# rafaelgmv/Distributed-Autonomous-Exploration-and-Mapping

Hardware: AMD Instinct MI355X
Metric: beam-cell updates/sec + frontier-extract ms on 16384² grid (higher is better)
Workload: dtype int32/u32 ray math + fp32 log-odds (fp64 endpoints)

## Files before the change

### distributed-autonomous-exploration-and-mapping_amd/csrc/dm_api.cpp

```cpp
#include <math.h>
#include <stdarg.h>
#include <stdio.h>
#include <string.h>

#include <algorithm>
#include <new>
#include <string>
#include <vector>

#include "dm_internal.h"

#include <stdlib.h>

hipError_t dm_sync_all(dm_grid* g) {
  for (hipStream_t s : {g->stream, g->fe_streams[0], g->fe_streams[1], g->pass_stream, g->big_stream}) {
    if (!s) continue;
    const hipError_t e = hipStreamSynchronize(s);
    if (e != hipSuccess) return e;
  }
  g->p_pending = false;
  for (auto& f : g->fw) f.busy_pending = false;
  return hipSuccess;
}

// ... 1302 lines not shown
  float* dr = nullptr;
  float* di = nullptr;
  auto cleanup = [&]() { dev_free(dp); dev_free(doff); dev_free(dr); dev_free(di); };
  if ((rc = dev_alloc(&dp, np, "ld06 points")) || (rc = dev_alloc(&doff, S + 1, "ld06 offsets")) ||
      (rc = dev_alloc(&dr, (int64_t)S * N, "ld06 ranges")) ||
      (intensities_out && (rc = dev_alloc(&di, (int64_t)S * N, "ld06 intensities")))) {
    cleanup();
    return rc;
  }
  hipError_t e = hipMemcpyAsync(dp, points, sizeof(dm_ld06_point) * (size_t)np, hipMemcpyHostToDevice, g->stream);
  if (e == hipSuccess)
    e = hipMemcpyAsync(doff, offsets, sizeof(int64_t) * (size_t)(S + 1), hipMemcpyHostToDevice, g->stream);
  if (e == hipSuccess) rc = dm_launch_ld06(g, S, dp, doff, N, laser_scan_dir ? 1 : 0, dr, di);
  if (e == hipSuccess && !rc)
    e = hipMemcpyAsync(ranges_out, dr, sizeof(float) * (size_t)S * N, hipMemcpyDeviceToHost, g->stream);
  if (e == hipSuccess && !rc && intensities_out)
    e = hipMemcpyAsync(intensities_out, di, sizeof(float) * (size_t)S * N, hipMemcpyDeviceToHost, g->stream);
  if (e == hipSuccess) e = hipStreamSynchronize(g->stream);
  cleanup();
  if (e != hipSuccess) return dm_hip_check(e, "dm_ld06_to_scans");
  return rc;
}

static const char kMagic[8] = {'D', 'M', 'A', 'P', '0', '0', '0', '1'};

int dm_save(dm_grid* g, const char* path) {
  int rc = check_grid(g);
  if (rc || (rc = use_device(g))) return rc;
  if (!path) return dm_set_error(DM_ERR_INVALID_ARG, "path is NULL");
  const int64_t cells = g->W * g->R;
  std::vector<float> L((size_t)cells);
  if ((rc = dm_get_logodds(g, L.data()))) return rc;
  FILE* f = fopen(path, "wb");
  if (!f) return dm_set_error(DM_ERR_IO, "cannot open %s for writing", path);
  bool ok = fwrite(kMagic, 1, 8, f) == 8 && fwrite(&g->p, sizeof(dm_params), 1, f) == 1 &&
            fwrite(L.data(), sizeof(float), (size_t)cells, f) == (size_t)cells;
  ok = (fclose(f) == 0) && ok;
  if (!ok) return dm_set_error(DM_ERR_IO, "short write to %s", path);
  return DM_OK;
}

int dm_load(dm_grid* g, const char* path) {
  int rc = check_grid(g);
  if (rc || (rc = use_device(g))) return rc;
  if (!path) return dm_set_error(DM_ERR_INVALID_ARG, "path is NULL");
  FILE* f = fopen(path, "rb");
  if (!f) return dm_set_error(DM_ERR_IO, "cannot open %s", path);
  char magic[8];
  dm_params p;
  const int64_t cells = g->W * g->R;
  std::vector<float> L((size_t)cells);
  bool ok = fread(magic, 1, 8, f) == 8 && memcmp(magic, kMagic, 8) == 0 &&
            fread(&p, sizeof p, 1, f) == 1;
  if (ok && (p.width != g->p.width || p.height != g->p.height || p.band_row0 != g->p.band_row0 ||
             p.band_rows != g->p.band_rows || p.resolution != g->p.resolution)) {
    fclose(f);
    return dm_set_error(DM_ERR_SHAPE, "checkpoint %s has a different grid geometry", path);
  }
  ok = ok && fread(L.data(), sizeof(float), (size_t)cells, f) == (size_t)cells;
  fclose(f);
  if (!ok) return dm_set_error(DM_ERR_IO, "%s is not a dm checkpoint or is truncated", path);
  return dm_set_logodds(g, L.data());
}

int dm_set_stream(dm_grid* g, void* stream) {
  if (int rc0 = not_on_sharded(g, "dm_set_stream")) return rc0;
  int rc = check_grid(g);
  if (rc || (rc = use_device(g))) return rc;
  DM_HIP(dm_sync_all(g));
  if (stream) {
    if (g->own_stream && g->stream) (void)hipStreamDestroy(g->stream);
    g->stream = (hipStream_t)stream;
    g->own_stream = false;
  } else if (!g->own_stream) {
    DM_HIP(hipStreamCreateWithFlags(&g->stream, hipStreamNonBlocking));
    g->own_stream = true;
  }
  return DM_OK;
}

int dm_synchronize(dm_grid* g) {
  if (g && g->sh) return dm_sh_synchronize(g);
  int rc = check_grid(g);
  if (rc || (rc = use_device(g))) return rc;
  DM_HIP(dm_sync_all(g));
  return DM_OK;
}

int dm_profile_enable(dm_grid* g, int enable) {
  if (g && g->sh) return dm_sh_profile_enable(g, enable);
  int rc = check_grid(g);
  if (rc) return rc;
  g->profile = enable != 0;
  return DM_OK;
}

int dm_profile_read(dm_grid* g, dm_kernel_stat* out, int32_t cap, int32_t* n_out) {
  if (g && g->sh) return dm_sh_profile_read(g, out, cap, n_out);
  int rc = check_grid(g);
  if (rc || (rc = use_device(g))) return rc;
  DM_HIP(hipStreamSynchronize(g->stream));
  for (auto& t : g->pending) {
    float ms = 0.0f;
    (void)hipEventElapsedTime(&ms, t.start, t.stop);
    (void)hipEventDestroy(t.start);
    (void)hipEventDestroy(t.stop);
    dm_kernel_stat* s = nullptr;
    for (auto& e : g->stats)
      if (t.name == e.name) s = &e;
    if (!s) {
      dm_kernel_stat ns;
      memset(&ns, 0, sizeof ns);
      snprintf(ns.name, sizeof ns.name, "%s", t.name.c_str());
      g->stats.push_back(ns);
      s = &g->stats.back();
    }
    s->launches += 1;
    s->total_ms += ms;
  }
  g->pending.clear();
  const int32_t n = (int32_t)g->stats.size();
  for (int32_t i = 0; i < std::min(n, cap); ++i) out[i] = g->stats[(size_t)i];
  if (n_out) *n_out = n;
  return DM_OK;
}

int dm_profile_reset(dm_grid* g) {
  if (g && g->sh) return dm_sh_profile_reset(g);
  int rc = check_grid(g);
  if (rc) return rc;
  int32_t n = 0;
  if ((rc = dm_profile_read(g, nullptr, 0, &n))) return rc;
  g->stats.clear();
  return DM_OK;
}

int dm_map_image(dm_grid* g, uint8_t* out) {
  if (g && g->sh) return (out ? dm_sh_map_image(g, out) : dm_set_error(DM_ERR_INVALID_ARG, "out is NULL"));
  int rc = check_grid(g);
  if (rc || (rc = use_device(g))) return rc;
  if (!out) return dm_set_error(DM_ERR_INVALID_ARG, "out is NULL");
  const int64_t cells = g->W * g->R;
  uint8_t* d = nullptr;
  if ((rc = dev_alloc(&d, cells, "image"))) return rc;
  rc = dm_launch_map_image(g, d);
  hipError_t e = hipSuccess;
  if (!rc) e = hipMemcpyAsync(out, d, (size_t)cells, hipMemcpyDeviceToHost, g->stream);
  if (!rc && e == hipSuccess) e = hipStreamSynchronize(g->stream);
  (void)hipFree(d);
  if (e != hipSuccess) return dm_hip_check(e, "dm_map_image");
  return rc;
}

}
```

### distributed-autonomous-exploration-and-mapping_amd/csrc/dm_frontier.hip

```cpp
#include "dm_internal.h"
#include "dm_uf.h"
#include "dm_phase.h"

#include <string.h>

#include <algorithm>

DM_PH_DECL(frontier)
DM_PH_DECL(ftile)

namespace {

constexpr int kFT = 256;
#ifndef DM_EDGE_KERNEL
#define DM_EDGE_KERNEL 1
#endif
#ifndef DM_EDGE_HALVE
#define DM_EDGE_HALVE 0
#endif
#if DM_EDGE_HALVE
#define EDGE_UNITE dm_uf_unite_idx_halve
#else
#define EDGE_UNITE dm_uf_unite_idx2
#endif
// ... 1318 lines not shown
    idx_out[p] = (int32_t)i;
  }
}

__global__ __launch_bounds__(256) void k_rs_rank(double ox, double oy, double res, long long* clusters,
                                                 const long long* sums, const long long* labels,
                                                 const unsigned long long* __restrict__ count, int64_t cap,
                                                 int64_t W, const unsigned long long* __restrict__ keys,
                                                 const int32_t* __restrict__ idx,
                                                 const int32_t* __restrict__ row_off,
                                                 dm_cluster* __restrict__ out, int32_t* __restrict__ rank_of,
                                                 unsigned long long* sorted, const unsigned long long* __restrict__ cnt,
                                                 int ncnt, int sorted_idx, const unsigned long long* __restrict__ fsh,
                                                 dm_raw_record* __restrict__ host_out, int64_t host_cap,
                                                 const unsigned long long* __restrict__ scan_failed) {
  const int64_t K = (int64_t)*count;
  if (*scan_failed) cap = -1;
  if (blockIdx.x == 0) write_rb_header(K, cap, sorted, cnt, ncnt, sorted_idx, fsh, host_out);
  if (K > cap) {
    fix_raw_records(clusters, sums, labels, K);
    return;
  }
  for (int64_t p = (int64_t)blockIdx.x * blockDim.x + threadIdx.x; p < K; p += (int64_t)gridDim.x * blockDim.x) {
    const unsigned long long key = keys[p];
    const int64_t row = (int64_t)(key / (unsigned long long)W);
    const int32_t lo = row_off[row], hi = row_off[row + 1];
    int32_t r = 0;
    int32_t q = lo;
    for (; q + 4 <= hi; q += 4)
      r += (keys[q] < key) + (keys[q + 1] < key) + (keys[q + 2] < key) + (keys[q + 3] < key);
    for (; q < hi; ++q) r += keys[q] < key;
    put_sorted(ox, oy, res, clusters, sums, labels, idx[p], (int64_t)lo + r, out, rank_of, host_out, host_cap);
  }
}

__global__ __launch_bounds__(256) void k_slot_labels(int64_t n, int64_t slot_cap, const int32_t* __restrict__ cslot,
                                                     const int32_t* __restrict__ slot_root,
                                                     const long long* __restrict__ slot_label,
                                                     long long* __restrict__ out) {
  for (int64_t i = (int64_t)blockIdx.x * blockDim.x + threadIdx.x; i < n;
       i += (int64_t)gridDim.x * blockDim.x) {
    const int32_t s = cslot[i];
    out[i] = (s < 0 || s >= slot_cap) ? -1 : slot_label[slot_root[s]];
  }
}

int grid_for(int64_t n, int threads, int64_t cap) {
  int64_t b = (n + threads - 1) / threads;
  if (b < 1) b = 1;
  if (b > cap) b = cap;
  return (int)b;
}

}

static_assert(sizeof(FGeom) == 88, "FGeom has no implicit padding");

static FGeom make_fgeom(const dm_grid* g, bool want_mask, bool want_labels) {
  FGeom fg;
  fg.W = (int32_t)g->W;
  fg.R = (int32_t)g->R;
  fg.row0 = (int32_t)g->row0;
  fg.TX = (int32_t)g->TX;
  fg.TY = (int32_t)g->TY;
  fg.NT = g->NT;
  fg.has_before = g->has_halo[0];
  fg.has_after = g->has_halo[1];
  fg.want_mask = want_mask ? 1 : 0;
  fg.want_labels = want_labels ? 1 : 0;
  fg.H = g->H;
  fg.slot_cap = g->slot_cap;
  fg.slot_per = g->slot_cap / kShards;
  fg.clu_cap = g->slot_cap;
  fg.min_size = g->p.min_frontier_size;
  return fg;
}

DM_PH_READER(frontier)
DM_PH_READER(ftile)

int dm_launch_edge_labels(dm_grid* g) {
  DM_LAUNCH(k_slot_labels, dim3(grid_for(2 * g->W, 256, 1024)), dim3(256), 0, g->stream,
                     2 * g->W, g->slot_cap, g->edge_slot, g->slot_root, g->slot_label, g->edge_label);
  DM_HIP(hipGetLastError());
  return DM_OK;
}

int dm_launch_rank_sort(hipStream_t stream, long long* clusters, const long long* sums,
                        const long long* labels, const unsigned long long* d_count,
                        int64_t max_records, double ox, double oy, double res, dm_cluster* out,
                        int32_t* rank_of, unsigned long long* d_sorted, const unsigned long long* cnt,
                        int ncnt, int sorted_idx, const unsigned long long* fsh, dm_raw_record* host_out,
                        int64_t host_cap, int64_t expect) {
  const int64_t cap = std::min<int64_t>(max_records, kRankSortCap);
  const int64_t want = dm_quantize_up(std::max<int64_t>(2 * expect, 2048));
  DM_LAUNCH(k_rank_sort, dim3(grid_for(std::min(cap, want), 64, 1 << 20)), dim3(kSortThreads), 0, stream,
                     ox, oy, res, clusters, sums, labels, d_count, cap, out, rank_of, d_sorted, cnt, ncnt, sorted_idx,
                     fsh, host_out, host_cap);
  DM_HIP(hipGetLastError());
  return DM_OK;
}

int dm_launch_bucket_sort(dm_grid* g, hipStream_t stream, long long* clusters, const long long* sums,
                          const long long* labels, const unsigned long long* d_count,
                          int64_t max_records, int64_t row_base, int64_t rows, dm_cluster* out,
                          int32_t* rank_of, unsigned long long* d_sorted, const unsigned long long* cnt,
                          int ncnt, int sorted_idx, const unsigned long long* fsh, dm_raw_record* host_out,
                          int64_t host_cap) {
  if (max_records > g->bs_cap || rows > g->rs_rows)
    return dm_set_error(DM_ERR_INVALID_ARG, "row sort: %lld records over %lld rows exceed its workspace",
                        (long long)max_records, (long long)rows);
  const long long base = row_base * g->W;
  const int64_t expect = std::min<int64_t>(max_records, std::max<int64_t>(2 * g->sort_hint, 4096));
  const int eg = grid_for(expect, 256, 4096);
  const int nsb = (int)((rows + kRsChunk - 1) / kRsChunk);
  DM_LAUNCH(k_rs_count, dim3(eg), dim3(256), 0, stream, clusters, labels, d_count, max_records, base, g->W,
            g->rs_cnt, g->bs_key, g->bs_idx2, g->rs_status, nsb);
  DM_HIP(hipGetLastError());
  DM_LAUNCH(k_rs_scan, dim3(nsb), dim3(256), 0, stream, d_count, max_records, rows, g->rs_cnt, g->rs_off,
            g->rs_status);
  DM_HIP(hipGetLastError());
  DM_LAUNCH(k_rs_place, dim3(eg), dim3(256), 0, stream, d_count, max_records, g->W, g->bs_key, g->bs_idx2,
            g->rs_off, g->bs_key2, g->bs_idx);
  DM_HIP(hipGetLastError());
  DM_LAUNCH(k_rs_rank, dim3(eg), dim3(256), 0, stream, g->p.origin_x, g->p.origin_y, g->p.resolution, clusters,
            sums, labels, d_count, max_records, g->W, g->bs_key2, g->bs_idx, g->rs_off, out, rank_of, d_sorted, cnt,
            ncnt, sorted_idx, fsh, host_out, host_cap, g->rs_status + nsb);
  DM_HIP(hipGetLastError());
  return DM_OK;
}

int dm_enqueue_frontiers(dm_grid* g, bool want_mask, bool want_labels, bool split, hipStream_t* end_stream) {
  const FGeom fg = make_fgeom(g, want_mask, want_labels);
  const int64_t cells = g->R * g->W;
  if (!split) DM_HIP(dm_join_pass_stream(g));
  ++g->rb[g->cur_slot].wepoch;
  ++g->fr_pass;
  g->fparity ^= 1;
  dm_grid::FrWs& fw = g->fw[g->fparity];
  if (fw.busy_pending) {
    DM_HIP(hipStreamWaitEvent(g->stream, fw.busy, 0));
    fw.busy_pending = false;
  }
  dm_select_fw(g, g->fparity);
  unsigned long long* list_n = g->fl_n + 16 * (g->fr_pass % 3);
  if (++g->relist_age >= g->relist_period)
    if (int rc = dm_launch_relist(g, true)) return rc;
  KernelTimer t;
  if (want_mask) DM_HIP(hipMemsetAsync(g->mask, 0, (size_t)cells, g->stream));
  if (want_labels) DM_HIP(hipMemsetAsync(g->cell_slot, 0xFF, sizeof(int32_t) * (size_t)cells, g->stream));
  const int64_t want_waves = g->ftile_hint > 0 ? dm_quantize_up(g->ftile_hint + g->ftile_hint / 4 + 64) : g->NT;
  const int wave_grid = grid_for(std::min<int64_t>(want_waves, g->NT), kFW, 8192);
  const int bits_grid = std::max(wave_grid, 64);
  const bool want_on = g->fmask_mode == 1 || (g->fmask_mode == 0 && g->ftile_hint >= kFmaskOnTiles);
  const bool want_off = g->fmask_mode == 2 || (g->fmask_mode == 0 && g->ftile_hint < kFmaskOnTiles / 4);
  if (!g->fmask_on && want_on) {
    if (!g->fmask_valid) {
      if (int rc = dm_launch_recount(g)) return rc;
    }
    g->fmask_on = true;
  } else if (g->fmask_on && want_off) {
    g->fmask_on = false;
  }
  const bool dense = g->frontier_kernel == 2 ||
                     (g->frontier_kernel == 0 && g->ftf_hint > 0 && g->runs_hint > kDenseRuns * g->ftf_hint &&
                      g->ftf_hint <= kDenseMaxTiles);
  const bool edge = DM_EDGE_KERNEL == 2 ||
                    (DM_EDGE_KERNEL == 1 && !dense && g->sort_hint <= std::max<int64_t>(g->ftile_hint, 1));
  auto* const big_kernel = edge ? k_frontier_tile_big<true> : k_frontier_tile_big<false>;
  auto* const wave_kernel = edge ? k_frontier_tile<true> : k_frontier_tile<false>;
  dm_timer_begin(g, "frontier_bits", &t);
  DM_LAUNCH(k_frontier_bits, dim3(bits_grid), dim3(kFW * 64), 0, g->stream, fg, g->state, g->halo, g->fmask,
            g->fedge, g->tile_seen, g->ftiles, g->ftiles_n, list_n, g->fbits, g->cnt, g->fmask_on ? 1 : 0,
            dense ? nullptr : g->big_tiles, g->fsh, g->edge_slot, 2 * g->W, g->slot_parent, g->fe_flag + kHaltWord,
            g->bits_flag + kStampWord);
  dm_timer_end(g, &t);
  DM_HIP(hipGetLastError());
  hipStream_t ps = g->stream;
  if (split) {
    ps = g->pass_stream;
    hipEvent_t eb = g->ev_bits[g->fparity];
    DM_HIP(hipEventRecord(eb, g->stream));
    DM_HIP(dm_mark_ws_free(g, eb));
    DM_HIP(hipStreamWaitEvent(ps, eb, 0));
  }
  if (end_stream) *end_stream = ps;
  if (!dense) {
    const int big_grid =
        grid_for(std::min<int64_t>(g->NT, dm_quantize_up(g->big_hint + g->big_hint / 4 + 64)), 1, 8192);
    DM_HIP(hipEventRecord(g->ev_bigfork, ps));
    DM_HIP(hipStreamWaitEvent(g->big_stream, g->ev_bigfork, 0));
    dm_timer_begin(g, "frontier_big", &t, g->big_stream);
    DM_LAUNCH(big_kernel, dim3(big_grid), dim3(kFT), 0, g->big_stream, fg, g->fbits,
              g->big_tiles,
              g->ftiles, list_n, g->border, g->rel, g->slot_label, g->slot_parent, g->slot_own,
              g->slot_acc, g->mask, g->cell_slot, g->edge_slot, g->cnt, g->fsh, 0);
    dm_timer_end(g, &t);
    DM_HIP(hipGetLastError());
    DM_HIP(hipEventRecord(g->ev_big, g->big_stream));
    dm_timer_begin(g, "frontier_tile", &t, ps);
    DM_LAUNCH(wave_kernel, dim3(wave_grid), dim3(kFW * 64), 0, ps, fg, g->fbits,
                       g->ftiles, list_n, g->border, g->rel,
                       g->slot_label, g->slot_parent, g->slot_own, g->slot_acc, g->mask, g->cell_slot,
                       g->edge_slot, g->cnt, g->fsh, g->big_tiles);
    dm_timer_end(g, &t);
    DM_HIP(hipGetLastError());
    DM_HIP(hipStreamWaitEvent(ps, g->ev_big, 0));
  } else {
    dm_timer_begin(g, "frontier_tile", &t, ps);
    const int dense_grid = grid_for(std::min<int64_t>(g->NT, g->ftile_hint > 0 ? want_waves : g->NT), 1, 8192);
    DM_LAUNCH(big_kernel, dim3(dense_grid), dim3(kFT), 0, ps, fg, g->fbits, nullptr,
              g->ftiles, list_n,
              g->border, g->rel, g->slot_label, g->slot_parent, g->slot_own, g->slot_acc, g->mask,
              g->cell_slot, g->edge_slot, g->cnt, g->fsh, 1);
    dm_timer_end(g, &t);
    DM_HIP(hipGetLastError());
  }
  if (edge) {
    dm_timer_begin(g, "frontier_edges", &t, ps);
    DM_LAUNCH(k_frontier_edges, dim3(grid_for(DM_EDGE_WAVES * std::min<int64_t>(want_waves, g->NT), kFW, 16384)),
              dim3(kFW * 64), 0, ps, fg, g->ftiles, list_n, g->border, g->rel,
              g->slot_parent, g->cnt);
    dm_timer_end(g, &t);
    DM_HIP(hipGetLastError());
  }
  const int sgrid = grid_for(g->slot_cap, 256, 1024);
  dm_timer_begin(g, "frontier_resolve", &t, ps);
  const int fuse = g->p.min_frontier_size <= 1 ? 1 : 0;
  DM_LAUNCH(k_frontier_resolve, dim3(grid_for(g->slot_cap, 256, g->n_cu)), dim3(256), 0, ps, fg,
                     g->slot_parent, g->slot_root, g->slot_own, g->slot_acc, g->fsh, fuse, g->slot_label,
                     g->clusters, g->slot_k, g->cnt);
  dm_timer_end(g, &t);
  DM_HIP(hipGetLastError());
  if (!fuse) {
    dm_timer_begin(g, "frontier_compact", &t, ps);
    DM_LAUNCH(k_frontier_compact, dim3(sgrid), dim3(256), 0, ps, fg,
                       g->slot_root, g->slot_label, g->slot_acc, g->clusters, g->slot_k, g->cnt, g->fsh);
    dm_timer_end(g, &t);
    DM_HIP(hipGetLastError());
  }
  if (want_labels) {
    DM_LAUNCH(k_slot_labels, dim3(grid_for(cells, 256, 8192)), dim3(256), 0, ps,
                       cells, g->slot_cap, g->cell_slot, g->slot_root, g->slot_label, g->labels);
    DM_HIP(hipGetLastError());
  }
  dm_timer_begin(g, "sort_clusters", &t, ps);
  const int rc = g->sort_hint > g->sort_min
      ? dm_launch_bucket_sort(g, ps, g->clusters, fuse ? g->slot_acc : nullptr, fuse ? g->slot_label : nullptr,
                              g->cnt + CNT_CLUSTERS, g->slot_cap, g->row0, g->R, g->out_clu,
                              g->rank_of, g->cnt + CNT_SORTED, g->cnt, CNT_N, CNT_SORTED, g->fsh,
                              g->h_out_dev, g->h_out_cap)
      : dm_launch_rank_sort(ps, g->clusters, fuse ? g->slot_acc : nullptr, fuse ? g->slot_label : nullptr,
                            g->cnt + CNT_CLUSTERS, g->slot_cap, g->p.origin_x,
                            g->p.origin_y, g->p.resolution, g->out_clu, g->rank_of, g->cnt + CNT_SORTED,
                            g->cnt, CNT_N, CNT_SORTED, g->fsh, g->h_out_dev, g->h_out_cap, g->sort_hint);
  dm_timer_end(g, &t);
  return rc;
}

int dm_frontiers_readback(dm_grid* g, int64_t* n_clusters, int64_t* copied) {
  const unsigned long long* hdr = dm_rb_header(g->h_out);
  memcpy(g->h_cnt, hdr, sizeof(unsigned long long) * CNT_N);
  *copied = std::min<int64_t>(g->h_out_cap, g->slot_cap);
  const unsigned long long most = hdr[CNT_N];
  if (g->h_cnt[CNT_OVERFLOW] & kOvPipeline)
    return dm_set_error(DM_ERR_PIPELINE, "the overlapped pipeline's front-end hand-off timed out: a map "
                                         "update was skipped; dm_reset the handle");
  if ((int64_t)most > g->slot_cap / kShards || (g->h_cnt[CNT_OVERFLOW] & kOvSlots)) {
    *n_clusters = (int64_t)most * kShards;
    return DM_ERR_CAPACITY;
  }
  if (g->h_cnt[CNT_OVERFLOW] & kOvUnionFind)
    return dm_set_error(DM_ERR_INCOMPLETE, "frontier union-find did not converge within its bound "
                                           "(dm_uf.h): this pass has no result");
  *n_clusters = (int64_t)g->h_cnt[CNT_CLUSTERS];
  g->sort_hint = *n_clusters;
  g->ftile_hint = (int64_t)g->h_cnt[CNT_FL0];
  g->runs_hint = (int64_t)hdr[CNT_N + 1];
  g->ftf_hint = (int64_t)hdr[CNT_N + 2];
  g->big_hint = (int64_t)hdr[CNT_N + 3];
  return DM_OK;
}

int dm_launch_frontiers(dm_grid* g, bool want_mask, bool want_labels, int64_t* n_clusters,
                        int64_t* copied) {
  int rc = dm_enqueue_frontiers(g, want_mask, want_labels);
  if (rc) return rc;
  DM_HIP(hipStreamSynchronize(g->stream));
  return dm_frontiers_readback(g, n_clusters, copied);
}
```

### distributed-autonomous-exploration-and-mapping_amd/csrc/dm_integrate.hip

```cpp
#include "dm_internal.h"
#include "dm_phase.h"

#include <algorithm>

DM_PH_DECL(integrate)
DM_TL_DECL(accum)

namespace {

constexpr int kLdsPitch = DM_TS + 1;

struct Geom {
  RayGeom r;
  int32_t act_cap;
  int64_t seg_cap;
  int64_t hitem_cap, heavy_cap;
  int64_t nb;
  int32_t chunks, chunk_len;
  int32_t sparse_pieces;
  int32_t pad;
};

struct BeamChunk {
  int64_t b;
  int32_t k_lo, k_hi;
};

__device__ inline BeamChunk beam_chunk(const Geom& g, int64_t v) {
  BeamChunk c;
  if (g.chunks == 1) {
    c.b = v; c.k_lo = 0; c.k_hi = 0x7FFFFFFF;
    return c;
  }
  const int32_t q = (int32_t)(v / g.nb);
  c.b = v - (int64_t)q * g.nb;
  c.k_lo = q * g.chunk_len;
  c.k_hi = q + 1 == g.chunks ? 0x7FFFFFFF : c.k_lo + g.chunk_len - 1;
  return c;
}

__device__ inline int lane_id() { return __lane_id(); }

constexpr int kHash = 1024;
constexpr int kProbe = 32;

__device__ inline uint32_t tile_hash(int32_t t) { return ((uint32_t)t * 2654435761u) >> 22; }

__device__ inline int hash_insert(int32_t* hkey, int32_t tile) {
  uint32_t h = tile_hash(tile);
  for (int p = 0; p < kProbe; ++p, h = (h + 1) & (kHash - 1)) {
    const int32_t k = atomicCAS(&hkey[h], -1, tile);
    if (k == -1 || k == tile) return (int)h;
  }
  return -1;
}

__device__ inline int hash_find(const int32_t* hkey, int32_t tile) {
  uint32_t h = tile_hash(tile);
  for (int p = 0; p < kProbe; ++p, h = (h + 1) & (kHash - 1)) {
    const int32_t k = hkey[h];
    if (k == tile) return (int)h;
    if (k == -1) return -1;
  }
  return -1;
}

struct LaneRun {
  bool head;
  int head_lane;
  int len;
  int rank;
};

__device__ inline LaneRun lane_run(int32_t tile) {
  const int lane = lane_id();
  const unsigned long long act = __ballot(1);
  const int32_t prev = __shfl_up(tile, 1);
  const bool prev_act = lane > 0 && ((act >> (lane - 1)) & 1ull);
  const bool head = !(prev_act && prev == tile);
  const unsigned long long heads = __ballot(head);
  const unsigned long long le = lane == 63 ? ~0ull : ((2ull << lane) - 1ull);
  LaneRun r;
  r.head = head;
  r.head_lane = 63 - __clzll(heads & le);
  const unsigned long long after = heads & ~le;
  const unsigned long long before_end = after ? ((1ull << (__ffsll(after) - 1)) - 1ull) : ~0ull;
  const unsigned long long from_head = ~((1ull << r.head_lane) - 1ull);
  r.len = __popcll(act & from_head & before_end);
  r.rank = __popcll(act & from_head & ((1ull << lane) - 1ull));
  return r;
}

__device__ inline void first_touch(const Geom& g, int32_t tile, int32_t old, int32_t* act_raw,
                                   unsigned long long* ish, unsigned long long* cnt) {
  if (old != 0) return;
  const int sh = blockIdx.x % kShards;
  const unsigned long long l = atomicAdd(&ish[sh * kShardWords + SH_ACT], 1ull);
  if (l < (unsigned long long)g.act_cap) act_raw[(int64_t)sh * g.act_cap + (int64_t)l] = tile;
  else atomicOr(&cnt[CNT_IOVERFLOW], 1ull);
}

__device__ inline PackedPiece make_piece(const Geom& g, const Beam& bm, int32_t tile, int32_t k0, int32_t k1) {
  const int32_t tx0 = (tile % g.r.TX) * DM_TS;
  const int32_t ty0 = (tile / g.r.TX) * DM_TS;
  return dm_pack_piece(dm_tile_piece(bm, k0, k1, g.r.row0, tx0, ty0, kLdsPitch));
}

__global__ __launch_bounds__(256) void k_beam_prep(RayArgs a, Geom g, const double* __restrict__ pose4,
                                                   const float* __restrict__ ranges,
                                                   const double* __restrict__ trig,
                                                   Beam* __restrict__ beams, int32_t* tile_count,
                                                   int32_t* act_raw, unsigned long long* ish,
                                                   int2* __restrict__ blk_hist, int32_t* __restrict__ blk_n,
                                                   unsigned long long* cnt) {
  __shared__ int32_t hkey[kHash];
  __shared__ int32_t hcnt[kHash];
  __shared__ int32_t s_nh;
  const int tid = threadIdx.x;
  for (int e = tid; e < kHash; e += 256) { hkey[e] = -1; hcnt[e] = 0; }
  if (tid == 0) s_nh = 0;
  __syncthreads();
  const int64_t v = (int64_t)blockIdx.x * blockDim.x + tid;
  if (v < g.nb * g.chunks) {
    const BeamChunk bc = beam_chunk(g, v);
    const int32_t s = (int32_t)(bc.b / a.N), i = (int32_t)(bc.b % a.N);
    const Beam bm = dm_make_beam(a, pose4, ranges, trig, s, i);
    if (bc.k_lo == 0) beams[bc.b] = bm;
    if ((bm.flags & 1) && bc.k_lo <= bm.n) {
      dm_for_each_piece(bm, g.r, [&](int32_t tile, int32_t, int32_t) {
        const LaneRun run = lane_run(tile);
        if (run.head) {
          const int h = hash_insert(hkey, tile);
          if (h >= 0) {
            atomicAdd(&hcnt[h], run.len);
          } else {
            const int32_t old = atomicAdd(&tile_count[tile], run.len);
            first_touch(g, tile, old, act_raw, ish, cnt);
          }
        }
      }, bc.k_lo, bc.k_hi);
    }
  }
  __syncthreads();
  int2* my_hist = blk_hist + (int64_t)blockIdx.x * kHash;
  for (int e = tid; e < kHash; e += 256) {
    const int32_t tile = hkey[e];
    if (tile < 0) continue;
    const int32_t old = atomicAdd(&tile_count[tile], hcnt[e]);
    first_touch(g, tile, old, act_raw, ish, cnt);
    my_hist[atomicAdd(&s_nh, 1)] = make_int2(tile, hcnt[e] | (e << 16));
  }
  __syncthreads();
  if (tid == 0) blk_n[blockIdx.x] = s_nh;
}

constexpr int kChunk = kIntegrateChunk;
// ... 58 lines not shown
  }
  __syncthreads();
  const int64_t n = min((int64_t)soff[kShards], (int64_t)g.act_cap);
  if (blockIdx.x == 0 && tid == 0) cnt[CNT_ACTIVE] = (unsigned long long)n;
  const int64_t stride = (int64_t)gridDim.x * blockDim.x;
  for (int64_t j0 = (int64_t)blockIdx.x * blockDim.x + (tid & ~63); j0 < n; j0 += stride) {
    const int64_t j = j0 + lane;
    int32_t t = -1, c = 0;
    if (j < n) {
      int a = 0, b = kShards - 1;
      while (a < b) {
        const int mid = (a + b + 1) >> 1;
        if (soff[mid] <= j) a = mid; else b = mid - 1;
      }
      t = act_raw[(int64_t)a * g.act_cap + (j - soff[a])];
      c = tile_count[t];
    }
    const bool heavy = c > kMedium;
    const bool medium = c > kChunk && !heavy;
    const bool sparse = t >= 0 && c <= g.sparse_pieces;
    const bool light = t >= 0 && c <= kChunk && !sparse;
    const int32_t nh_items = heavy ? (c + kChunk - 1) / kChunk : (medium ? 1 : 0);
    unsigned long long* const ctr[5] = {&cnt[CNT_SEGS], &cnt[CNT_ITEMS], &cnt[CNT_LITEMS], &cnt[CNT_SITEMS],
                                        &cnt[CNT_HEAVY]};
    const unsigned long long want[5] = {(unsigned long long)c, (unsigned long long)nh_items, light ? 1ull : 0ull,
                                        sparse ? 1ull : 0ull, heavy ? 1ull : 0ull};
    unsigned long long got[5];
    wave_alloc_n<5>(ctr, want, got);
    const unsigned long long p0 = got[0], hi = got[1], li = got[2], si = got[3], ho = got[4];
    if (t < 0) continue;
    tile_cur[t] = (int32_t)p0;
    const bool fits = (int64_t)(p0 + c) <= g.seg_cap && (int64_t)(hi + nh_items) <= g.hitem_cap &&
                      (int64_t)li < (int64_t)g.act_cap && (int64_t)si < (int64_t)g.act_cap &&
                      (int64_t)ho < g.heavy_cap;
    if (!fits) {
      atomicOr(&cnt[CNT_IOVERFLOW], 4ull);
      continue;
    }
    if (sparse) {
      litems[(int64_t)g.act_cap - 1 - (int64_t)si] = make_int4(t, (int32_t)p0, c, -1);
    } else if (light) {
      litems[li] = make_int4(t, (int32_t)p0, c, -1);
    } else if (medium) {
      hitems[hi] = make_int4(t, (int32_t)p0, c, -1);
    } else {
      const int32_t wide = c >= 65536 ? 1 : 0;
      heavy_list[ho] = t | (wide << 31);
      for (int32_t q = 0; q < nh_items; ++q)
        hitems[hi + q] = make_int4(t, (int32_t)p0 + q * kChunk, min(kChunk, c - q * kChunk),
                                   (int32_t)(2 * ho + wide));
    }
  }
}

__device__ inline void put_piece(const Geom& g, PackedPiece* pieces, int64_t idx, const Beam& bm,
                                 int32_t tile, int32_t k0, int32_t k1, unsigned long long* cnt) {
  if (idx >= 0 && idx < g.seg_cap) {
    pieces[idx] = make_piece(g, bm, tile, k0, k1);
  } else {
    atomicOr(&cnt[CNT_IOVERFLOW], 2ull);
  }
}

__global__ __launch_bounds__(256) void k_scatter(RayArgs a, Geom g, const Beam* __restrict__ beams,
                                                 int32_t* tile_cur, const int2* __restrict__ blk_hist,
                                                 const int32_t* __restrict__ blk_n,
                                                 PackedPiece* __restrict__ pieces, unsigned long long* cnt) {
  __shared__ int32_t hkey[kHash];
  __shared__ int32_t hcnt[kHash];
  __shared__ int32_t hbase[kHash];
  const int tid = threadIdx.x;
  for (int e = tid; e < kHash; e += 256) { hkey[e] = -1; hcnt[e] = 0; }
  const int64_t v = (int64_t)blockIdx.x * blockDim.x + tid;
  const bool in = v < g.nb * g.chunks;
  const BeamChunk bc = beam_chunk(g, in ? v : 0);
  Beam bm;
  bm.flags = 0;
  if (in) bm = beams[bc.b];
  const int32_t nh = blk_n[blockIdx.x];
  __syncthreads();
  const int2* my_hist = blk_hist + (int64_t)blockIdx.x * kHash;
  for (int e = tid; e < nh; e += 256) {
    const int2 te = my_hist[e];
    const int h = hash_insert(hkey, te.x);
    if (h >= 0) hbase[h] = atomicAdd(&tile_cur[te.x], te.y & 0xFFFF);
  }
  __syncthreads();
  const bool valid = in && (bm.flags & 1) && bc.k_lo <= bm.n;
  if (valid) {
    dm_for_each_piece(bm, g.r, [&](int32_t tile, int32_t k0, int32_t k1) {
      const LaneRun run = lane_run(tile);
      int32_t pos = -1;
      if (run.head) {
        const int h = hash_find(hkey, tile);
        pos = h >= 0 ? hbase[h] + atomicAdd(&hcnt[h], run.len) : atomicAdd(&tile_cur[tile], run.len);
      }
      pos = __shfl(pos, run.head_lane);
      put_piece(g, pieces, (int64_t)pos + run.rank, bm, tile, k0, k1, cnt);
    }, bc.k_lo, bc.k_hi);
  }
}

struct ApplyArgs {
  float l_occ, l_free, l_min, l_max, occ_t, free_t;
};

__device__ inline int8_t state_of(const ApplyArgs& p, float L) {
  int32_t r = -1;
  r = L <= p.free_t ? 0 : r;
  r = L >= p.occ_t ? 100 : r;
  r = L == 0.0f ? -1 : r;
  return (int8_t)r;
}

__device__ inline float apply_one(const ApplyArgs& p, float L, uint32_t h, uint32_t m) {
  const float t = (float)h * p.l_occ;
  const float u = (float)m * p.l_free;
  L = L + t;
  L = L + u;
  return __builtin_amdgcn_fmed3f(L, p.l_min, p.l_max);
}

#ifndef DM_APPLY_BFI
#define DM_APPLY_BFI 1
#endif
__device__ inline uint32_t nz_mask(uint32_t x) {
  uint32_t r;
  asm("v_min_u32_e32 %0, 1, %1\n\tv_sub_u32_e32 %0, 0, %0" : "=&v"(r) : "v"(x));
  return r;
}
__device__ inline uint32_t bfi(uint32_t m, uint32_t a, uint32_t b) {
  uint32_t r;
  asm("v_bfi_b32 %0, %1, %2, %3" : "=v"(r) : "v"(m), "v"(a), "v"(b));
  return r;
}
__device__ inline uint32_t state_bits(const ApplyArgs& p, float L) {
  const int32_t sge = (int32_t)__float_as_uint(L - p.occ_t) >> 31;
  const int32_t sle = (int32_t)__float_as_uint(p.free_t - L) >> 31;
  const int32_t mz = (int32_t)((__float_as_uint(L) & 0x7FFFFFFFu) - 1u) >> 31;
  uint32_t s = bfi((uint32_t)sle, 0xFFFFFFFFu, 0u);
  s = bfi((uint32_t)sge, s, 100u);
  return s | (uint32_t)mz;
}

__device__ inline uint8_t state_nibbles(uint32_t w) {
  auto zb = [](uint32_t v) {
    uint32_t t = (v & 0x7F7F7F7Fu) + 0x7F7F7F7Fu;
    t = ~(t | v | 0x7F7F7F7Fu);
    return (((t >> 7) * 0x00204081u) >> 21) & 0xFu;
  };
  return (uint8_t)(zb(w) | (zb(~w) << 4));
}

template <class G>
__device__ inline uint8_t state_nibbles_at(const G& g, const int8_t* __restrict__ state, int32_t x0, int32_t y) {
  uint32_t fn = 0u, un = 0u;
  for (int e = 0; e < 4; ++e) {
    if (x0 + e >= g.r.W) break;
    const int8_t b = state[(int64_t)y * g.r.W + x0 + e];
    fn |= (b == 0 ? 1u : 0u) << e;
    un |= (b == -1 ? 1u : 0u) << e;
  }
  return (uint8_t)(fn | (un << 4));
}

__device__ inline uint32_t every4th(uint64_t x) {
  x &= 0x1111111111111111ull;
  x = (x | (x >> 3)) & 0x0303030303030303ull;
  x = (x | (x >> 6)) & 0x000F000F000F000Full;
  x = (x | (x >> 12)) & 0x000000FF000000FFull;
  return (uint32_t)((x | (x >> 24)) & 0xFFFFull);
}

struct EdgeAcc {
  uint64_t w[4] = {0ull, 0ull, 0ull, 0ull};
};
__device__ inline void edge_acc(EdgeAcc& e, uint32_t out, int q, int lane) {
  const int c = lane & 3;
  const uint64_t b0 = __ballot(c == 0 && ((out >> 4) & 1u));
  const uint64_t b3 = __ballot(c == 3 && ((out >> 31) & 1u));
  e.w[0] |= (uint64_t)every4th(b0) << (16 * q);
  e.w[1] |= (uint64_t)every4th(b3 >> 3) << (16 * q);
  if (q == 0 || q == 3) {
    const uint32_t u16 = ((out >> 4) & 0xFu) | ((out >> 8) & 0xF0u) | ((out >> 12) & 0xF00u) | ((out >> 16) & 0xF000u);
    const int base = q == 0 ? 0 : 60;
    uint64_t r = 0ull;
#pragma unroll
    for (int k = 0; k < 4; ++k) r |= (uint64_t)__shfl(u16, base + k) << (16 * k);
    e.w[q == 0 ? 2 : 3] = r;
  }
}

__device__ inline void edge_store(const EdgeAcc& e, uint64_t* __restrict__ fedge, int64_t tile, uint64_t rows,
                                  int lane) {
  if (lane >= 4) return;
  const uint64_t v = lane == 0 ? e.w[0] : lane == 1 ? e.w[1] : lane == 2 ? e.w[2] : e.w[3];
  const uint64_t m = lane < 2 ? rows : ((rows >> (lane == 2 ? 0 : 63)) & 1ull) ? ~0ull : 0ull;
  uint64_t* p = fedge + tile * 4 + lane;
  if (m == ~0ull) *p = v;
  else if (m) *p = (*p & ~m) | (v & m);
}

__device__ inline int32_t zero_bytes(uint32_t x) {
  uint32_t t = (x & 0x7F7F7F7Fu) + 0x7F7F7F7Fu;
  t = ~(t | x | 0x7F7F7F7Fu);
  return __popc(t);
}

template <int ROWS>
struct CellRows {
  float4 l[ROWS];
  char4 s[ROWS];
  bool vec;

  __device__ void prefetch(const Geom& g, int32_t tx0, int32_t ty0, int ly0, int dly, int cx,
                           const float* __restrict__ L, const int8_t* __restrict__ state, int vec_ok) {
    vec = vec_ok && tx0 + cx + 4 <= g.r.W;
#pragma unroll
    for (int rr = 0; rr < ROWS; ++rr) {
      const int32_t y = ty0 + ly0 + rr * dly;
      const int64_t base = (vec && y < g.r.R) ? (int64_t)y * g.r.W + tx0 + cx : 0;
      l[rr] = *reinterpret_cast<const float4*>(L + base);
      s[rr] = *reinterpret_cast<const char4*>(state + base);
    }
  }

  template <class Touched>
  __device__ void load_touched(const Geom& g, int32_t tx0, int32_t ty0, int ly0, int dly, int cx,
                               const float* __restrict__ L, const int8_t* __restrict__ state, int vec_ok,
                               Touched&& touched) {
    vec = vec_ok && tx0 + cx + 4 <= g.r.W;
#pragma unroll
    for (int rr = 0; rr < ROWS; ++rr) {
      const int32_t y = ty0 + ly0 + rr * dly;
      l[rr] = make_float4(0.0f, 0.0f, 0.0f, 0.0f);
      s[rr] = make_char4(0, 0, 0, 0);
      if (vec && y < g.r.R && touched(ly0 + rr * dly)) {
        const int64_t base = (int64_t)y * g.r.W + tx0 + cx;
        l[rr] = *reinterpret_cast<const float4*>(L + base);
        s[rr] = *reinterpret_cast<const char4*>(state + base);
      }
    }
  }

  template <class Counts>
  __device__ void apply(const Geom& g, const ApplyArgs& p, int32_t tx0, int32_t ty0, int ly0, int dly,
                        int cx, float* __restrict__ L, int8_t* __restrict__ state, Counts&& counts,
                        int32_t* sh_T, int32_t* sh_free, uint32_t* sh_U) {
    int32_t dT = 0, dFree = 0;
    uint32_t dU = 0;
#pragma unroll
    for (int rr = 0; rr < ROWS; ++rr) {
      const int ly = ly0 + rr * dly;
      const int32_t y = ty0 + ly;
      if (y >= g.r.R) continue;
      uint32_t h4[4], m4[4];
      counts(ly, h4, m4);
      if (((h4[0] | m4[0]) | (h4[1] | m4[1]) | (h4[2] | m4[2]) | (h4[3] | m4[3])) == 0u) continue;
      const int64_t base = (int64_t)y * g.r.W + tx0 + cx;
      if (sh_U) {
#pragma unroll
        for (int e = 0; e < 4; ++e) dU += tx0 + cx + e < g.r.W ? h4[e] + m4[e] : 0u;
      }
      if (vec && DM_APPLY_BFI) {
        const float lv[4] = {l[rr].x, l[rr].y, l[rr].z, l[rr].w};
        const uint32_t sw = *reinterpret_cast<const uint32_t*>(&s[rr]);
        uint32_t nlb[4], nsw = 0u, msk = 0u;
#pragma unroll
        for (int e = 0; e < 4; ++e) {
          const uint32_t mh = nz_mask(h4[e] | m4[e]);
          const float nl = apply_one(p, lv[e], h4[e], m4[e]);
          nlb[e] = bfi(mh, __float_as_uint(nl), __float_as_uint(lv[e]));
          nsw |= (state_bits(p, nl) & 0xFFu) << (8 * e);
          msk |= (mh & 0xFFu) << (8 * e);
          dT += (int32_t)(mh & 1u);
        }
        const uint32_t ns = bfi(msk, nsw, sw);
        dFree += zero_bytes(ns) - zero_bytes(sw);
        *reinterpret_cast<float4*>(L + base) =
            make_float4(__uint_as_float(nlb[0]), __uint_as_float(nlb[1]), __uint_as_float(nlb[2]),
                        __uint_as_float(nlb[3]));
        *reinterpret_cast<uint32_t*>(state + base) = ns;
      } else if (vec) {
        float lv[4] = {l[rr].x, l[rr].y, l[rr].z, l[rr].w};
        int8_t sv[4] = {(int8_t)s[rr].x, (int8_t)s[rr].y, (int8_t)s[rr].z, (int8_t)s[rr].w};
#pragma unroll
        for (int e = 0; e < 4; ++e) {
          const bool hit = (h4[e] | m4[e]) != 0u;
          const float nl = apply_one(p, lv[e], h4[e], m4[e]);
          const int8_t ns = state_of(p, nl);
          lv[e] = hit ? nl : lv[e];
          sv[e] = hit ? ns : sv[e];
          dT += hit ? 1 : 0;
        }
        const char4 ns4 = make_char4(sv[0], sv[1], sv[2], sv[3]);
        dFree += zero_bytes(*reinterpret_cast<const uint32_t*>(&ns4)) -
                 zero_bytes(*reinterpret_cast<const uint32_t*>(&s[rr]));
        *reinterpret_cast<float4*>(L + base) = make_float4(lv[0], lv[1], lv[2], lv[3]);
        *reinterpret_cast<char4*>(state + base) = ns4;
      } else {
        for (int e = 0; e < 4; ++e) {
          if ((h4[e] | m4[e]) == 0u || tx0 + cx + e >= g.r.W) continue;
          const int64_t i = base + e;
          const int8_t old = state[i];
          const float nl = apply_one(p, L[i], h4[e], m4[e]);
          const int8_t ns = state_of(p, nl);
          L[i] = nl;
          state[i] = ns;
          dT += 1;
          dFree += (ns == 0) - (old == 0);
        }
      }
    }
    if (dT) atomicAdd(sh_T, dT);
    if (dFree) atomicAdd(sh_free, dFree);
    if (dU) atomicAdd(sh_U, dU);
  }
};

__device__ inline int32_t walk_tp(uint32_t* tl, const TilePiece& tp, int32_t len, int lane) {
  int32_t wl = len;
  for (int o = 32; o > 0; o >>= 1) wl = max(wl, __shfl_xor(wl, o));
  const int32_t s0 = len > 0 ? lane % len : 0;
  PieceCursor cur;
  cur.init(tp);
  if (s0 > 0) {
    const int32_t num = tp.rem0 + s0 * tp.two_adb;
    const int32_t dq = dm_udiv_small(num, tp.two_n, __builtin_amdgcn_rcpf((float)tp.two_n));
    cur.addr = tp.addr0 + s0 * tp.da + dq * tp.db;
    cur.rem = num - dq * tp.two_n;
  }
  int32_t k = s0;
  for (int32_t st = 0; st < wl; ++st) {
    if (st < len) {
      atomicAdd(&tl[cur.addr], 1u);
      cur.step(tp);
      if (++k == len) cur.init(tp);
    }
  }
  if (len > 0 && tp.addr_end >= 0) atomicAdd(&tl[tp.addr_end], 0xFFFFu);
  return len;
}

__device__ inline int32_t walk_piece(uint32_t* tl, const PackedPiece& mine, bool valid, int lane) {
  const TilePiece tp = dm_unpack_piece(mine.x, mine.y, mine.z, mine.w);
  return walk_tp(tl, tp, valid ? tp.len : 0, lane);
}

#ifndef DM_SPLIT_WALK
#define DM_SPLIT_WALK 1
#endif

__device__ inline int32_t walk_tp_split(uint32_t* tl, const TilePiece& tp, int32_t len, int32_t f, int32_t part,
                                        float rf, int lane) {
  const SplitPart sp = dm_split_part(len, f, part, rf);
  int32_t wl = sp.n;
  for (int o = 32; o > 0; o >>= 1) wl = max(wl, __shfl_xor(wl, o));
  const int32_t spare = kTileWords + lane;
  PieceCursor cur;
  if (f == 1) cur.init(tp);
  else cur.init_at(tp, sp.j0, __builtin_amdgcn_rcpf((float)tp.two_n));
  for (int32_t st = 0; st < wl; ++st) {
    atomicAdd(&tl[st < sp.n ? cur.addr : spare], 1u);
    cur.step(tp);
  }
  if (sp.n > 0 && sp.j0 + sp.n == len && tp.addr_end >= 0) atomicAdd(&tl[tp.addr_end], 0xFFFFu);
  return sp.n;
}

constexpr int kSparseMax = 15;
#ifndef DM_SPARSE_LIST
#define DM_SPARSE_LIST 256
#endif
constexpr int kSparseList = DM_SPARSE_LIST > 0 ? DM_SPARSE_LIST : 1;

__device__ inline int32_t to_pitch64(int32_t a) {
  return a >= 0 ? a - a / kLdsPitch : -((-a) - (-a) / kLdsPitch);
}

__device__ inline int32_t walk_piece_bytes(uint32_t* tq, const PackedPiece& mine, bool valid, int32_t f,
                                           int32_t part, float rf) {
  TilePiece tp = dm_unpack_piece(mine.x, mine.y, mine.z, mine.w);
  const int32_t len = valid ? tp.len : 0;
  const SplitPart sp = dm_split_part(len, f, part, rf);
  int32_t wl = sp.n;
  for (int o = 32; o > 0; o >>= 1) wl = max(wl, __shfl_xor(wl, o));
  tp.addr0 = to_pitch64(tp.addr0);
  tp.da = to_pitch64(tp.da);
  tp.db = to_pitch64(tp.db);
  PieceCursor cur;
  if (f == 1) cur.init(tp);
  else cur.init_at(tp, sp.j0, __builtin_amdgcn_rcpf((float)tp.two_n));
  for (int32_t st = 0; st < wl; ++st) {
    if (st < sp.n) atomicAdd(&tq[cur.addr >> 2], 1u << (8 * (cur.addr & 3)));
    cur.step(tp);
  }
  if (sp.n > 0 && sp.j0 + sp.n == len && tp.addr_end >= 0) {
    const int32_t e = to_pitch64(tp.addr_end);
    atomicAdd(&tq[e >> 2], 0x0Fu << (8 * (e & 3)));
  }
  return sp.n;
}

__device__ inline PackedPiece no_piece() {
  PackedPiece q;
  q.x = 0u; q.y = 0u; q.z = 0u; q.w = 1u;
  return q;
}

__device__ inline int32_t free_update(int32_t old, int32_t dfree, int32_t tile, int32_t* tlist,
                                      unsigned long long* tlist_n) {
  int32_t v = old + dfree;
  if (dfree > 0 && !(old & kTileListed)) {
    v |= kTileListed;
    tlist[atomicAdd(tlist_n, 1ull)] = tile;
  }
  return v;
}

__device__ inline void finish_tile(const Geom& g, int32_t tile, int32_t T, int32_t dfree, uint32_t U,
                                   bool heavy, int32_t* tile_count, int32_t* tile_free, int32_t old_free,
                                   int32_t* tlist, unsigned long long* tlist_n, unsigned long long* ish) {
  unsigned long long* sh = ish + (blockIdx.x % kShards) * kShardWords;
  if (T) {
    atomicAdd(&sh[SH_T], (unsigned long long)T);
    if (heavy) atomicAdd(&sh[SH_TH], (unsigned long long)T);
  }
  if (U) atomicAdd(&sh[SH_U], (unsigned long long)U);
  if (dfree) tile_free[tile] = free_update(old_free, dfree, tile, tlist, tlist_n);
  tile_count[tile] = 0;
}

__device__ inline void heavy_quarter(const Geom& g, const ApplyArgs& p, int64_t h, int q, int32_t tile,
                                     bool wide, uint32_t* __restrict__ slabs, float* __restrict__ L,
                                     int8_t* __restrict__ state, int32_t* s_T, int32_t* s_free,
                                     uint32_t* s_U) {
  constexpr int kQ = DM_TS * DM_TS / 4;
  const int tid = threadIdx.x;
  const int32_t x = (tile % g.r.TX) * DM_TS + (tid & 63);
  const int32_t yq = (tile / g.r.TX) * DM_TS + q * (DM_TS / 4) + (tid >> 6);
  uint32_t* sh = slabs + h * (2 * DM_TS * DM_TS) + q * kQ + tid;
  uint32_t hc[4], mc[4];
  float lv[4];
  int8_t sv[4];
#pragma unroll
  for (int k = 0; k < 4; ++k) {
    const int32_t y = yq + 4 * k;
    lv[k] = 0.0f;
    sv[k] = 0;
    if (y < g.r.R && x < g.r.W) {
      lv[k] = L[(int64_t)y * g.r.W + x];
      sv[k] = state[(int64_t)y * g.r.W + x];
    }
  }
#pragma unroll
  for (int k = 0; k < 4; ++k) {
    hc[k] = atomicExch(sh + k * kQuarter, 0u);
    mc[k] = wide ? atomicExch(sh + DM_TS * DM_TS + k * kQuarter, 0u) : 0u;
  }
  int32_t dT = 0, dFree = 0;
  uint32_t dU = 0;
#pragma unroll
  for (int k = 0; k < 4; ++k) {
    uint32_t hk = hc[k], mk;
    if (wide) {
      mk = mc[k];
    } else {
      mk = hk & 0xFFFFu;
      hk >>= 16;
    }
    const int32_t y = yq + 4 * k;
    if ((hk | mk) == 0u || y >= g.r.R || x >= g.r.W) continue;
    const int64_t i = (int64_t)y * g.r.W + x;
    const float nl = apply_one(p, lv[k], hk, mk);
    const int8_t ns = state_of(p, nl);
    L[i] = nl;
    state[i] = ns;
    dU += hk + mk;
    dT += 1;
    dFree += (ns == 0) - (sv[k] == 0);
  }
  if (dT) atomicAdd(s_T, dT);
  if (dFree) atomicAdd(s_free, dFree);
  if (dU) atomicAdd(s_U, dU);
}

#ifndef DM_ACCUM_OCC
#define DM_ACCUM_OCC 7
#endif
#ifndef DM_EARLY_PIECES
#define DM_EARLY_PIECES 1
#endif
constexpr int kAccumPerCu = DM_ACCUM_OCC;
__global__ __launch_bounds__(kQuarter, kAccumPerCu) void k_tile_accum(
    Geom g, ApplyArgs p, const int4* __restrict__ list_a, int cnt_a, const int4* __restrict__ list_b,
    int cnt_b, int cnt_c, const PackedPiece* __restrict__ pieces, int32_t* tile_count, int32_t* tile_free,
    uint32_t* __restrict__ slabs, float* __restrict__ L, int8_t* __restrict__ state,
    const unsigned long long* __restrict__ cnt, unsigned long long* ish, int vec_ok,
    const int32_t* __restrict__ heavy_list, int32_t* heavy_done, int32_t* tlist, unsigned long long* tlist_n,
    unsigned long long* hint, const unsigned long long* __restrict__ halt, uint8_t* __restrict__ tile_seen) {
  __shared__ uint32_t tl[kTileWords + 64];
  __shared__ int32_t s_T, s_free, s_last;
  __shared__ uint32_t s_U;
  const int tid = threadIdx.x, lane = lane_id();
  DM_TL_BEGIN();
  const unsigned long long hv = *halt;
  const unsigned long long ca = cnt[cnt_a];
  const unsigned long long cb = cnt[cnt_b];
  const unsigned long long cc = cnt[cnt_c];
  const int64_t HI = min((int64_t)ca, g.hitem_cap);
  const int64_t LI = min((int64_t)cb, (int64_t)g.act_cap);
  const int64_t n_items = HI + LI;
  const int64_t SI = min((int64_t)cc, (int64_t)g.act_cap);
  const int64_t G = gridDim.x;
  const int64_t sp_rank = ((int64_t)blockIdx.x - n_items % G + G) % G;
  if (blockIdx.x == 0 && tid == 0) {
    volatile unsigned long long* h = hint;
    h[0] = (unsigned long long)(n_items + (SI + 3) / 4);
    h[1] = (unsigned long long)(n_items + SI);
  }
  const unsigned long long idle =
      ((int64_t)blockIdx.x >= n_items && sp_rank * (kQuarter / 64) >= SI) ? 1ull : 0ull;
  if ((hv | idle) != 0ull) {
    DM_TL_END(accum, 0);
    return;
  }
  auto item_of = [&](int64_t it) {
    int4 d = it < n_items ? (it < HI ? list_a[it] : list_b[it - HI]) : make_int4(0, 0, 0, -1);
    d.z = (int64_t)d.y + d.z <= g.seg_cap ? d.z : 0;
    return d;
  };
  const int cx = (tid & 15) * 4;
  __shared__ unsigned long long s_accT, s_accU;
  int4 info = item_of(blockIdx.x);
  int4 next = item_of(blockIdx.x + G);
  PackedPiece mine;
  CellRows<4> cells;
  int32_t tfree;
  auto split_of = [&](const int4& d) -> int32_t {
    const int32_t c = __builtin_amdgcn_readfirstlane(d.z);
    const int32_t heavy = __builtin_amdgcn_readfirstlane(d.w);
    return DM_SPLIT_WALK && heavy < 0 ? dm_split_factor(c, kQuarter) : 1;
  };
  auto piece_of = [&](int32_t f) -> int32_t {
    return f == 1 ? tid : dm_udiv_small(tid, f, __builtin_amdgcn_rcpf((float)f));
  };
  auto load_pieces = [&](const int4& d) -> PackedPiece {
    const int32_t c0 = __builtin_amdgcn_readfirstlane(d.y);
    const int32_t c = __builtin_amdgcn_readfirstlane(d.z);
    return pieces[c0 + min(piece_of(split_of(d)), max(c - 1, 0))];
  };
  mine = load_pieces(info);
  PackedPiece mine_n = mine;
  for (int e = tid; e < kTileWords; e += kQuarter) tl[e] = 0u;
  if (tid == 0) { s_T = 0; s_free = 0; s_U = 0u; s_accT = 0ull; s_accU = 0ull; }
  __syncthreads();
  DM_PH_INIT();
  [[maybe_unused]] unsigned long long tl_word = 0;
  for (int64_t it = blockIdx.x; it < n_items; it += G) {
    tl_word += 1;
    const int32_t tile = __builtin_amdgcn_readfirstlane(info.x);
    const int32_t c0 = __builtin_amdgcn_readfirstlane(info.y);
    const int32_t c = __builtin_amdgcn_readfirstlane(info.z);
    const int32_t heavy = __builtin_amdgcn_readfirstlane(info.w);
    const int32_t tx0 = (tile % g.r.TX) * DM_TS, ty0 = (tile / g.r.TX) * DM_TS;
    DM_PH(dm_phase_acc_integrate, 0);
    if (heavy >= 0) {
      walk_piece(tl, mine, tid < c, lane);
      if (DM_EARLY_PIECES) mine_n = load_pieces(next);
      __syncthreads();
      DM_PH(dm_phase_acc_integrate, 1);
      DM_PH_COUNT(dm_phase_acc_integrate, 17, 1);
      DM_PH_COUNT(dm_phase_acc_integrate, 19, c);
      uint32_t* sh = slabs + (int64_t)(heavy >> 1) * (2 * DM_TS * DM_TS);
      if (heavy & 1) {
        for (int e = tid; e < DM_TS * DM_TS; e += kQuarter) {
          const uint32_t v = tl[(e >> 6) * kLdsPitch + (e & 63)];
          const uint32_t h = v >> 16, m = v & 0xFFFFu;
          if (h) atomicAdd(&sh[e], h);
          if (m) atomicAdd(&sh[DM_TS * DM_TS + e], m);
        }
      } else {
        for (int e = tid; e < DM_TS * DM_TS; e += kQuarter) {
          const uint32_t v = tl[(e >> 6) * kLdsPitch + (e & 63)];
          if (v) atomicAdd(&sh[e], v);
        }
      }
      DM_PH(dm_phase_acc_integrate, 2);
      asm volatile("s_waitcnt vmcnt(0)" ::: "memory");
      __syncthreads();
      if (tid == 0) {
        const int32_t n_it = (tile_count[tile] + kChunk - 1) / kChunk;
        s_last = atomicAdd(&heavy_done[heavy >> 1], 1) == n_it - 1;
      }
      __syncthreads();
      if (s_last) {
#ifdef DM_PHASE_TIMING
        const long long tf0 = wall_clock64();
#endif
        const int64_t h = heavy >> 1;
        const bool wide = heavy_list[h] < 0;
        const int32_t old_free = tid == 0 ? tile_free[tile] : 0;
        for (int q = 0; q < 4; ++q)
          heavy_quarter(g, p, h, q, tile, wide, slabs, L, state, &s_T, &s_free, &s_U);
        __syncthreads();
        if (tid == 0) {
          finish_tile(g, tile, s_T, s_free, s_U, true, tile_count, tile_free, old_free, tlist, tlist_n, ish);
          heavy_done[h] = 0;
          tile_seen[tile] = 1;
        }
#ifdef DM_PHASE_TIMING
        tl_word += (unsigned long long)(wall_clock64() - tf0) << 32;
#endif
      }
    } else {
      tfree = tile_free[tile];
      cells.prefetch(g, tx0, ty0, tid >> 4, 16, cx, L, state, vec_ok);
      int32_t u;
      if (c <= kChunk) {
        const int32_t f = split_of(info);
        const int32_t pi = piece_of(f);
        const TilePiece tp = dm_unpack_piece(mine.x, mine.y, mine.z, mine.w);
        u = walk_tp_split(tl, tp, pi < c ? tp.len : 0, f, tid - pi * f, __builtin_amdgcn_rcpf((float)f), lane);
      } else {
        u = walk_piece(tl, mine, tid < c, lane);
        for (int32_t r0 = kChunk; r0 < c; r0 += kChunk) {
          const PackedPiece more = r0 + tid < c ? pieces[c0 + r0 + tid] : no_piece();
          u += walk_piece(tl, more, r0 + tid < c, lane);
        }
      }
      const bool inside = tx0 + DM_TS <= g.r.W && ty0 + DM_TS <= g.r.R;
      if (inside) {
        for (int o = 32; o > 0; o >>= 1) u += __shfl_xor(u, o);
        if (lane == 0) atomicAdd(&s_U, (uint32_t)u);
      }
      if (DM_EARLY_PIECES) mine_n = load_pieces(next);
      __syncthreads();
      DM_PH(dm_phase_acc_integrate, 3);
      DM_PH_COUNT(dm_phase_acc_integrate, 16, 1);
      DM_PH_COUNT(dm_phase_acc_integrate, 18, c);
      cells.apply(g, p, tx0, ty0, tid >> 4, 16, cx, L, state,
                  [&](int ly, uint32_t* h4, uint32_t* m4) {
                    for (int e = 0; e < 4; ++e) {
                      const uint32_t v = tl[ly * kLdsPitch + cx + e];
                      h4[e] = v >> 16;
                      m4[e] = v & 0xFFFFu;
                    }
                  },
                  &s_T, &s_free, inside ? nullptr : &s_U);
      DM_PH(dm_phase_acc_integrate, 4);
    }
    __syncthreads();
    if (tid == 0 && heavy < 0) {
      s_accT += (unsigned long long)s_T;
      s_accU += (unsigned long long)s_U;
      if (s_free) tile_free[tile] = free_update(tfree, s_free, tile, tlist, tlist_n);
      tile_count[tile] = 0;
      tile_seen[tile] = 1;
    }
    info = next;
    next = item_of(it + 2 * G);
    mine = DM_EARLY_PIECES ? mine_n : load_pieces(info);
    for (int e = tid; e < kTileWords; e += kQuarter) tl[e] = 0u;
    if (tid == 0) { s_T = 0; s_free = 0; s_U = 0u; }
    __syncthreads();
  }
  __shared__ int32_t s_wT[kQuarter / 64], s_wfree[kQuarter / 64];
  __shared__ uint32_t s_wU[kQuarter / 64];
  __shared__ uint16_t s_list[kQuarter / 64][kSparseList];
  const int wv = tid >> 6;
  uint32_t* tq = tl + wv * (DM_TS * DM_TS / 4);
  const int hcx = (lane & 15) * 4;
  if (lane == 0) { s_wT[wv] = 0; s_wfree[wv] = 0; s_wU[wv] = 0u; }
  const int nw = kQuarter / 64;
  for (int64_t it = sp_rank * nw + wv; it < SI; it += (int64_t)G * nw) {
    int4 d = list_b[(int64_t)g.act_cap - 1 - it];
    d.z = (int64_t)d.y + d.z <= g.seg_cap ? d.z : 0;
    const int32_t tile = d.x, c0 = d.y, c = d.z;
    if (lane == 0 && wv == 0) tl_word += 1ull << 16;
    const int32_t tx0 = (tile % g.r.TX) * DM_TS, ty0 = (tile / g.r.TX) * DM_TS;
    const int32_t fs = DM_SPLIT_WALK ? dm_split_factor(c, 64) : 1;
    const float rfs = __builtin_amdgcn_rcpf((float)fs);
    const int32_t spi = fs == 1 ? lane : dm_udiv_small(lane, fs, rfs);
    const PackedPiece sp = spi < c ? pieces[c0 + spi] : no_piece();
    const int32_t sfree = tile_free[tile];
    int32_t u = walk_piece_bytes(tq, sp, spi < c, fs, lane - spi * fs, rfs);
    const bool inside = tx0 + DM_TS <= g.r.W && ty0 + DM_TS <= g.r.R;
    uint32_t wU = 0u;
    if (inside) {
      for (int o = 32; o > 0; o >>= 1) u += __shfl_xor(u, o);
      wU = (uint32_t)u;
    }
    __builtin_amdgcn_fence(__ATOMIC_ACQ_REL, "wavefront");
    __builtin_amdgcn_wave_barrier();
    DM_PH(dm_phase_acc_integrate, 6);
    auto counts = [&](int wi, uint32_t* h4, uint32_t* m4) {
      const uint32_t w = tq[wi];
      for (int e = 0; e < 4; ++e) {
        const uint32_t v = (w >> (8 * e)) & 0xFFu;
        h4[e] = v >> 4;
        m4[e] = v & 0xFu;
      }
    };
    uint16_t* lst = s_list[wv];
    int nt = 0;
    {
      const unsigned long long lt = (1ull << lane) - 1ull;
#pragma unroll
      for (int k = 0; k < 16; ++k) {
        const int wi = k * 64 + lane;
        const bool nz = tq[wi] != 0u;
        const unsigned long long m = __ballot(nz);
        const int at = nt + __popcll(m & lt);
        if (nz && at < kSparseList) lst[at] = (uint16_t)wi;
        nt += __popcll(m);
      }
    }
    __builtin_amdgcn_fence(__ATOMIC_ACQ_REL, "wavefront");
    __builtin_amdgcn_wave_barrier();
    if (DM_SPARSE_LIST > 0 && nt <= kSparseList) {
      for (int e0 = 0; e0 < nt; e0 += 128) {
        const int ea = e0 + lane, eb = e0 + 64 + lane;
        const int wa = ea < nt ? lst[ea] : 0, wb = eb < nt ? lst[eb] : 0;
        CellRows<1> ca, cb;
        ca.load_touched(g, tx0, ty0, wa >> 4, 0, (wa & 15) * 4, L, state, vec_ok, [&](int) { return ea < nt; });
        cb.load_touched(g, tx0, ty0, wb >> 4, 0, (wb & 15) * 4, L, state, vec_ok, [&](int) { return eb < nt; });
        if (ea < nt)
          ca.apply(g, p, tx0, ty0, wa >> 4, 0, (wa & 15) * 4, L, state,
                   [&](int, uint32_t* h4, uint32_t* m4) { counts(wa, h4, m4); }, &s_wT[wv], &s_wfree[wv],
                   inside ? nullptr : &s_wU[wv]);
        if (eb < nt)
          cb.apply(g, p, tx0, ty0, wb >> 4, 0, (wb & 15) * 4, L, state,
                   [&](int, uint32_t* h4, uint32_t* m4) { counts(wb, h4, m4); }, &s_wT[wv], &s_wfree[wv],
                   inside ? nullptr : &s_wU[wv]);
      }
    } else {
      for (int pass = 0; pass < 4; ++pass) {
        const int ly0 = (lane >> 4) + 16 * pass;
        CellRows<4> sc;
        sc.load_touched(g, tx0, ty0, ly0, 4, hcx, L, state, vec_ok,
                        [&](int ly) { return tq[ly * 16 + (hcx >> 2)] != 0u; });
        sc.apply(g, p, tx0, ty0, ly0, 4, hcx, L, state,
                 [&](int ly, uint32_t* h4, uint32_t* m4) { counts(ly * 16 + (hcx >> 2), h4, m4); },
                 &s_wT[wv], &s_wfree[wv], inside ? nullptr : &s_wU[wv]);
      }
    }
    DM_PH(dm_phase_acc_integrate, 7);
    DM_PH_COUNT(dm_phase_acc_integrate, 21, 1);
    DM_PH_COUNT(dm_phase_acc_integrate, 22, c);
    __builtin_amdgcn_fence(__ATOMIC_ACQ_REL, "wavefront");
    __builtin_amdgcn_wave_barrier();
    if (lane == 0) {
      const int32_t T = s_wT[wv], df = s_wfree[wv];
      const uint32_t U = s_wU[wv] + wU;
      atomicAdd(&s_accT, (unsigned long long)T);
      atomicAdd(&s_accU, (unsigned long long)U);
      if (df) tile_free[tile] = free_update(sfree, df, tile, tlist, tlist_n);
      tile_count[tile] = 0;
      tile_seen[tile] = 1;
      s_wT[wv] = 0;
      s_wfree[wv] = 0;
      s_wU[wv] = 0u;
    }
    for (int e = lane; e < DM_TS * DM_TS / 4; e += 64) tq[e] = 0u;
    __builtin_amdgcn_fence(__ATOMIC_ACQ_REL, "wavefront");
    __builtin_amdgcn_wave_barrier();
  }
  __syncthreads();
  if (tid == 0) {
    unsigned long long* sh = ish + (blockIdx.x % kShards) * kShardWords;
    if (s_accT) atomicAdd(&sh[SH_T], s_accT);
    if (s_accU) atomicAdd(&sh[SH_U], s_accU);
  }
  DM_PH_FLUSH(dm_phase_acc_integrate);
  DM_TL_END(accum, tl_word);
}


__global__ __launch_bounds__(256) void k_integrate_reset(unsigned long long* cnt, unsigned long long* ish) {
  const int i = blockIdx.x * blockDim.x + threadIdx.x;
  constexpr int nI = (int)(sizeof(kIntegrateCounters) / sizeof(kIntegrateCounters[0]));
  if (i < nI) cnt[kIntegrateCounters[i]] = 0ull;
  if (i < kShards * kShardWords) ish[i] = 0ull;
}

constexpr unsigned long long kGateTicks = 500000000ull;

__global__ __launch_bounds__(64) void k_seq_signal(unsigned long long* flag) {
  if (threadIdx.x != 0) return;
  const unsigned long long v = __hip_atomic_load(flag + kSigWord, __ATOMIC_RELAXED, __HIP_MEMORY_SCOPE_AGENT);
  __hip_atomic_store(flag + kSigWord, v + 1, __ATOMIC_RELAXED, __HIP_MEMORY_SCOPE_AGENT);
}

__global__ __launch_bounds__(64) void k_seq_gate(unsigned long long* flag, unsigned long long* err,
                                                 unsigned long long err_bit, unsigned long long ticks,
                                                 unsigned long long fault) {
  if (threadIdx.x != 0) return;
  const unsigned long long seq = flag[kGateWord] + 1;
  flag[kGateWord] = seq;
  const unsigned long long t0 = wall_clock64();
  while (__hip_atomic_load(flag + kSigWord, __ATOMIC_RELAXED, __HIP_MEMORY_SCOPE_AGENT) < seq + fault) {
    __builtin_amdgcn_s_sleep(2);
    if (wall_clock64() - t0 > ticks) {
      atomicOr(err, err_bit);
      return;
    }
  }
}

__device__ inline uint8_t fmask_byte(uint64_t fm, uint64_t um, int j) {
  return (uint8_t)(((fm >> (4 * j)) & 0xFull) | (((um >> (4 * j)) & 0xFull) << 4));
}

__global__ __launch_bounds__(256) void k_recount(Geom g, const int8_t* __restrict__ state,
                                                 int32_t* __restrict__ tile_free, uint8_t* __restrict__ fmask,
                                                 uint64_t* __restrict__ fedge, uint8_t* __restrict__ tile_seen) {
  const int64_t tile = blockIdx.x;
  const int32_t tx0 = (int32_t)(tile % g.r.TX) * DM_TS, ty0 = (int32_t)(tile / g.r.TX) * DM_TS;
  __shared__ int32_t acc, seen;
  __shared__ uint64_t s_edge[4][4];
  if (threadIdx.x == 0) { acc = 0; seen = 0; }
  __syncthreads();
  int32_t c = 0, known = 0;
  uint64_t ew[4] = {0ull, 0ull, 0ull, 0ull};
  uint8_t* tm = fmask + tile * (DM_TS * 16);
  for (int e = threadIdx.x; e < DM_TS * DM_TS; e += 256) {
    const int32_t x = tx0 + (e & 63), y = ty0 + (e >> 6);
    const int8_t b = (x < g.r.W && y < g.r.R) ? state[(int64_t)y * g.r.W + x] : (int8_t)1;
    c += b == 0;
    known |= (x < g.r.W && y < g.r.R && b != -1) ? 1 : 0;
    const uint64_t fm = __ballot(b == 0);
    const uint64_t um = __ballot(b == -1);
    const int l = e & 63, r = e >> 6;
    if (l < 16) tm[r * 16 + l] = fmask_byte(fm, um, l);
    ew[0] |= (um & 1ull) << r;
    ew[1] |= (um >> 63) << r;
    if (r == 0) ew[2] = um;
    if (r == DM_TS - 1) ew[3] = um;
  }
  if (c) atomicAdd(&acc, c);
  if (known) seen = 1;
  const int l4 = __lane_id();
  if (l4 < 4) s_edge[threadIdx.x >> 6][l4] = l4 == 0 ? ew[0] : l4 == 1 ? ew[1] : l4 == 2 ? ew[2] : ew[3];
  __syncthreads();
  if (threadIdx.x == 0) {
    tile_free[tile] = acc;
    tile_seen[tile] = (uint8_t)seen;
  }
  if (threadIdx.x < 4)
    fedge[tile * 4 + threadIdx.x] = s_edge[0][threadIdx.x] | s_edge[1][threadIdx.x] | s_edge[2][threadIdx.x] |
                                    s_edge[3][threadIdx.x];
}

constexpr int kListIters = 16;
__global__ __launch_bounds__(256) void k_list_tiles(int64_t NT, int32_t* __restrict__ tile_free,
                                                    int32_t* __restrict__ ftiles, unsigned long long* list_n,
                                                    int iters) {
  const int lane = __lane_id();
  __shared__ int32_t s_wn[kListIters][4];
  __shared__ unsigned long long s_base;
  const int w = threadIdx.x >> 6;
  const int64_t chunk = (int64_t)iters * blockDim.x;
  for (int64_t c0 = (int64_t)blockIdx.x * chunk; c0 < NT; c0 += (int64_t)gridDim.x * chunk) {
    uint32_t mine = 0u;
    for (int i = 0; i < iters; ++i) {
      const int64_t t = c0 + (int64_t)i * blockDim.x + threadIdx.x;
      if (t >= NT) continue;
      const int32_t v = tile_free[t];
      const bool f = (v & kTileFreeMask) > 0;
      mine |= (f ? 1u : 0u) << i;
      if (f != ((v & kTileListed) != 0)) tile_free[t] = f ? (v | kTileListed) : (v & kTileFreeMask);
    }
    for (int i = 0; i < iters; ++i) {
      const unsigned long long bal = __ballot((mine >> i) & 1u);
      if (lane == 0) s_wn[i][w] = __popcll(bal);
    }
    __syncthreads();
    if (threadIdx.x == 0) {
      int total = 0;
      for (int i = 0; i < iters; ++i) total += s_wn[i][0] + s_wn[i][1] + s_wn[i][2] + s_wn[i][3];
      s_base = total ? atomicAdd(list_n, (unsigned long long)total) : 0ull;
    }
    __syncthreads();
    int64_t pre = (int64_t)s_base;
    for (int i = 0; i < iters; ++i) {
      const bool f = (mine >> i) & 1u;
      const unsigned long long bal = __ballot(f);
      int before = 0;
      for (int q = 0; q < w; ++q) before += s_wn[i][q];
      if (f) {
        const int64_t t = c0 + (int64_t)i * blockDim.x + threadIdx.x;
        ftiles[pre + before + __popcll(bal & ((1ull << lane) - 1ull))] = (int32_t)t;
      }
      pre += s_wn[i][0] + s_wn[i][1] + s_wn[i][2] + s_wn[i][3];
    }
    __syncthreads();
  }
}

__device__ inline uint64_t upto_rows(int p) {
  return p >= 63 ? ~0ull : ((2ull << p) - 1ull);
}

__global__ __launch_bounds__(256) void k_fmask_items(Geom g, const int4* __restrict__ list_a, int cnt_a,
                                                     const int4* __restrict__ list_b, int cnt_b, int cnt_c,
                                                     const PackedPiece* __restrict__ pieces,
                                                     const unsigned long long* __restrict__ cnt,
                                                     const int8_t* __restrict__ state, uint8_t* __restrict__ fmask,
                                                     uint64_t* __restrict__ fedge,
                                                     const unsigned long long* __restrict__ halt) {
  if (*halt) return;
  const int64_t HI = min((int64_t)cnt[cnt_a], g.hitem_cap);
  const int64_t LI = min((int64_t)cnt[cnt_b], (int64_t)g.act_cap);
  const int64_t SI = min((int64_t)cnt[cnt_c], (int64_t)g.act_cap);
  const int lane = __lane_id();
  for (int64_t it = (int64_t)blockIdx.x * 4 + (threadIdx.x >> 6); it < HI + LI + SI;
       it += (int64_t)gridDim.x * 4) {
    const int4 d = it < HI ? list_a[it]
                           : (it < HI + LI ? list_b[it - HI] : list_b[(int64_t)g.act_cap - 1 - (it - HI - LI)]);
    const int32_t tile = __builtin_amdgcn_readfirstlane(d.x);
    uint64_t rows = ~0ull;
    if (it >= HI + LI) {
      const int32_t c0 = __builtin_amdgcn_readfirstlane(d.y);
      const int32_t c = __builtin_amdgcn_readfirstlane(d.z);
      uint64_t mine = 0ull;
      if (lane < c && (int64_t)c0 + c <= g.seg_cap) {
        const PackedPiece q = pieces[c0 + lane];
        const TilePiece tp = dm_unpack_piece(q.x, q.y, q.z, q.w);
        if (tp.len > 0) {
          const int32_t ya = tp.addr0 / kLdsPitch;
          const int32_t yb = dm_piece_addr(tp, tp.len - 1, __builtin_amdgcn_rcpf((float)tp.two_n)) / kLdsPitch;
          const int lo = min(ya, yb), hi = max(ya, yb);
          mine = upto_rows(hi) & ~(lo > 0 ? upto_rows(lo - 1) : 0ull);
        }
      }
      for (int o = 32; o > 0; o >>= 1) mine |= __shfl_xor(mine, o);
      rows = mine;
    }
    const int32_t tx0 = (tile % g.r.TX) * DM_TS, ty0 = (tile / g.r.TX) * DM_TS;
    const int32_t x0 = tx0 + (lane & 3) * 16;
    uint8_t* tm = fmask + (int64_t)tile * (DM_TS * 16);
    EdgeAcc ea;
#pragma unroll
    for (int q = 0; q < 4; ++q) {
      const int ly = 16 * q + (lane >> 2);
      const bool mine = (rows >> ly) & 1ull;
      const int32_t y = ty0 + ly;
      uint32_t out = 0u;
      if (mine && y < g.r.R) {
        const int64_t off = (int64_t)y * g.r.W + x0;
        if (x0 + 16 <= g.r.W && (off & 15) == 0) {
          const uint4 v = *reinterpret_cast<const uint4*>(state + off);
          const uint32_t wd[4] = {v.x, v.y, v.z, v.w};
#pragma unroll
          for (int k = 0; k < 4; ++k) out |= (uint32_t)state_nibbles(wd[k]) << (8 * k);
        } else {
          for (int k = 0; k < 4; ++k) out |= (uint32_t)state_nibbles_at(g, state, x0 + 4 * k, y) << (8 * k);
        }
      }
      if (mine) *reinterpret_cast<uint32_t*>(tm + ly * 16 + (lane & 3) * 4) = out;
      edge_acc(ea, out, q, lane);
    }
    edge_store(ea, fedge, tile, rows, lane);
  }
}

__global__ __launch_bounds__(256) void k_state_from_l(ApplyArgs p, int64_t cells, const float* __restrict__ L,
                                                      int8_t* __restrict__ state) {
  for (int64_t i = (int64_t)blockIdx.x * blockDim.x + threadIdx.x; i < cells;
       i += (int64_t)gridDim.x * blockDim.x)
    state[i] = state_of(p, L[i]);
}

__global__ __launch_bounds__(256) void k_set_state(ApplyArgs p, int64_t cells, const int8_t* __restrict__ in,
                                                   float* __restrict__ L, int8_t* __restrict__ state) {
  for (int64_t i = (int64_t)blockIdx.x * blockDim.x + threadIdx.x; i < cells;
       i += (int64_t)gridDim.x * blockDim.x) {
    const int8_t v = in[i];
    const float l = v == 100 ? p.l_occ : (v == 0 ? p.l_free : 0.0f);
    L[i] = l;
    state[i] = state_of(p, l);
  }
}

__global__ __launch_bounds__(256) void k_map_image(int64_t R, int64_t W, const int8_t* __restrict__ state,
                                                   uint8_t* __restrict__ img) {
  const int64_t cells = R * W;
  for (int64_t i = (int64_t)blockIdx.x * blockDim.x + threadIdx.x; i < cells;
       i += (int64_t)gridDim.x * blockDim.x) {
    const int64_t y = i / W, x = i - y * W;
    const int8_t v = state[i];
    img[(R - 1 - y) * W + x] = v == 0 ? 255 : (v == 100 ? 0 : 127);
  }
}

static_assert(sizeof(Geom) == 72 && sizeof(RayArgs) == 40 && sizeof(ApplyArgs) == 24,
              "kernel argument structs have no implicit padding");

Geom make_geom(const dm_grid* g) {
  Geom ge;
  ge.r.W = (int32_t)g->W;
  ge.r.R = (int32_t)g->R;
  ge.r.row0 = (int32_t)g->row0;
  ge.r.TX = (int32_t)g->TX;
  ge.r.TY = (int32_t)g->TY;
  ge.act_cap = (int32_t)g->act_cap;
  ge.seg_cap = g->segs_cap;
  ge.hitem_cap = g->hitem_cap;
  ge.heavy_cap = g->heavy_cap;
  ge.nb = 0;
  ge.chunks = 1;
  ge.chunk_len = 0;
  ge.sparse_pieces = std::min(g->sparse_pieces, kSparseMax);
  ge.pad = 0;
  return ge;
}

ApplyArgs make_apply(const dm_grid* g) {
  ApplyArgs a;
  a.l_occ = g->p.l_occ;
  a.l_free = g->p.l_free;
  a.l_min = g->p.l_min == 0.0f ? 0.0f : g->p.l_min;
  a.l_max = g->p.l_max == 0.0f ? 0.0f : g->p.l_max;
  a.occ_t = g->p.occ_thresh == 0.0f ? 0.0f : g->p.occ_thresh;
  a.free_t = g->p.free_thresh == 0.0f ? 0.0f : g->p.free_thresh;
  return a;
}

int grid_for(int64_t n, int threads, int64_t cap = 8192) {
  int64_t b = (n + threads - 1) / threads;
  if (b < 1) b = 1;
  if (b > cap) b = cap;
  return (int)b;
}

}

DM_PH_READER(integrate)
DM_TL_READER(accum)

int dm_launch_integrate(dm_grid* g, int32_t S, const double* d_pose4, int32_t N,
                        const float* d_ranges, const double* d_trig) {
  const int64_t nb = (int64_t)S * N;
  g->iw_cur = (g->iw_cur + 1) % dm_grid::kIntSets;
  dm_grid::IntWs& w = g->iw[g->iw_cur];
  hipStream_t fs = g->stream;
  if (g->overlap) {
    fs = dm_fe_stream_of(g, g->iw_cur);
    DM_HIP(dm_mark_ws_free(g));
    DM_HIP(hipStreamWaitEvent(fs, w.free_wait ? w.free_wait : w.ev_free, 0));
  }
  DM_LAUNCH(k_integrate_reset, dim3(2), dim3(256), 0, fs, w.cnt, w.sh);
  DM_HIP(hipGetLastError());
  if (nb == 0) {
    if (g->overlap) {
      DM_HIP(hipEventRecord(g->ev_fe, fs));
      DM_HIP(hipStreamWaitEvent(g->stream, g->ev_fe, 0));
      w.free_owed = true;
    }
    return DM_OK;
  }
  RayArgs a;
  a.S = S;
  a.N = N;
  a.ox = g->p.origin_x;
  a.oy = g->p.origin_y;
  a.res = g->p.resolution;
  a.range_min = g->p.range_min;
  a.range_max = g->p.range_max;
  Geom ge = make_geom(g);
  ge.nb = nb;
  ge.chunks = dm_integrate_chunks(g, nb);
  ge.chunk_len = (int32_t)((g->nmax + ge.chunks) / ge.chunks);
  const int nblk = (int)((nb * ge.chunks + 255) / 256);
  KernelTimer t;
  dm_timer_begin(g, "beam_prep", &t, fs);
  DM_LAUNCH(k_beam_prep, dim3(nblk), dim3(256), 0, fs, a, ge, d_pose4, d_ranges,
            d_trig, w.beams, w.tile_count, w.act_raw, w.sh, w.blk_hist, w.blk_n, w.cnt);
  dm_timer_end(g, &t);
  DM_HIP(hipGetLastError());
  dm_timer_begin(g, "plan", &t, fs);
  DM_LAUNCH(k_plan, dim3(grid_for(g->act_cap, kPlanThreads, 256)), dim3(kPlanThreads), 0, fs,
                     ge, w.act_raw, w.sh, w.tile_cur, w.tile_count, w.hitems, w.litems,
                     w.heavy_list, w.cnt);
  dm_timer_end(g, &t);
  DM_HIP(hipGetLastError());
  dm_timer_begin(g, "scatter", &t, fs);
  DM_LAUNCH(k_scatter, dim3(nblk), dim3(256), 0, fs, a, ge, w.beams,
            w.tile_cur, w.blk_hist, w.blk_n, w.pieces, w.cnt);
  dm_timer_end(g, &t);
  DM_HIP(hipGetLastError());
  if (g->overlap) {
    DM_HIP(hipEventRecord(g->ev_fe_end[g->iw_cur % 2], fs));
    unsigned long long* flag = dm_fe_flag_of(g, g->iw_cur);
    if (int rc = dm_launch_signal(fs, flag)) return rc;
    if (int rc = dm_launch_gate(g->stream, flag, g->fe_flag + kHaltWord, 1ull, g->fault_gate ? 1000ull : 0ull,
                                g->fault_gate ? (1ull << 40) : 0ull))
      return rc;
  }
#ifdef DM_FE_DUMMY
  if (g->overlap) {
    struct Dummy {
      Beam* beams = nullptr; int32_t* tc = nullptr; int32_t* act = nullptr; int2* hist = nullptr;
      int32_t* hn = nullptr; unsigned long long* sh = nullptr; unsigned long long* cnt = nullptr;
      int64_t nb = 0, nt = 0, blocks = 0, act_cap = 0;
    };
    static Dummy d;
    if (d.nb < nb || d.nt < g->NT || d.blocks < nblk || d.act_cap < g->act_cap) {
      (void)hipDeviceSynchronize();
      for (void* q : {(void*)d.beams, (void*)d.tc, (void*)d.act, (void*)d.hist, (void*)d.hn, (void*)d.sh,
                      (void*)d.cnt})
        if (q) (void)hipFree(q);
      d.nb = nb; d.nt = g->NT; d.blocks = nblk; d.act_cap = g->act_cap;
      DM_HIP(hipMalloc((void**)&d.beams, sizeof(Beam) * nb));
      DM_HIP(hipMalloc((void**)&d.tc, sizeof(int32_t) * g->NT));
      DM_HIP(hipMalloc((void**)&d.act, sizeof(int32_t) * g->act_cap * kShards));
      DM_HIP(hipMalloc((void**)&d.hist, sizeof(int2) * 1024 * nblk));
      DM_HIP(hipMalloc((void**)&d.hn, sizeof(int32_t) * nblk));
      DM_HIP(hipMalloc((void**)&d.sh, sizeof(unsigned long long) * kShards * kShardWords));
      DM_HIP(hipMalloc((void**)&d.cnt, sizeof(unsigned long long) * CNT_N));
    }
    DM_HIP(hipMemsetAsync(d.tc, 0, sizeof(int32_t) * g->NT, fs));
    DM_LAUNCH(k_integrate_reset, dim3(2), dim3(256), 0, fs, d.cnt, d.sh);
    DM_LAUNCH(k_beam_prep, dim3(nblk), dim3(256), 0, fs, a, ge, d_pose4, d_ranges, d_trig, d.beams, d.tc,
              d.act, d.sh, d.hist, d.hn, d.cnt);
    DM_HIP(hipGetLastError());
  }
#endif
  const int vec_ok = (g->W % 4 == 0) ? 1 : 0;
  dm_timer_begin(g, "tile_accum", &t);
  const volatile unsigned long long* hint = g->h_hint;
  const int64_t cap = g->hitem_cap + g->act_cap;
#ifndef DM_ACCUM_HINT
#define DM_ACCUM_HINT 1
#endif
  const int64_t hw = DM_ACCUM_HINT ? (int64_t)hint[0] : 0, hi = DM_ACCUM_HINT ? (int64_t)hint[1] : 0;
  const int64_t accum_wgs = hw > 0 ? std::min(cap, dm_quantize_up(hw + hw / 16 + 64)) : cap;
  DM_LAUNCH(k_tile_accum, dim3(grid_for(accum_wgs, 1, dm_grid::kAccumGrid)),
                     dim3(kQuarter), 0,
                     g->stream, ge, make_apply(g), w.hitems, (int)CNT_ITEMS, w.litems, (int)CNT_LITEMS,
                     (int)CNT_SITEMS, w.pieces, w.tile_count, g->tile_free, w.slabs, g->L, g->state, w.cnt, w.sh, vec_ok,
                     w.heavy_list, w.heavy_done, g->ftiles, g->ftiles_n, g->d_hint, g->fe_flag + kHaltWord,
                     g->tile_seen);
  dm_timer_end(g, &t);
  DM_HIP(hipGetLastError());
  if (g->overlap) w.free_owed = true;
  if (!g->fmask_on) {
    g->fmask_valid = false;
    return DM_OK;
  }
  dm_timer_begin(g, "fmask", &t);
  const int64_t fmask_items = hi > 0 ? std::min(cap, dm_quantize_up(hi + hi / 16 + 64)) : cap;
  DM_LAUNCH(k_fmask_items, dim3(grid_for(fmask_items, 4, 8192)), dim3(256), 0, g->stream,
                     ge, w.hitems, (int)CNT_ITEMS, w.litems, (int)CNT_LITEMS, (int)CNT_SITEMS, w.pieces, w.cnt,
                     g->state, g->fmask, g->fedge,
                     g->fe_flag + kHaltWord);
  dm_timer_end(g, &t);
  DM_HIP(hipGetLastError());
  return DM_OK;
}

int dm_launch_signal(hipStream_t s, unsigned long long* flag) {
  DM_LAUNCH(k_seq_signal, dim3(1), dim3(64), 0, s, flag);
  DM_HIP(hipGetLastError());
  return DM_OK;
}

int dm_launch_gate(hipStream_t s, unsigned long long* flag, unsigned long long* err, unsigned long long err_bit,
                   unsigned long long ticks, unsigned long long fault) {
  DM_LAUNCH(k_seq_gate, dim3(1), dim3(64), 0, s, flag, err, err_bit, ticks ? ticks : kGateTicks, fault);
  DM_HIP(hipGetLastError());
  return DM_OK;
}

int dm_launch_relist(dm_grid* g, bool swap) {
  if (swap) {
    const int x = 1 - g->flist_cur;
    if (g->flist_ev_set[x] && hipEventQuery(g->flist_ev[x]) != hipSuccess)
      DM_HIP(hipStreamWaitEvent(g->stream, g->flist_ev[x], 0));
    if (g->pass_stream) {
      DM_HIP(hipEventRecord(g->flist_ev[g->flist_cur], g->pass_stream));
      g->flist_ev_set[g->flist_cur] = true;
    }
    g->flist_cur = x;
    g->ftiles = g->flist[x];
    g->ftiles_n = g->flist_n[x];
  }
  DM_HIP(hipMemsetAsync(g->ftiles_n, 0, sizeof(unsigned long long), g->stream));
  const int iters = (int)std::min<int64_t>(kListIters, std::max<int64_t>(1, (g->NT + 65535) / 65536));
  DM_LAUNCH(k_list_tiles, dim3(grid_for((g->NT + iters - 1) / iters, 256, 1024)), dim3(256), 0, g->stream,
            g->NT, g->tile_free, g->ftiles, g->ftiles_n, iters);
  DM_HIP(hipGetLastError());
  g->relist_age = 0;
  g->relist_period = swap ? std::min(2 * g->relist_period, kRelistPasses) : 1;
  return DM_OK;
}

int dm_launch_recount(dm_grid* g) {
  const Geom ge = make_geom(g);
  DM_HIP(dm_join_pass_stream(g));
  DM_LAUNCH(k_recount, dim3((unsigned)g->NT), dim3(256), 0, g->stream, ge, g->state,
                     g->tile_free, g->fmask, g->fedge, g->tile_seen);
  DM_HIP(hipGetLastError());
  if (int rc = dm_launch_relist(g, false)) return rc;
  g->fmask_valid = true;
  return DM_OK;
}

int dm_launch_state_from_logodds(dm_grid* g) {
  const int64_t cells = g->R * g->W;
  DM_LAUNCH(k_state_from_l, dim3(grid_for(cells, 256)), dim3(256), 0, g->stream,
                     make_apply(g), cells, g->L, g->state);
  DM_HIP(hipGetLastError());
  return dm_launch_recount(g);
}

int dm_launch_set_state(dm_grid* g, const int8_t* d_in) {
  const int64_t cells = g->R * g->W;
  DM_LAUNCH(k_set_state, dim3(grid_for(cells, 256)), dim3(256), 0, g->stream,
                     make_apply(g), cells, d_in, g->L, g->state);
  DM_HIP(hipGetLastError());
  return dm_launch_recount(g);
}

int dm_launch_map_image(dm_grid* g, uint8_t* d_img) {
  const int64_t cells = g->R * g->W;
  DM_LAUNCH(k_map_image, dim3(grid_for(cells, 256)), dim3(256), 0, g->stream, g->R,
                     g->W, g->state, d_img);
  DM_HIP(hipGetLastError());
  return DM_OK;
}
```

### distributed-autonomous-exploration-and-mapping_amd/csrc/dm_internal.h

```cpp
#pragma once

#include <hip/hip_runtime.h>
#include <stdint.h>

#include <atomic>
#include <chrono>
#include <string>
#include <vector>

#include "../../include/dm.h"

#include "dm_ray.h"


enum {
  CNT_ACTIVE = 0,
  CNT_U = 1,
  CNT_T = 2,
  CNT_SEGS = 3,
  CNT_FTILES = 4,
  CNT_SLOTS = 5,
  CNT_CLUSTERS = 6,
  CNT_OVERFLOW = 7,
  CNT_ITEMS = 8,
  CNT_HEAVY = 9,
  CNT_TH = 10,
  CNT_SORTED = 11,
  CNT_FL0 = 12,
  CNT_STAMP = 13,
  CNT_LITEMS = 14,
  CNT_IOVERFLOW = 15,
  CNT_BIG = 16,
  CNT_SITEMS = 17,
  CNT_N = 18
};
constexpr unsigned long long kOvSlots = 4ull;
constexpr unsigned long long kOvUnionFind = 8ull;
constexpr unsigned long long kOvPipeline = 32ull;
constexpr int kHaltWord = 8;
constexpr int kSigWord = 0;
constexpr int kGateWord = 4;
constexpr int kStampWord = 8;
constexpr int kIntegrateCounters[] = {CNT_ACTIVE, CNT_U, CNT_T, CNT_SEGS, CNT_ITEMS,
                                      CNT_HEAVY, CNT_TH, CNT_LITEMS, CNT_IOVERFLOW, CNT_SITEMS};

constexpr int kIntegrateChunk = 256;
constexpr int kIntegrateMedium = 1024;


constexpr int kShards = 32;
constexpr int kShardWords = 16;
static_assert(kShards * kShardWords == 512, "k_integrate_reset covers 512 shard words");
enum { SH_U = 0, SH_T = 1, SH_TH = 2, SH_ACT = 3 };
enum { SH_SLOT = 0, SH_RUNS = 1, SH_FTF = 2, SH_BIG = 3 };

constexpr int kNStats = 11;
constexpr bool dm_stat_is_frontier(int i) { return i >= 7 && i <= 9; }

constexpr int kRbRecords = 6;
static_assert(kRbRecords * sizeof(dm_cluster) >= (CNT_N + 4) * sizeof(unsigned long long), "readback header");
struct dm_raw_record {
  long long label, size, sum_x, sum_y;
};
constexpr int kRbHostRecords = 6;
static_assert(kRbHostRecords * sizeof(dm_raw_record) >= (CNT_N + 4) * sizeof(unsigned long long),
              "readback header");
__host__ __device__ inline unsigned long long* dm_rb_header(dm_raw_record* records) {
  return reinterpret_cast<unsigned long long*>(records - kRbHostRecords);
}
__host__ __device__ inline const unsigned long long* dm_rb_header(const dm_raw_record* records) {
  return reinterpret_cast<const unsigned long long*>(records - kRbHostRecords);
}
__host__ __device__ inline double dm_centroid(double origin, long long sum, long long size, double res) {
  const double m = (double)sum / (double)size;
  return origin + (m + 0.5) * res;
}

struct dm_grid;
hipError_t dm_copy_shards(dm_grid* g);
inline unsigned long long dm_shard_sum(const unsigned long long* sh, int field) {
  unsigned long long s = 0;
  for (int i = 0; i < kShards; ++i) s += sh[i * kShardWords + field];
  return s;
}

struct KernelTimer {
  std::string name;
  hipEvent_t start, stop;
  hipStream_t stream = nullptr;
};

struct dm_shard_set;

struct dm_grid {
  dm_params p;
  dm_shard_set* sh = nullptr;
  int device = 0;
  int n_cu = 256;
  hipStream_t stream = nullptr;
  bool own_stream = false;
  bool overlap = false;
#ifndef DM_FE_STREAMS
#define DM_FE_STREAMS 1
#endif
  static constexpr int kFeStreams = DM_FE_STREAMS;
  static_assert(kFeStreams == 1 || kFeStreams == 2, "one or two front-end streams");
  hipStream_t fe_streams[2] = {nullptr, nullptr};
  hipEvent_t ev_fe = nullptr;
  hipEvent_t ev_fe_end[2] = {nullptr, nullptr};
  unsigned long long* fe_flag = nullptr;
  bool fault_gate = false;
  hipEvent_t ev_bits[2] = {nullptr, nullptr};
  uint64_t integrate_seq = 0;
  struct RbSlot {
    dm_cluster* out_clu = nullptr;
    dm_raw_record* h_out = nullptr;
    dm_raw_record* h_out_dev = nullptr;
    int64_t h_out_cap = 0;
    dm_cluster* m_out = nullptr;
    hipEvent_t ev = nullptr;
    int kind = 0;
    uint64_t seq = 0;
    uint64_t gen = 0;
    uint64_t pass = 0;
    int64_t merge_n = 0;
    uint64_t wepoch = 0, mepoch = 0;
  };
#ifndef DM_RB_SLOTS
#define DM_RB_SLOTS 2
#endif
  static constexpr int kRbSlots = DM_RB_SLOTS;
  static constexpr int kRbSync = kRbSlots;
  RbSlot rb[kRbSlots + 1];
  int rb_head = 0, rb_count = 0;
  int cur_slot = 0;
  uint64_t rb_gen = 0;
  uint64_t fr_pass = 0, m_pass = 0;
  int64_t W = 0, H = 0, R = 0, row0 = 0;
  int64_t TX = 0, TY = 0, NT = 0;
  int32_t nmax = 0;

  float* L = nullptr;
  int8_t* state = nullptr;
  int32_t* tile_free = nullptr;
  uint8_t* fmask = nullptr;
  uint64_t* fedge = nullptr;
  uint8_t* tile_seen = nullptr;
  bool fmask_on = false, fmask_valid = false;
  int fmask_mode = 0;
  unsigned long long* cnt = nullptr;
  unsigned long long* h_cnt = nullptr;
  unsigned long long* fsh = nullptr;
  unsigned long long* h_sh = nullptr;

  int64_t beams_cap = 0;
  int64_t blk_cap = 0;
  int64_t segs_cap = 0;
  int64_t act_cap = 0;
  int64_t hitem_cap = 0;
  int64_t heavy_cap = 0;
  struct IntWs {
    Beam* beams = nullptr;
    int2* blk_hist = nullptr;
    int32_t* blk_n = nullptr;
    int32_t* act_raw = nullptr;
    PackedPiece* pieces = nullptr;
    int4* hitems = nullptr;
    int4* litems = nullptr;
    int32_t* heavy_list = nullptr;
    uint32_t* slabs = nullptr;
    int32_t* heavy_done = nullptr;
    int32_t* tile_count = nullptr;
    int32_t* tile_cur = nullptr;
    unsigned long long* cnt = nullptr;
    unsigned long long* sh = nullptr;
    double* pose4 = nullptr;
    float* ranges = nullptr;
    int64_t pose_cap = 0, ranges_cap = 0;
    hipEvent_t ev_free = nullptr;
    hipEvent_t free_wait = nullptr;
    bool free_owed = false;
  };
  static constexpr int kIntSets = 2;
  IntWs iw[kIntSets];
  int iw_cur = 0;
  double* trig = nullptr; int32_t trig_n = -1; float trig_amin = 0, trig_inc = 0;
  int64_t trig_cap = 0;
  static constexpr int kPoseRing = 2;
  double* h_pose4[kPoseRing] = {nullptr, nullptr};
  hipEvent_t ev_pose[kPoseRing] = {nullptr, nullptr};
  double* h_pose4_dev[kPoseRing] = {nullptr, nullptr};
#ifndef DM_HOST_POSE
#define DM_HOST_POSE 1
#endif
  int64_t h_pose_cap = 0;
  int pose_head = 0;
  int32_t last_S = 0, last_N = 0;

  struct FrWs {
    unsigned long long* cnt = nullptr;
    unsigned long long* fsh = nullptr;
    int32_t* big_tiles = nullptr;
    uint64_t* fbits = nullptr;
    int32_t* edge_slot = nullptr;
    int32_t* slot_parent = nullptr;
    hipEvent_t busy = nullptr;
    hipEvent_t ev_split = nullptr;
    bool busy_pending = false;
    uint64_t busy_pass = 0;
  };
  FrWs fw[2];
  unsigned long long* fl_n = nullptr;
  hipStream_t pass_stream = nullptr;
  hipStream_t big_stream = nullptr;
  hipEvent_t ev_bigfork = nullptr, ev_big = nullptr;
  unsigned long long* bits_flag = nullptr;
  hipEvent_t p_tail = nullptr;
  bool p_pending = false;
  uint64_t p_tail_pass = 0;
  int32_t* ftiles = nullptr;
  unsigned long long* ftiles_n = nullptr;
  int32_t* flist[2] = {nullptr, nullptr};
  unsigned long long* flist_n[2] = {nullptr, nullptr};
  hipEvent_t flist_ev[2] = {nullptr, nullptr};
  bool flist_ev_set[2] = {false, false};
  int flist_cur = 0;
  int relist_age = 0;
  int relist_period = 1;
  int32_t* big_tiles = nullptr;
  uint64_t* fbits = nullptr;
  int32_t* border = nullptr;
  unsigned long long* rel = nullptr;
  int32_t fparity = 0;
  int64_t border_cap = 0;
  int64_t slot_cap = 0;
  long long* slot_label = nullptr;
  int32_t* slot_parent = nullptr;
  int32_t* slot_root = nullptr;
  long long* slot_own = nullptr;
  long long* slot_acc = nullptr;
  long long* clusters = nullptr;
  int32_t* slot_k = nullptr;
  int32_t* rank_of = nullptr;
  dm_cluster* out_clu = nullptr;
  dm_raw_record* h_out = nullptr;
  dm_raw_record* h_out_dev = nullptr;
  int64_t h_out_cap = 0;
  int32_t* cell_slot = nullptr;
  int32_t* edge_slot = nullptr;
  long long* edge_label = nullptr;
  uint8_t* mask = nullptr;
  long long* labels = nullptr;
  int8_t* halo = nullptr;
  int has_halo[2] = {0, 0};
  bool frontier_valid = false;

  unsigned long long* bs_key = nullptr;
  unsigned long long* bs_key2 = nullptr;
  int32_t* bs_idx = nullptr;
  int32_t* bs_idx2 = nullptr;
  int64_t bs_cap = 0;
  int32_t* rs_cnt = nullptr;
  int32_t* rs_off = nullptr;
  unsigned long long* rs_status = nullptr;
  int64_t rs_rows = 0;
  int64_t sort_hint = 0, msort_hint = 0;
  int64_t ftile_hint = 0;
  int64_t runs_hint = 0, ftf_hint = 0;
  int64_t big_hint = 0;
  int64_t sort_min = 4096;
  int frontier_kernel = 0;
  static constexpr int kAccumGrid = 16384;
  static constexpr int kChunkThreadsPerCu = 512;
  int sparse_pieces = 15;

  int64_t m_cap = 0;
  int32_t* m_parent = nullptr;
  long long* m_label = nullptr;
  long long* m_acc = nullptr;
  long long* m_clu = nullptr;
  dm_cluster* m_out = nullptr;
  unsigned long long* m_cnt = nullptr;
  unsigned long long* h_mcnt = nullptr;
  unsigned long long* h_hint = nullptr;
  unsigned long long* d_hint = nullptr;

  int goal_slot = -1, goal_kind = 0;
  uint64_t goal_epoch = 0, goal_gen = 0;
  int64_t goal_n = 0;
  unsigned long long* goal_k[2] = {nullptr, nullptr};
  uint32_t* goal_i[2] = {nullptr, nullptr};
  int64_t goal_cap = 0;
  double* goal_io = nullptr;
  int64_t* goal_idx = nullptr;

  bool profile = false;
  std::vector<KernelTimer> pending;
  std::vector<dm_kernel_stat> stats;
};

inline void dm_select_slot(dm_grid* g, int slot) {
  const dm_grid::RbSlot& r = g->rb[slot];
  g->cur_slot = slot;
  g->out_clu = r.out_clu;
  g->h_out = r.h_out;
  g->h_out_dev = r.h_out_dev;
  g->h_out_cap = r.h_out_cap;
  g->m_out = r.m_out;
}

inline hipStream_t dm_fe_stream_of(const dm_grid* g, int set) {
  return g->fe_streams[set % dm_grid::kFeStreams];
}
inline unsigned long long* dm_fe_flag_of(const dm_grid* g, int set) {
  return g->fe_flag + 16 * (set % dm_grid::kFeStreams);
}
inline int dm_next_set(const dm_grid* g) { return (g->iw_cur + 1) % dm_grid::kIntSets; }

inline hipError_t dm_mark_ws_free(dm_grid* g, hipEvent_t recorded = nullptr) {
  for (int i = 0; i < dm_grid::kIntSets; ++i) {
    dm_grid::IntWs& w = g->iw[i];
    if (!w.free_owed) continue;
    w.free_owed = false;
    w.free_wait = recorded ? recorded : w.ev_free;
    if (recorded) continue;
    const hipError_t e = hipEventRecord(w.ev_free, g->stream);
    if (e != hipSuccess) return e;
  }
  return hipSuccess;
}

inline void dm_select_fw(dm_grid* g, int s) {
  const dm_grid::FrWs& f = g->fw[s];
  g->cnt = f.cnt;
  g->fsh = f.fsh;
  g->big_tiles = f.big_tiles;
  g->fbits = f.fbits;
  g->edge_slot = f.edge_slot;
  g->slot_parent = f.slot_parent;
}

inline void dm_cpu_relax() {
#if defined(__x86_64__) || defined(__i386__)
  __builtin_ia32_pause();
#elif defined(__aarch64__)
  asm volatile("yield" ::: "memory");
#else
  std::atomic_signal_fence(std::memory_order_seq_cst);
#endif
}

inline hipError_t dm_event_wait(hipEvent_t ev) {
  constexpr long long kSpinNs = 2000000;
  const auto t0 = std::chrono::steady_clock::now();
  for (unsigned it = 0;; ++it) {
    const hipError_t e = hipEventQuery(ev);
    if (e != hipErrorNotReady) return e;
    if ((it & 63u) == 63u &&
        std::chrono::duration_cast<std::chrono::nanoseconds>(std::chrono::steady_clock::now() - t0).count() > kSpinNs)
      return hipEventSynchronize(ev);
    dm_cpu_relax();
  }
}

inline hipError_t dm_join_pass_stream(dm_grid* g) {
  if (!g->p_pending) return hipSuccess;
  g->p_pending = false;
  return hipStreamWaitEvent(g->stream, g->p_tail, 0);
}

inline int32_t dm_integrate_chunks(const dm_grid* g, int64_t nb) {
  const int64_t want = (int64_t)dm_grid::kChunkThreadsPerCu * (int64_t)(g->n_cu > 0 ? g->n_cu : 256);
  if (nb <= 0 || nb >= want) return 1;
  const int64_t by_len = (g->nmax + 1) / 64 > 1 ? (g->nmax + 1) / 64 : 1;
  const int64_t by_fill = (want + nb - 1) / nb;
  return (int32_t)(by_fill < by_len ? by_fill : by_len);
}


int dm_launch_integrate(dm_grid* g, int32_t S, const double* d_pose4, int32_t N,
                        const float* d_ranges, const double* d_trig);
int dm_launch_recount(dm_grid* g);
int dm_launch_relist(dm_grid* g, bool swap);
constexpr int kRelistPasses = 16;
int dm_launch_state_from_logodds(dm_grid* g);
int dm_launch_map_image(dm_grid* g, uint8_t* d_img);
int dm_launch_set_state(dm_grid* g, const int8_t* d_state_in);
int dm_enqueue_frontiers(dm_grid* g, bool want_mask, bool want_labels, bool split = false,
                         hipStream_t* end_stream = nullptr);
int dm_launch_signal(hipStream_t s, unsigned long long* flag);
int dm_launch_gate(hipStream_t s, unsigned long long* flag, unsigned long long* err, unsigned long long err_bit,
                   unsigned long long ticks = 0, unsigned long long fault = 0);
int dm_launch_edge_labels(dm_grid* g);
int dm_frontiers_readback(dm_grid* g, int64_t* n_clusters, int64_t* copied);
int dm_launch_frontiers(dm_grid* g, bool want_mask, bool want_labels, int64_t* n_clusters,
                        int64_t* copied);
int dm_launch_rank_sort(hipStream_t stream, long long* clusters, const long long* sums,
                        const long long* labels, const unsigned long long* d_count,
                        int64_t max_records, double ox, double oy, double res, dm_cluster* out,
                        int32_t* rank_of, unsigned long long* d_sorted, const unsigned long long* cnt,
                        int ncnt, int sorted_idx, const unsigned long long* fsh, dm_raw_record* host_out,
                        int64_t host_cap, int64_t expect);
constexpr int64_t kFmaskOnTiles = 8192;
constexpr int32_t kTileListed = 1 << 30;
constexpr int32_t kTileFreeMask = kTileListed - 1;
constexpr int64_t kSlotsPerTile = 4;
int dm_grow_bucket_sort(dm_grid* g, int64_t n);
int dm_launch_bucket_sort(dm_grid* g, hipStream_t stream, long long* clusters, const long long* sums,
                          const long long* labels, const unsigned long long* d_count,
                          int64_t max_records, int64_t row_base, int64_t rows, dm_cluster* out,
                          int32_t* rank_of, unsigned long long* d_sorted, const unsigned long long* cnt,
                          int ncnt, int sorted_idx, const unsigned long long* fsh, dm_raw_record* host_out,
                          int64_t host_cap);
int64_t dm_export_nbytes(int64_t W, int64_t rec_cap);
int dm_launch_export(dm_grid* g, hipStream_t s, void* d_export, int64_t rec_cap);
int dm_launch_merge(dm_grid* g, hipStream_t s, const void* d_gathered, int32_t nranks, int64_t rec_cap,
                    int64_t min_size);
inline hipStream_t dm_exchange_stream_of(const dm_grid* g) { return g->overlap ? g->pass_stream : g->stream; }
int dm_launch_goal_topk(dm_grid* g, const dm_cluster* d_recs, int64_t K, const double* d_robots, int32_t R,
                        int32_t T, int64_t min_size, double w, double min_dist,
                        const unsigned long long** d_k, const uint32_t** d_i);
int dm_launch_goal_gather(dm_grid* g, const dm_cluster* d_recs, const int64_t* d_idx, int32_t R, double* d_xy);
int dm_launch_ld06(dm_grid* g, int32_t S, const dm_ld06_point* d_pts, const int64_t* d_offsets,
                   int32_t N, int dir, float* d_ranges, float* d_intensities);

int dm_sh_destroy(dm_grid* g);
int dm_sh_reset(dm_grid* g);
int dm_sh_integrate(dm_grid* g, int32_t S, const double* poses, int32_t N, const float* ranges, float amin,
                    float inc, uint64_t* U, uint64_t* T);
int dm_sh_integrate_async(dm_grid* g, int32_t S, const double* poses, int32_t N, const float* ranges,
                          float amin, float inc);
int dm_sh_integrate_device(dm_grid* g, int32_t S, const double* d_pose4, int32_t N, const float* d_ranges,
                           float amin, float inc);
int dm_sh_last_counts(dm_grid* g, uint64_t* U, uint64_t* T);
int dm_sh_last_stats(dm_grid* g, uint64_t* out, int32_t cap, int32_t* n_out);
int dm_sh_get_state(dm_grid* g, int8_t* out);
int dm_sh_get_logodds(dm_grid* g, float* out);
int dm_sh_set_logodds(dm_grid* g, const float* in);
int dm_sh_set_state(dm_grid* g, const int8_t* in);
int dm_sh_frontiers(dm_grid* g, uint8_t* mask, int64_t* labels, dm_cluster* out, int64_t cap, int64_t* n_out);
int dm_sh_frontiers_begin(dm_grid* g);
int dm_sh_frontiers_end(dm_grid* g, dm_cluster* out, int64_t cap, int64_t* n_out);
int dm_sh_frontiers_poll(dm_grid* g, int32_t* ready);
int dm_sh_assign_goals(dm_grid* g, const double* robots_xy, int32_t n_robots, int64_t min_size, double w,
                       double min_distance, int64_t* out_index, double* out_xy);
int dm_sh_set_overlap(dm_grid* g, int32_t on);
int dm_sh_synchronize(dm_grid* g);
int dm_sh_profile_enable(dm_grid* g, int enable);
int dm_sh_profile_read(dm_grid* g, dm_kernel_stat* out, int32_t cap, int32_t* n_out);
int dm_sh_profile_reset(dm_grid* g);
int dm_sh_map_image(dm_grid* g, uint8_t* out);
int dm_sh_ld06_to_scans(dm_grid* g, int32_t S, const dm_ld06_point* points, const int64_t* offsets, int32_t N,
                        int dir, float* ranges, float* intensities);
int dm_sh_ld06_to_scans_device(dm_grid* g, int32_t S, const dm_ld06_point* d_points, const int64_t* d_offsets,
                               int32_t N, int dir, float* d_ranges, float* d_intensities);

int dm_set_error(int code, const char* fmt, ...);
int dm_hip_check(hipError_t e, const char* what);
void dm_timer_begin(dm_grid* g, const char* name, KernelTimer* t, hipStream_t s = nullptr);
void dm_timer_end(dm_grid* g, KernelTimer* t);

#define DM_HIP(call)                                         \
  do {                                                       \
    hipError_t _e = (call);                                  \
    if (_e != hipSuccess) return dm_hip_check(_e, #call);    \
  } while (0)

#define DM_LAUNCH(kernel, grid, block, shmem, stream, ...) \
  hipLaunchKernelGGL(kernel, grid, block, shmem, stream, __VA_ARGS__)

inline int64_t dm_quantize_up(int64_t n) {
  if (n <= 8) return n;
  int sh = 0;
  while ((n >> sh) >= 8) ++sh;
  const int64_t step = (int64_t)1 << sh;
  return ((n + step - 1) / step) * step;
}
```

### distributed-autonomous-exploration-and-mapping_amd/csrc/dm_sharded.cpp

```cpp
#include <string.h>

#include <algorithm>
#include <new>
#include <numeric>
#include <vector>

#include "dm_internal.h"

namespace {

constexpr int kSets = 2;

struct Staging {
  double* poses = nullptr;
  float* ranges = nullptr;
  int64_t pose_cap = 0, ranges_cap = 0;
};

int64_t ceil_div(int64_t a, int64_t b) { return (a + b - 1) / b; }

template <class T>
int dev_alloc_on(int dev, T** p, int64_t count, const char* what) {
  (void)hipSetDevice(dev);
  if (*p) { (void)hipFree(*p); *p = nullptr; }
// ... 311 lines not shown
    st.poses = nullptr;
    st.pose_cap = 0;
    DM_HIP(hipHostMalloc((void**)&st.poses, sizeof(double) * 3 * (size_t)std::max(S, 1), hipHostMallocDefault));
    st.pose_cap = (int64_t)std::max(S, 1) * 3;
  }
  if ((int64_t)S * N > st.ranges_cap) {
    if (st.ranges) (void)hipHostFree(st.ranges);
    st.ranges = nullptr;
    st.ranges_cap = 0;
    const int64_t n = std::max<int64_t>((int64_t)S * N, 1);
    DM_HIP(hipHostMalloc((void**)&st.ranges, sizeof(float) * (size_t)n, hipHostMallocDefault));
    st.ranges_cap = n;
  }
  const double reach = (double)p.range_max + 2.0 * p.resolution;
  const double ylo = p.origin_y + (double)s->row0[(size_t)r] * p.resolution - reach;
  const double yhi = p.origin_y + (double)(s->row0[(size_t)r] + s->rows[(size_t)r]) * p.resolution + reach;
  int32_t k = 0;
  for (int32_t i = 0; i < S; ++i) {
    const double y = poses[3 * i + 1];
    if (y < ylo || y > yhi) continue;
    memcpy(st.poses + 3 * (size_t)k, poses + 3 * (size_t)i, 3 * sizeof(double));
    memcpy(st.ranges + (size_t)k * (size_t)N, ranges + (size_t)i * (size_t)N, sizeof(float) * (size_t)N);
    ++k;
  }
  *S_out = k;
  return DM_OK;
}

}

int dm_sh_integrate_async(dm_grid* g, int32_t S, const double* poses, int32_t N, const float* ranges,
                          float amin, float inc) {
  dm_shard_set* s = g->sh;
  if (S < 0 || N < 0) return dm_set_error(DM_ERR_SHAPE, "S and N must be >= 0");
  if ((int64_t)S * N > 0 && (!poses || !ranges)) return dm_set_error(DM_ERR_INVALID_ARG, "poses/ranges is NULL");
  int rc = 0;
  for (int r = 0; r < s->P; ++r) {
    int32_t k = 0;
    if ((rc = sh_stage(s, g->p, r, S, poses, N, ranges, &k))) return rc;
    s->active[(size_t)r] = k > 0;
    if (!k) continue;
    int& head = s->stage_head[(size_t)r];
    const Staging& st = s->stage[head][(size_t)r];
    if ((rc = dm_integrate_async(s->band[(size_t)r], k, st.poses, N, st.ranges, amin, inc))) return rc;
    head = (head + 1) % 3;
  }
  return DM_OK;
}

int dm_sh_last_counts(dm_grid* g, uint64_t* U, uint64_t* T) {
  dm_shard_set* s = g->sh;
  uint64_t su = 0, st = 0;
  for (int r = 0; r < s->P; ++r) {
    if (!s->active[(size_t)r]) continue;
    uint64_t u = 0, t = 0;
    if (int rc = dm_last_counts(s->band[(size_t)r], &u, &t)) return rc;
    su += u;
    st += t;
  }
  if (U) *U = su;
  if (T) *T = st;
  return DM_OK;
}

int dm_sh_integrate(dm_grid* g, int32_t S, const double* poses, int32_t N, const float* ranges, float amin,
                    float inc, uint64_t* U, uint64_t* T) {
  if (int rc = dm_sh_integrate_async(g, S, poses, N, ranges, amin, inc)) return rc;
  return dm_sh_last_counts(g, U, T);
}

int dm_sh_integrate_device(dm_grid* g, int32_t S, const double* d_pose4, int32_t N, const float* d_ranges,
                           float amin, float inc) {
  dm_shard_set* s = g->sh;
  if (S < 0 || N < 0) return dm_set_error(DM_ERR_SHAPE, "S and N must be >= 0");
  const int64_t nb = (int64_t)S * N;
  if (nb > 0 && (!d_pose4 || !d_ranges)) return dm_set_error(DM_ERR_INVALID_ARG, "poses/ranges is NULL");
  int src = s->dev[0];
  if (nb > 0) {
    hipPointerAttribute_t a;
    DM_HIP(hipPointerGetAttributes(&a, d_ranges));
    src = a.device;
  }
  const bool wait_in = s->in_pending;
  s->in_pending = false;
  for (int r = 0; r < s->P; ++r) {
    dm_grid* b = s->band[(size_t)r];
    const int d = s->dev[(size_t)r];
    const double* pp = d_pose4;
    const float* rp = d_ranges;
    hipStream_t fs = b->overlap ? dm_fe_stream_of(b, dm_next_set(b)) : b->stream;
    DM_HIP(hipSetDevice(d));
    if (wait_in) DM_HIP(hipStreamWaitEvent(fs, s->ev_in, 0));
    if (nb > 0 && d != src) {
      if ((int64_t)S * 4 > s->d_pose_cap[(size_t)r] || nb > s->d_ranges_cap[(size_t)r]) {
        if (int rc = dm_synchronize(b)) return rc;
      }
      if ((int64_t)S * 4 > s->d_pose_cap[(size_t)r]) {
        if (int rc = dev_alloc_on(d, &s->d_pose[(size_t)r], (int64_t)S * 4, "sharded poses")) return rc;
        s->d_pose_cap[(size_t)r] = (int64_t)S * 4;
      }
      if (nb > s->d_ranges_cap[(size_t)r]) {
        if (int rc = dev_alloc_on(d, &s->d_ranges[(size_t)r], nb, "sharded ranges")) return rc;
        s->d_ranges_cap[(size_t)r] = nb;
      }
      if (dm_grid::kFeStreams > 1 && b->overlap) DM_HIP(hipStreamWaitEvent(fs, b->ev_fe_end[b->iw_cur % 2], 0));
      DM_HIP(hipMemcpyPeerAsync(s->d_pose[(size_t)r], d, d_pose4, src, sizeof(double) * 4 * (size_t)S, fs));
      DM_HIP(hipMemcpyPeerAsync(s->d_ranges[(size_t)r], d, d_ranges, src, sizeof(float) * (size_t)nb, fs));
      pp = s->d_pose[(size_t)r];
      rp = s->d_ranges[(size_t)r];
    }
    if (int rc = dm_integrate_device(b, S, pp, N, rp, amin, inc)) return rc;
    s->active[(size_t)r] = 1;
  }
  return DM_OK;
}


int dm_sh_get_state(dm_grid* g, int8_t* out) {
  dm_shard_set* s = g->sh;
  for (int r = 0; r < s->P; ++r)
    if (int rc = dm_get_state(s->band[(size_t)r], out + s->row0[(size_t)r] * s->W)) return rc;
  return DM_OK;
}

int dm_sh_get_logodds(dm_grid* g, float* out) {
  dm_shard_set* s = g->sh;
  for (int r = 0; r < s->P; ++r)
    if (int rc = dm_get_logodds(s->band[(size_t)r], out + s->row0[(size_t)r] * s->W)) return rc;
  return DM_OK;
}

int dm_sh_set_logodds(dm_grid* g, const float* in) {
  dm_shard_set* s = g->sh;
  for (int r = 0; r < s->P; ++r)
    if (int rc = dm_set_logodds(s->band[(size_t)r], in + s->row0[(size_t)r] * s->W)) return rc;
  return DM_OK;
}

int dm_sh_set_state(dm_grid* g, const int8_t* in) {
  dm_shard_set* s = g->sh;
  for (int r = 0; r < s->P; ++r)
    if (int rc = dm_set_state(s->band[(size_t)r], in + s->row0[(size_t)r] * s->W)) return rc;
  return DM_OK;
}

int dm_sh_map_image(dm_grid* g, uint8_t* out) {
  dm_shard_set* s = g->sh;
  for (int r = 0; r < s->P; ++r)
    if (int rc = dm_map_image(s->band[(size_t)r], out + (s->H - s->row0[(size_t)r] - s->rows[(size_t)r]) * s->W))
      return rc;
  return DM_OK;
}

int dm_sh_reset(dm_grid* g) {
  dm_shard_set* s = g->sh;
  for (int r = 0; r < s->P; ++r)
    if (int rc = dm_reset(s->band[(size_t)r])) return rc;
  return DM_OK;
}

int dm_sh_synchronize(dm_grid* g) { return sh_sync(g->sh); }

int dm_sh_set_overlap(dm_grid* g, int32_t on) {
  dm_shard_set* s = g->sh;
  for (int r = 0; r < s->P; ++r)
    if (int rc = dm_set_overlap(s->band[(size_t)r], on)) return rc;
  return DM_OK;
}

int dm_sh_last_stats(dm_grid* g, uint64_t* out, int32_t cap, int32_t* n_out) {
  dm_shard_set* s = g->sh;
  if (cap > 0 && !out) return dm_set_error(DM_ERR_INVALID_ARG, "out is NULL");
  uint64_t sum[kNStats] = {0};
  for (int r = 0; r < s->P; ++r) {
    uint64_t v[kNStats] = {0};
    int32_t n = 0;
    if (int rc = dm_last_stats(s->band[(size_t)r], v, kNStats, &n)) return rc;
    for (int i = 0; i < kNStats; ++i)
      if (s->active[(size_t)r] || dm_stat_is_frontier(i)) sum[i] += v[i];
  }
  for (int32_t i = 0; i < cap && i < kNStats; ++i) out[i] = sum[i];
  if (n_out) *n_out = kNStats;
  return DM_OK;
}

int dm_sh_profile_enable(dm_grid* g, int enable) {
  dm_shard_set* s = g->sh;
  for (int r = 0; r < s->P; ++r)
    if (int rc = dm_profile_enable(s->band[(size_t)r], enable)) return rc;
  return DM_OK;
}

int dm_sh_profile_read(dm_grid* g, dm_kernel_stat* out, int32_t cap, int32_t* n_out) {
  dm_shard_set* s = g->sh;
  std::vector<dm_kernel_stat> all;
  for (int r = 0; r < s->P; ++r) {
    int32_t n = 0;
    if (int rc = dm_profile_read(s->band[(size_t)r], nullptr, 0, &n)) return rc;
    std::vector<dm_kernel_stat> v((size_t)std::max(n, 1));
    if (int rc = dm_profile_read(s->band[(size_t)r], v.data(), n, &n)) return rc;
    for (int32_t i = 0; i < n; ++i) {
      auto it = std::find_if(all.begin(), all.end(),
                             [&](const dm_kernel_stat& e) { return !strcmp(e.name, v[(size_t)i].name); });
      if (it == all.end()) {
        all.push_back(v[(size_t)i]);
      } else {
        it->launches += v[(size_t)i].launches;
        it->total_ms += v[(size_t)i].total_ms;
      }
    }
  }
  for (int32_t i = 0; i < cap && i < (int32_t)all.size(); ++i) out[i] = all[(size_t)i];
  if (n_out) *n_out = (int32_t)all.size();
  return DM_OK;
}

int dm_sh_profile_reset(dm_grid* g) {
  dm_shard_set* s = g->sh;
  for (int r = 0; r < s->P; ++r)
    if (int rc = dm_profile_reset(s->band[(size_t)r])) return rc;
  return DM_OK;
}


namespace {

int sh_labels(dm_shard_set* s, uint8_t* mask, int64_t* labels) {
  const int P = s->P;
  const int64_t W = s->W;
  HostMerge hm;
  hm.labels.resize((size_t)P);
  hm.base.resize((size_t)P);
  int64_t total = 0;
  for (int r = 0; r < P; ++r) {
    const int64_t off = s->row0[(size_t)r] * W;
    std::vector<dm_cluster> c(4096);
    int64_t n = 0;
    int rc = 0;
    while (true) {
      rc = dm_frontiers(s->band[(size_t)r], mask ? mask + off : nullptr, labels ? labels + off : nullptr, c.data(),
                        (int64_t)c.size(), &n);
      if (rc != DM_ERR_CAPACITY) break;
      c.resize((size_t)n);
    }
    if (rc) return rc;
    if (!labels) continue;
    hm.base[(size_t)r] = total;
    auto& v = hm.labels[(size_t)r];
    v.resize((size_t)n);
    for (int64_t i = 0; i < n; ++i) v[(size_t)i] = c[(size_t)i].label;
    total += n;
  }
  if (!labels) return DM_OK;
  hm.parent.resize((size_t)total);
  hm.final_label.resize((size_t)total);
  for (int r = 0; r < P; ++r)
    for (size_t i = 0; i < hm.labels[(size_t)r].size(); ++i) {
      const int64_t e = hm.base[(size_t)r] + (int64_t)i;
      hm.parent[(size_t)e] = e;
      hm.final_label[(size_t)e] = hm.labels[(size_t)r][i];
    }
  for (int r = 0; r + 1 < P; ++r) {
    const int64_t* last = labels + (s->row0[(size_t)r] + s->rows[(size_t)r] - 1) * W;
    const int64_t* first = labels + s->row0[(size_t)r + 1] * W;
    for (int64_t x = 0; x < W; ++x) {
      if (last[x] < 0) continue;
      const int64_t a = hm.elem(r, last[x]);
      for (int64_t d = -1; d <= 1; ++d) {
        const int64_t y = x + d;
        if (y < 0 || y >= W || first[y] < 0) continue;
        const int64_t b = hm.elem(r + 1, first[y]);
        if (a >= 0 && b >= 0) hm.unite(a, b);
      }
    }
  }
  for (int r = 0; r < P; ++r) {
    int64_t* lab = labels + s->row0[(size_t)r] * W;
    const int64_t cells = s->rows[(size_t)r] * W;
    for (int64_t i = 0; i < cells; ++i) {
      if (lab[i] < 0) continue;
      const int64_t e = hm.elem(r, lab[i]);
      if (e >= 0) lab[i] = hm.final_label[(size_t)hm.find(e)];
    }
  }
  return DM_OK;
}

}

int dm_sh_frontiers(dm_grid* g, uint8_t* mask, int64_t* labels, dm_cluster* out, int64_t cap, int64_t* n_out) {
  dm_shard_set* s = g->sh;
  if (cap < 0 || (cap > 0 && !out)) return dm_set_error(DM_ERR_INVALID_ARG, "bad cluster buffer");
  int rc = 0;
  int k = s->set;
  for (int attempt = 0;; ++attempt) {
    const bool synced = s->pending > 0;
    if (synced && (rc = sh_sync(s))) return rc;
    if ((rc = sh_refresh_bands(s, synced))) return rc;
    k = s->set;
    if ((rc = sh_enqueue_exchange(s, k))) return rc;
    DM_HIP(hipSetDevice(s->dev[0]));
    int64_t n = 0;
    rc = dm_merge_bands(s->band[0], s->gathered[k], s->P, s->rec_cap, s->min_size, out, cap, &n);
    if (n_out) *n_out = n;
    if (rc != DM_ERR_INCOMPLETE) break;
    if (attempt == 4) return dm_set_error(DM_ERR_INCOMPLETE, "band exports stayed incomplete after growing");
// ... 81 lines not shown
```

### distributed-autonomous-exploration-and-mapping_amd/dm/_ffi.py

```python
from __future__ import annotations

import ctypes
import os
import threading

_HERE = os.path.dirname(os.path.abspath(__file__))
LIB_PATH = os.environ.get("DM_LIB", os.path.join(_HERE, "libdm.so"))

DM_OK = 0
DM_ERR_INVALID_ARG = -1
DM_ERR_SHAPE = -2
DM_ERR_HIP = -3
DM_ERR_OOM = -4
DM_ERR_CAPACITY = -5
DM_ERR_IO = -6
DM_ERR_STATE = -7
DM_ERR_INCOMPLETE = -8
DM_ERR_PIPELINE = -9
DM_ERR_COLLECTIVE = -10
DM_TILE = 64

_ERR_NAMES = {
    DM_ERR_INVALID_ARG: "DM_ERR_INVALID_ARG",
    DM_ERR_SHAPE: "DM_ERR_SHAPE",
    DM_ERR_HIP: "DM_ERR_HIP",
    DM_ERR_OOM: "DM_ERR_OOM",
    DM_ERR_CAPACITY: "DM_ERR_CAPACITY",
    DM_ERR_IO: "DM_ERR_IO",
    DM_ERR_STATE: "DM_ERR_STATE",
    DM_ERR_INCOMPLETE: "DM_ERR_INCOMPLETE",
    DM_ERR_PIPELINE: "DM_ERR_PIPELINE",
    DM_ERR_COLLECTIVE: "DM_ERR_COLLECTIVE",
}


class DmError(RuntimeError):

    def __init__(self, code: int, message: str):
        self.code = code
        super().__init__(f"{_ERR_NAMES.get(code, code)}: {message}")


class DmParams(ctypes.Structure):

    _fields_ = [
        ("width", ctypes.c_int64),
        ("height", ctypes.c_int64),
        ("resolution", ctypes.c_double),
        ("origin_x", ctypes.c_double),
        ("origin_y", ctypes.c_double),
        ("range_min", ctypes.c_float),
        ("range_max", ctypes.c_float),
        ("l_occ", ctypes.c_float),
        ("l_free", ctypes.c_float),
        ("l_min", ctypes.c_float),
        ("l_max", ctypes.c_float),
        ("occ_thresh", ctypes.c_float),
        ("free_thresh", ctypes.c_float),
        ("min_frontier_size", ctypes.c_int64),
        ("band_row0", ctypes.c_int64),
        ("band_rows", ctypes.c_int64),
    ]

    def as_dict(self) -> dict:
        return {name: getattr(self, name) for name, _ in self._fields_}


class DmCluster(ctypes.Structure):

    _fields_ = [
        ("label", ctypes.c_int64),
        ("size", ctypes.c_int64),
        ("sum_x", ctypes.c_int64),
        ("sum_y", ctypes.c_int64),
        ("cx_m", ctypes.c_double),
        ("cy_m", ctypes.c_double),
    ]


class DmLd06Point(ctypes.Structure):

    _fields_ = [
        ("angle_deg", ctypes.c_float),
        ("distance_mm", ctypes.c_uint16),
        ("intensity", ctypes.c_uint8),
        ("pad", ctypes.c_uint8),
    ]


LD06_POINT_DTYPE = [("angle_deg", "<f4"), ("distance_mm", "<u2"), ("intensity", "u1"), ("pad", "u1")]


class DmKernelStat(ctypes.Structure):
    _fields_ = [
        ("name", ctypes.c_char * 32),
        ("launches", ctypes.c_uint64),
        ("total_ms", ctypes.c_double),
    ]


CLUSTER_DTYPE = [
    ("label", "<i8"),
    ("size", "<i8"),
    ("sum_x", "<i8"),
    ("sum_y", "<i8"),
    ("cx_m", "<f8"),
    ("cy_m", "<f8"),
]

_vp = ctypes.c_void_p
_i32 = ctypes.c_int32
_i64 = ctypes.c_int64
_f32 = ctypes.c_float

SIGNATURES = {
    "dm_default_params": [ctypes.POINTER(DmParams), _i64, _i64],
    "dm_create": [ctypes.POINTER(_vp), ctypes.POINTER(DmParams), ctypes.c_int],
    "dm_create_sharded": [ctypes.POINTER(_vp), ctypes.POINTER(DmParams), _i32, ctypes.POINTER(_i32)],
    "dm_sharded_band_rows": [_i64, _i32, _i32, ctypes.POINTER(_i64), ctypes.POINTER(_i64)],
    "dm_sharded_info": [_vp, ctypes.POINTER(_i32), ctypes.POINTER(_i64)],
    "dm_destroy": [_vp],
    "dm_reset": [_vp],
    "dm_get_params": [_vp, ctypes.POINTER(DmParams)],
    "dm_integrate": [_vp, _i32, _vp, _i32, _vp, _f32, _f32, _vp, _vp],
    "dm_integrate_device": [_vp, _i32, _vp, _i32, _vp, _f32, _f32],
    "dm_integrate_async": [_vp, _i32, _vp, _i32, _vp, _f32, _f32],
    "dm_last_counts": [_vp, _vp, _vp],
    "dm_last_stats": [_vp, _vp, _i32, ctypes.POINTER(_i32)],
    "dm_get_state": [_vp, _vp],
    "dm_get_logodds": [_vp, _vp],
    "dm_set_logodds": [_vp, _vp],
    "dm_set_state": [_vp, _vp],
    "dm_frontiers": [_vp, _vp, _vp, _vp, _i64, ctypes.POINTER(_i64)],
    "dm_set_halo": [_vp, _vp, _vp],
    "dm_set_halo_device": [_vp, _vp, _vp],
    "dm_get_edge_rows": [_vp, _vp, _vp],
    "dm_get_edge_rows_device": [_vp, _vp, _vp],
    "dm_get_edge_labels": [_vp, _vp, _vp],
    "dm_save": [_vp, ctypes.c_char_p],
    "dm_load": [_vp, ctypes.c_char_p],
    "dm_set_stream": [_vp, _vp],
    "dm_exchange_stream": [_vp, ctypes.POINTER(ctypes.c_void_p)],
    "dm_synchronize": [_vp],
    "dm_profile_enable": [_vp, ctypes.c_int],
    "dm_profile_read": [_vp, ctypes.POINTER(DmKernelStat), _i32, ctypes.POINTER(_i32)],
    "dm_profile_reset": [_vp],
    "dm_map_image": [_vp, _vp],
    "dm_ld06_to_scans": [_vp, _i32, _vp, _vp, _i32, ctypes.c_int, _vp, _vp],
    "dm_ld06_to_scans_device": [_vp, _i32, _vp, _vp, _i32, ctypes.c_int, _vp, _vp],
    "dm_export_bytes": [_vp, _i64, ctypes.POINTER(_i64)],
    "dm_frontiers_export_device": [_vp, _vp, _i64],
    "dm_merge_bands": [_vp, _vp, _i32, _i64, _i64, _vp, _i64, ctypes.POINTER(_i64)],
    "dm_merge_bands_begin": [_vp, _vp, _i32, _i64, _i64],
    "dm_merge_bands_end": [_vp, _vp, _i64, ctypes.POINTER(_i64)],
    "dm_merge_max_band_k": [_vp, ctypes.POINTER(_i64)],
    "dm_frontiers_begin": [_vp],
    "dm_max_passes_in_flight": [],
    "dm_frontiers_end": [_vp, _vp, _i64, ctypes.POINTER(_i64)],
    "dm_frontiers_poll": [_vp, ctypes.POINTER(_i32)],
    "dm_set_overlap": [_vp, _i32],
    "dm_atomic_peak": [ctypes.c_int, _vp, _i32, ctypes.POINTER(_i32)],
    "dm_assign_goals": [_vp, _vp, _i32, ctypes.c_int64, ctypes.c_double, ctypes.c_double, _vp, _vp],
}
STRING_FUNCS = ("dm_last_error", "dm_version")

_lib = None
_lib_lock = threading.Lock()


def load_library(path: str | None = None) -> ctypes.CDLL:
    global _lib
    with _lib_lock:
        if _lib is not None:
            return _lib
        p = path or LIB_PATH
        if not os.path.exists(p):
            raise DmError(
                DM_ERR_STATE,
                f"libdm.so not found at {p}; build it with "
                "`make -C distributed-autonomous-exploration-and-mapping_amd/csrc` "
                "(or __graft_entry__.build())",
            )
        lib = ctypes.CDLL(p, mode=ctypes.RTLD_GLOBAL)
        for name, argtypes in SIGNATURES.items():
            fn = getattr(lib, name)
            fn.argtypes = argtypes
            fn.restype = ctypes.c_int
        for name in STRING_FUNCS:
            fn = getattr(lib, name)
            fn.argtypes = []
            fn.restype = ctypes.c_char_p
        _lib = lib
        return lib


def last_error() -> str:
    v = load_library().dm_last_error()
    return v.decode() if isinstance(v, bytes) else str(v)


def check(rc: int) -> int:
    if rc < 0:
        msg = load_library().dm_last_error()
        raise DmError(rc, msg.decode() if msg else "")
    return rc


def exported_symbols() -> list[str]:
    return list(SIGNATURES) + list(STRING_FUNCS)
```

### distributed-autonomous-exploration-and-mapping_amd/dm/grid.py

```python
from __future__ import annotations

import ctypes
import threading
from dataclasses import dataclass

import numpy as np

from . import _ffi
from ._ffi import CLUSTER_DTYPE, DmError, DmParams, check, load_library


def default_params(width: int, height: int, **overrides) -> DmParams:
    lib = load_library()
    p = DmParams()
    check(lib.dm_default_params(ctypes.byref(p), int(width), int(height)))
    res_given = "resolution" in overrides
    for k, v in overrides.items():
        if not hasattr(p, k):
            raise DmError(_ffi.DM_ERR_INVALID_ARG, f"unknown parameter {k!r}")
        setattr(p, k, v)
    if res_given and "origin_x" not in overrides:
        p.origin_x = -0.5 * p.width * p.resolution
    if res_given and "origin_y" not in overrides:
        p.origin_y = -0.5 * p.height * p.resolution
# ... 23 lines not shown
    labels: np.ndarray | None = None

    def __len__(self) -> int:
        return int(self.clusters.shape[0])


def _vp(a: np.ndarray | None):
    return None if a is None else a.ctypes.data_as(ctypes.c_void_p)


class OccupancyMapper:

    def __init__(self, params: DmParams, device: int = 0, devices=None):
        self._lib = load_library()
        self._lock = threading.RLock()
        self._h = ctypes.c_void_p()
        if devices is not None:
            devs = (ctypes.c_int32 * len(devices))(*[int(d) for d in devices])
            check(self._lib.dm_create_sharded(ctypes.byref(self._h), ctypes.byref(params), len(devices), devs))
            device = int(devices[0])
        else:
            check(self._lib.dm_create(ctypes.byref(self._h), ctypes.byref(params), int(device)))
        self.devices = list(devices) if devices is not None else [int(device)]
        out = DmParams()
        check(self._lib.dm_get_params(self._h, ctypes.byref(out)))
        self.params = out
        self.device = device
        self.width = int(out.width)
        self.rows = int(out.band_rows)
        self.row0 = int(out.band_row0)
        self._cap = 1 << 12
        self.last_incomplete = None

    def close(self):
        with self._lock:
            if self._h:
                self._lib.dm_destroy(self._h)
                self._h = ctypes.c_void_p()

    def __del__(self):
        try:
            self.close()
        except Exception:
            pass

    def __enter__(self):
        return self

    def __exit__(self, *exc):
        self.close()

    def _handle(self):
        if not self._h:
            raise DmError(_ffi.DM_ERR_STATE, "mapper is closed")
        return self._h

    def integrate(self, poses, ranges, angle_min, angle_increment):
        poses = np.ascontiguousarray(poses, dtype=np.float64).reshape(-1, 3)
        ranges = np.ascontiguousarray(ranges, dtype=np.float32)
        if ranges.ndim != 2:
            ranges = ranges.reshape(poses.shape[0], -1)
        S, N = ranges.shape
        U = ctypes.c_uint64(0)
        T = ctypes.c_uint64(0)
        with self._lock:
            check(self._lib.dm_integrate(self._handle(), S, _vp(poses), N, _vp(ranges),
                                         float(angle_min), float(angle_increment),
                                         ctypes.byref(U), ctypes.byref(T)))
        return int(U.value), int(T.value)

    def integrate_scan(self, scan, pose):
        ranges = np.asarray(scan.ranges, dtype=np.float32)[None, :]
        return self.integrate(np.asarray(pose, np.float64)[None, :], ranges,
                              np.float32(scan.angle_min), np.float32(scan.angle_increment))

    def integrate_async(self, poses, ranges_ptr: int, S: int, N: int, angle_min, angle_increment):
        poses = np.ascontiguousarray(poses, dtype=np.float64).reshape(-1, 3)
        if poses.shape[0] != S:
            raise DmError(_ffi.DM_ERR_SHAPE, f"poses has {poses.shape[0]} rows, S = {S}")
        with self._lock:
            check(self._lib.dm_integrate_async(self._handle(), int(S), _vp(poses), int(N),
                                               ctypes.c_void_p(ranges_ptr), float(angle_min),
                                               float(angle_increment)))

    def integrate_device(self, d_pose4_ptr: int, S: int, d_ranges_ptr: int, N: int,
                         angle_min, angle_increment):
        with self._lock:
            check(self._lib.dm_integrate_device(self._handle(), int(S), ctypes.c_void_p(d_pose4_ptr),
                                                int(N), ctypes.c_void_p(d_ranges_ptr),
                                                float(angle_min), float(angle_increment)))

    def last_counts(self):
        U = ctypes.c_uint64(0)
        T = ctypes.c_uint64(0)
        with self._lock:
            check(self._lib.dm_last_counts(self._handle(), ctypes.byref(U), ctypes.byref(T)))
        return int(U.value), int(T.value)

    STAT_NAMES = ("updates", "touched", "touched_heavy", "pieces", "active_tiles", "work_items",
                  "heavy_tiles", "frontier_tiles", "frontier_slots", "frontier_clusters", "sparse_items")

    def last_stats(self) -> dict:
        k = len(self.STAT_NAMES)
        out = (ctypes.c_uint64 * k)()
        n = ctypes.c_int32(0)
        with self._lock:
            check(self._lib.dm_last_stats(self._handle(), out, k, ctypes.byref(n)))
        return {k: int(out[i]) for i, k in enumerate(self.STAT_NAMES)}

    def ld06_to_scans(self, points, offsets, n_beams: int, laser_scan_dir: bool = True,
                      want_intensities: bool = False):
        pts = np.ascontiguousarray(points, dtype=np.dtype(_ffi.LD06_POINT_DTYPE))
        off = np.ascontiguousarray(offsets, dtype=np.int64)
        S = off.shape[0] - 1
        ranges = np.empty((S, n_beams), np.float32)
        inten = np.empty((S, n_beams), np.float32) if want_intensities else None
        with self._lock:
            check(self._lib.dm_ld06_to_scans(self._handle(), S, _vp(pts), _vp(off), int(n_beams),
                                             1 if laser_scan_dir else 0, _vp(ranges), _vp(inten)))
        return (ranges, inten) if want_intensities else ranges

    def state(self) -> np.ndarray:
        out = np.empty((self.rows, self.width), np.int8)
        with self._lock:
            check(self._lib.dm_get_state(self._handle(), _vp(out)))
        return out

    def logodds(self) -> np.ndarray:
        out = np.empty((self.rows, self.width), np.float32)
        with self._lock:
            check(self._lib.dm_get_logodds(self._handle(), _vp(out)))
        return out

    def set_logodds(self, L):
        L = np.ascontiguousarray(L, dtype=np.float32).reshape(self.rows, self.width)
        with self._lock:
            check(self._lib.dm_set_logodds(self._handle(), _vp(L)))

    def set_state(self, st):
        st = np.ascontiguousarray(st, dtype=np.int8).reshape(self.rows, self.width)
        with self._lock:
            check(self._lib.dm_set_state(self._handle(), _vp(st)))

    def reset(self):
        with self._lock:
            check(self._lib.dm_reset(self._handle()))

    def map_image(self) -> np.ndarray:
        out = np.empty((self.rows, self.width), np.uint8)
        with self._lock:
            check(self._lib.dm_map_image(self._handle(), _vp(out)))
        return out

    def assign_goals(self, robots_xy, min_size: int = 8, distance_weight: float = 1.0,
                     min_distance: float = 0.0):
        xy = np.ascontiguousarray(np.asarray(robots_xy, np.float64).reshape(-1, 2))
        R = xy.shape[0]
        idx = np.empty(R, np.int64)
        out = np.empty((R, 2), np.float64)
        with self._lock:
            check(self._lib.dm_assign_goals(self._handle(), _vp(xy), R, int(min_size), float(distance_weight),
                                            float(min_distance), _vp(idx), _vp(out)))
        return [(int(i), (float(p[0]), float(p[1]))) if i >= 0 else None for i, p in zip(idx, out)]

    def frontiers(self, want_mask=False, want_labels=False, cap=None) -> Frontiers:
        mask = np.empty((self.rows, self.width), np.uint8) if want_mask else None
        labels = np.empty((self.rows, self.width), np.int64) if want_labels else None
        n = ctypes.c_int64(0)
        with self._lock:
            if cap is not None and self._cap < cap:
                self._cap = max(1, int(cap))
            while True:
                buf = np.empty(self._cap, dtype=np.dtype(CLUSTER_DTYPE))
                rc = self._lib.dm_frontiers(self._handle(), _vp(mask), _vp(labels), _vp(buf),
                                            buf.shape[0], ctypes.byref(n))
                if rc == _ffi.DM_ERR_CAPACITY and n.value > buf.shape[0]:
                    self._cap = int(n.value) * 2
                    continue
                check(rc)
                break
            clusters = buf[: int(n.value)]
        return Frontiers(clusters=clusters, mask=mask, labels=labels)

    def frontiers_begin(self):
        with self._lock:
            check(self._lib.dm_frontiers_begin(self._handle()))

    def frontiers_ready(self) -> bool:
        r = ctypes.c_int32(0)
        with self._lock:
            check(self._lib.dm_frontiers_poll(self._handle(), ctypes.byref(r)))
        return bool(r.value)

    def frontiers_end(self) -> Frontiers | None:
        n = ctypes.c_int64(0)
        with self._lock:
            while True:
                buf = np.empty(self._cap, dtype=np.dtype(CLUSTER_DTYPE))
                rc = self._lib.dm_frontiers_end(self._handle(), _vp(buf), buf.shape[0], ctypes.byref(n))
                if rc == _ffi.DM_ERR_CAPACITY and n.value > buf.shape[0]:
                    self._cap = int(n.value) * 2
                    continue
                if rc == _ffi.DM_ERR_INCOMPLETE:
                    self.last_incomplete = _ffi.last_error()
                    return None
                check(rc)
                return Frontiers(clusters=buf[: int(n.value)])

    def set_overlap(self, on: bool = True):
        with self._lock:
            check(self._lib.dm_set_overlap(self._handle(), 1 if on else 0))

    def set_halo(self, before=None, after=None):
        b = None if before is None else np.ascontiguousarray(before, np.int8)
        a = None if after is None else np.ascontiguousarray(after, np.int8)
        with self._lock:
            check(self._lib.dm_set_halo(self._handle(), _vp(b), _vp(a)))

    def set_halo_device(self, before_ptr: int | None, after_ptr: int | None):
        with self._lock:
            check(self._lib.dm_set_halo_device(self._handle(),
                                               None if before_ptr is None else ctypes.c_void_p(before_ptr),
                                               None if after_ptr is None else ctypes.c_void_p(after_ptr)))

    def edge_rows(self):
        first = np.empty(self.width, np.int8)
        last = np.empty(self.width, np.int8)
        with self._lock:
            check(self._lib.dm_get_edge_rows(self._handle(), _vp(first), _vp(last)))
        return first, last

    def edge_rows_device(self, first_ptr: int, last_ptr: int):
        with self._lock:
            check(self._lib.dm_get_edge_rows_device(self._handle(), ctypes.c_void_p(first_ptr),
                                                    ctypes.c_void_p(last_ptr)))

    def edge_labels(self):
        first = np.empty(self.width, np.int64)
        last = np.empty(self.width, np.int64)
        with self._lock:
            check(self._lib.dm_get_edge_labels(self._handle(), _vp(first), _vp(last)))
        return first, last

    def export_bytes(self, rec_cap: int) -> int:
        n = ctypes.c_int64(0)
        check(self._lib.dm_export_bytes(self._handle(), int(rec_cap), ctypes.byref(n)))
        return int(n.value)

    def frontiers_export_device(self, d_export_ptr: int, rec_cap: int):
        with self._lock:
            check(self._lib.dm_frontiers_export_device(self._handle(), ctypes.c_void_p(d_export_ptr),
                                                       int(rec_cap)))

    def exchange_stream(self) -> int:
        s = ctypes.c_void_p(0)
        with self._lock:
            check(self._lib.dm_exchange_stream(self._handle(), ctypes.byref(s)))
        return int(s.value or 0)

    def merge_bands(self, d_gathered_ptr: int, nranks: int, rec_cap: int, min_size: int):
        n = ctypes.c_int64(0)
        with self._lock:
            while True:
                buf = self._mbuf if getattr(self, "_mbuf", None) is not None else \
                    np.empty(1 << 14, dtype=np.dtype(CLUSTER_DTYPE))
                rc = self._lib.dm_merge_bands(self._handle(), ctypes.c_void_p(d_gathered_ptr), int(nranks),
                                              int(rec_cap), int(min_size), _vp(buf), buf.shape[0],
                                              ctypes.byref(n))
                self._mbuf = buf
                if rc == _ffi.DM_ERR_INCOMPLETE:
                    self.last_incomplete = _ffi.last_error()
                    return None, int(n.value)
                if rc == _ffi.DM_ERR_CAPACITY and n.value > buf.shape[0]:
                    self._mbuf = np.empty(int(n.value) * 2, dtype=np.dtype(CLUSTER_DTYPE))
                    continue
                check(rc)
                return buf[: int(n.value)].copy(), None

    def merge_max_band_k(self) -> int:
        k = ctypes.c_int64(0)
        with self._lock:
            check(self._lib.dm_merge_max_band_k(self._handle(), ctypes.byref(k)))
        return int(k.value)

    def merge_bands_begin(self, d_gathered_ptr: int, nranks: int, rec_cap: int, min_size: int):
        with self._lock:
            check(self._lib.dm_merge_bands_begin(self._handle(), ctypes.c_void_p(d_gathered_ptr), int(nranks),
                                                 int(rec_cap), int(min_size)))

    def merge_bands_end(self):
        n = ctypes.c_int64(0)
        with self._lock:
            while True:
                buf = self._mbuf if getattr(self, "_mbuf", None) is not None else \
                    np.empty(1 << 14, dtype=np.dtype(CLUSTER_DTYPE))
                rc = self._lib.dm_merge_bands_end(self._handle(), _vp(buf), buf.shape[0], ctypes.byref(n))
                self._mbuf = buf
                if rc == _ffi.DM_ERR_INCOMPLETE:
                    self.last_incomplete = _ffi.last_error()
                    return None, int(n.value)
                if rc == _ffi.DM_ERR_CAPACITY and n.value > buf.shape[0]:
                    self._mbuf = np.empty(int(n.value) * 2, dtype=np.dtype(CLUSTER_DTYPE))
                    continue
                check(rc)
                return buf[: int(n.value)].copy(), None

# ... 34 lines not shown
```

### include/dm.h

```cpp
#ifndef DM_H
#define DM_H

#include <stddef.h>
#include <stdint.h>

#ifdef __cplusplus
extern "C" {
#endif

#define DM_OK 0
#define DM_ERR_INVALID_ARG (-1)
#define DM_ERR_SHAPE (-2)
#define DM_ERR_HIP (-3)
#define DM_ERR_OOM (-4)
#define DM_ERR_CAPACITY (-5)
#define DM_ERR_IO (-6)
#define DM_ERR_STATE (-7)
#define DM_ERR_INCOMPLETE (-8)
#define DM_ERR_PIPELINE (-9)
#define DM_ERR_COLLECTIVE (-10)

#define DM_TILE 64

typedef struct dm_params {
  int64_t width;
  int64_t height;
  double resolution;
  double origin_x;
  double origin_y;
  float range_min;
  float range_max;
  float l_occ;
  float l_free;
  float l_min;
  float l_max;
  float occ_thresh;
  float free_thresh;
  int64_t min_frontier_size;
  int64_t band_row0;
  int64_t band_rows;
} dm_params;

typedef struct dm_cluster {
  int64_t label;
  int64_t size;
  int64_t sum_x;
  int64_t sum_y;
  double cx_m;
  double cy_m;
} dm_cluster;

typedef struct dm_kernel_stat {
  char name[32];
  uint64_t launches;
  double total_ms;
} dm_kernel_stat;

typedef struct dm_grid dm_grid;

int dm_default_params(dm_params* p, int64_t width, int64_t height);

int dm_create(dm_grid** out, const dm_params* p, int device);
int dm_destroy(dm_grid* g);
int dm_reset(dm_grid* g);
int dm_get_params(const dm_grid* g, dm_params* out);

int dm_integrate(dm_grid* g, int32_t S, const double* poses, int32_t N,
                 const float* ranges, float angle_min, float angle_increment,
                 uint64_t* out_updates, uint64_t* out_touched);

int dm_integrate_async(dm_grid* g, int32_t S, const double* poses, int32_t N,
                       const float* ranges, float angle_min, float angle_increment);

int dm_integrate_device(dm_grid* g, int32_t S, const double* d_pose4,
                        int32_t N, const float* d_ranges, float angle_min,
                        float angle_increment);
int dm_last_counts(dm_grid* g, uint64_t* updates, uint64_t* touched);

int dm_last_stats(dm_grid* g, uint64_t* out, int32_t cap, int32_t* n_out);

int dm_get_state(dm_grid* g, int8_t* out);
int dm_get_logodds(dm_grid* g, float* out);
int dm_set_logodds(dm_grid* g, const float* in);
int dm_set_state(dm_grid* g, const int8_t* in);

int dm_frontiers(dm_grid* g, uint8_t* mask, int64_t* labels, dm_cluster* out,
                 int64_t cap, int64_t* n_out);

int dm_frontiers_begin(dm_grid* g);
int dm_frontiers_end(dm_grid* g, dm_cluster* out, int64_t cap, int64_t* n_out);
int dm_frontiers_poll(dm_grid* g, int32_t* ready);
int dm_max_passes_in_flight(void);

int dm_set_overlap(dm_grid* g, int32_t on);


int dm_create_sharded(dm_grid** out, const dm_params* p, int32_t nranks, const int32_t* devices);
int dm_sharded_band_rows(int64_t height, int32_t nranks, int32_t rank, int64_t* row0, int64_t* rows);
int dm_sharded_info(const dm_grid* g, int32_t* nranks, int64_t* rec_cap);

int dm_set_halo(dm_grid* g, const int8_t* row_before, const int8_t* row_after);
int dm_set_halo_device(dm_grid* g, const int8_t* d_row_before,
                       const int8_t* d_row_after);
int dm_get_edge_rows(dm_grid* g, int8_t* first_row, int8_t* last_row);
int dm_get_edge_rows_device(dm_grid* g, int8_t* d_first_row, int8_t* d_last_row);
int dm_get_edge_labels(dm_grid* g, int64_t* first_row, int64_t* last_row);

int dm_export_bytes(const dm_grid* g, int64_t rec_cap, int64_t* bytes);
int dm_frontiers_export_device(dm_grid* g, void* d_export, int64_t rec_cap);
int dm_exchange_stream(dm_grid* g, void** stream);
int dm_merge_bands(dm_grid* g, const void* d_gathered, int32_t nranks, int64_t rec_cap,
                   int64_t min_size, dm_cluster* out, int64_t cap, int64_t* n_out);
int dm_merge_bands_begin(dm_grid* g, const void* d_gathered, int32_t nranks, int64_t rec_cap,
                         int64_t min_size);
int dm_merge_bands_end(dm_grid* g, dm_cluster* out, int64_t cap, int64_t* n_out);
int dm_merge_max_band_k(const dm_grid* g, int64_t* max_k);

typedef struct dm_ld06_point {
  float angle_deg;
  uint16_t distance_mm;
  uint8_t intensity;
  uint8_t pad;
} dm_ld06_point;

int dm_ld06_to_scans(dm_grid* g, int32_t S, const dm_ld06_point* points,
                     const int64_t* offsets, int32_t N, int laser_scan_dir,
                     float* ranges_out, float* intensities_out);
int dm_ld06_to_scans_device(dm_grid* g, int32_t S, const dm_ld06_point* d_points,
                            const int64_t* d_offsets, int32_t N, int laser_scan_dir,
                            float* d_ranges_out, float* d_intensities_out);

int dm_save(dm_grid* g, const char* path);
int dm_load(dm_grid* g, const char* path);

int dm_set_stream(dm_grid* g, void* stream);
int dm_synchronize(dm_grid* g);
int dm_profile_enable(dm_grid* g, int enable);
int dm_profile_read(dm_grid* g, dm_kernel_stat* out, int32_t cap, int32_t* n_out);
int dm_profile_reset(dm_grid* g);

int dm_map_image(dm_grid* g, uint8_t* out);

int dm_assign_goals(dm_grid* g, const double* robots_xy, int32_t n_robots, int64_t min_size,
                    double distance_weight, double min_distance, int64_t* out_index, double* out_xy);

int dm_atomic_peak(int device, double* out, int32_t cap, int32_t* n_out);

const char* dm_last_error(void);
const char* dm_version(void);

#ifdef __cplusplus
}
#endif
#endif
```

Measured before the change: 213.1 billion.

## Fuse frontier bit-record maintenance into tile accumulation kernel

Removes the separate k_fmask_items pass and the adaptive fmask on/off heuristic. The tile accumulation kernel now emits per-tile frontier nibble records and edge words straight from the updated state registers, with a re-read fallback for heavy or non-vector tiles. The accumulate kernel is also templated on vec_ok so the scalar path is compiled out. This saves a second pass over touched cells, at the cost of extra LDS atomics and record stores in the hot integrate kernel, which now always run. A debug checker entry point is added.

```diff
diff --git a/distributed-autonomous-exploration-and-mapping_amd/csrc/dm_api.cpp b/distributed-autonomous-exploration-and-mapping_amd/csrc/dm_api.cpp
--- a/distributed-autonomous-exploration-and-mapping_amd/csrc/dm_api.cpp
+++ b/distributed-autonomous-exploration-and-mapping_amd/csrc/dm_api.cpp
@@ -1478,4 +1478,23 @@
   return rc;
 }
 
-}
+int dm_check_bit_records(dm_grid* g, int64_t* mismatches) {
+  if (g && g->sh) return (mismatches ? dm_sh_check_bit_records(g, mismatches)
+                                     : dm_set_error(DM_ERR_INVALID_ARG, "mismatches is NULL"));
+  int rc = check_grid(g);
+  if (rc || (rc = use_device(g))) return rc;
+  if (!mismatches) return dm_set_error(DM_ERR_INVALID_ARG, "mismatches is NULL");
+  unsigned long long* d = nullptr;
+  if ((rc = dev_alloc(&d, 1, "record mismatches"))) return rc;
+  unsigned long long n = 0;
+  hipError_t e = hipMemsetAsync(d, 0, sizeof n, g->stream);
+  if (e == hipSuccess) rc = dm_launch_check_records(g, d);
+  if (!rc && e == hipSuccess) e = hipMemcpyAsync(&n, d, sizeof n, hipMemcpyDeviceToHost, g->stream);
+  if (!rc && e == hipSuccess) e = hipStreamSynchronize(g->stream);
+  (void)hipFree(d);
+  if (e != hipSuccess) return dm_hip_check(e, "dm_check_bit_records");
+  *mismatches = (int64_t)n;
+  return rc;
+}
+
+}
diff --git a/distributed-autonomous-exploration-and-mapping_amd/csrc/dm_frontier.hip b/distributed-autonomous-exploration-and-mapping_amd/csrc/dm_frontier.hip
--- a/distributed-autonomous-exploration-and-mapping_amd/csrc/dm_frontier.hip
+++ b/distributed-autonomous-exploration-and-mapping_amd/csrc/dm_frontier.hip
@@ -1494,16 +1494,7 @@
   const int64_t want_waves = g->ftile_hint > 0 ? dm_quantize_up(g->ftile_hint + g->ftile_hint / 4 + 64) : g->NT;
   const int wave_grid = grid_for(std::min<int64_t>(want_waves, g->NT), kFW, 8192);
   const int bits_grid = std::max(wave_grid, 64);
-  const bool want_on = g->fmask_mode == 1 || (g->fmask_mode == 0 && g->ftile_hint >= kFmaskOnTiles);
-  const bool want_off = g->fmask_mode == 2 || (g->fmask_mode == 0 && g->ftile_hint < kFmaskOnTiles / 4);
-  if (!g->fmask_on && want_on) {
-    if (!g->fmask_valid) {
-      if (int rc = dm_launch_recount(g)) return rc;
-    }
-    g->fmask_on = true;
-  } else if (g->fmask_on && want_off) {
-    g->fmask_on = false;
-  }
+  const int use_fmask = g->fmask_mode == 2 ? 0 : 1;
   const bool dense = g->frontier_kernel == 2 ||
                      (g->frontier_kernel == 0 && g->ftf_hint > 0 && g->runs_hint > kDenseRuns * g->ftf_hint &&
                       g->ftf_hint <= kDenseMaxTiles);
@@ -1513,7 +1504,7 @@
   auto* const wave_kernel = edge ? k_frontier_tile<true> : k_frontier_tile<false>;
   dm_timer_begin(g, "frontier_bits", &t);
   DM_LAUNCH(k_frontier_bits, dim3(bits_grid), dim3(kFW * 64), 0, g->stream, fg, g->state, g->halo, g->fmask,
-            g->fedge, g->tile_seen, g->ftiles, g->ftiles_n, list_n, g->fbits, g->cnt, g->fmask_on ? 1 : 0,
+            g->fedge, g->tile_seen, g->ftiles, g->ftiles_n, list_n, g->fbits, g->cnt, use_fmask,
             dense ? nullptr : g->big_tiles, g->fsh, g->edge_slot, 2 * g->W, g->slot_parent, g->fe_flag + kHaltWord,
             g->bits_flag + kStampWord);
   dm_timer_end(g, &t);
diff --git a/distributed-autonomous-exploration-and-mapping_amd/csrc/dm_integrate.hip b/distributed-autonomous-exploration-and-mapping_amd/csrc/dm_integrate.hip
--- a/distributed-autonomous-exploration-and-mapping_amd/csrc/dm_integrate.hip
+++ b/distributed-autonomous-exploration-and-mapping_amd/csrc/dm_integrate.hip
@@ -2,6 +2,7 @@
 #include "dm_phase.h"
 
 #include <algorithm>
+#include <type_traits>
 
 DM_PH_DECL(integrate)
 DM_TL_DECL(accum)
@@ -366,54 +367,103 @@
   return (uint8_t)(zb(w) | (zb(~w) << 4));
 }
 
-template <class G>
-__device__ inline uint8_t state_nibbles_at(const G& g, const int8_t* __restrict__ state, int32_t x0, int32_t y) {
-  uint32_t fn = 0u, un = 0u;
-  for (int e = 0; e < 4; ++e) {
-    if (x0 + e >= g.r.W) break;
-    const int8_t b = state[(int64_t)y * g.r.W + x0 + e];
-    fn |= (b == 0 ? 1u : 0u) << e;
-    un |= (b == -1 ? 1u : 0u) << e;
-  }
-  return (uint8_t)(fn | (un << 4));
-}
-
-__device__ inline uint32_t every4th(uint64_t x) {
-  x &= 0x1111111111111111ull;
-  x = (x | (x >> 3)) & 0x0303030303030303ull;
-  x = (x | (x >> 6)) & 0x000F000F000F000Full;
-  x = (x | (x >> 12)) & 0x000000FF000000FFull;
-  return (uint32_t)((x | (x >> 24)) & 0xFFFFull);
-}
-
-struct EdgeAcc {
-  uint64_t w[4] = {0ull, 0ull, 0ull, 0ull};
+__device__ inline uint8_t fmask_byte(uint64_t fm, uint64_t um, int j) {
+  return (uint8_t)(((fm >> (4 * j)) & 0xFull) | (((um >> (4 * j)) & 0xFull) << 4));
+}
+
+__device__ inline void edge_row(uint64_t (&ew)[4], uint64_t um, int r) {
+  ew[0] |= (um & 1ull) << r;
+  ew[1] |= (um >> 63) << r;
+  if (r == 0) ew[2] = um;
+  if (r == DM_TS - 1) ew[3] = um;
+}
+
+template <class G, class Byte, class Sink>
+__device__ inline void tile_record_rows(const G& g, const int8_t* __restrict__ state, int64_t tile, int r0, int dr,
+                                        uint64_t (&ew)[4], Byte&& byte, Sink&& sink) {
+  const int32_t tx0 = (int32_t)(tile % g.r.TX) * DM_TS, ty0 = (int32_t)(tile / g.r.TX) * DM_TS;
+  const int lane = (int)__lane_id();
+  constexpr int kB = 8;
+  const int32_t x = tx0 + lane;
+  for (int rb = r0; rb < DM_TS; rb += kB * dr) {
+    int8_t b[kB];
+#pragma unroll
+    for (int j = 0; j < kB; ++j) {
+      const int r = rb + j * dr;
+      const bool in = r < DM_TS && x < g.r.W && ty0 + r < g.r.R;
+      b[j] = in ? state[(int64_t)(ty0 + r) * g.r.W + x] : (int8_t)1;
+    }
+#pragma unroll
+    for (int j = 0; j < kB; ++j) {
+      const int r = rb + j * dr;
+      if (r >= DM_TS) break;
+      const bool in = x < g.r.W && ty0 + r < g.r.R;
+      const uint64_t fm = __ballot(b[j] == 0);
+      const uint64_t um = __ballot(b[j] == -1);
+      if (lane < 16) byte(r, fmask_byte(fm, um, lane));
+      edge_row(ew, um, r);
+      sink(r, b[j], in);
+    }
+  }
+}
+
+__device__ inline void edge_or_words(uint32_t* s_edge, const uint64_t (&ew)[4]) {
+#pragma unroll
+  for (int k = 0; k < 4; ++k) {
+    if ((uint32_t)ew[k]) atomicOr(&s_edge[2 * k], (uint32_t)ew[k]);
+    if ((uint32_t)(ew[k] >> 32)) atomicOr(&s_edge[2 * k + 1], (uint32_t)(ew[k] >> 32));
+  }
+}
+
+struct DenseRec {
+  static constexpr bool on = true, all = true;
+  uint8_t* rec;
+  uint32_t* s_edge;
+  uint32_t tid;
+  __device__ void dense(uint32_t pk) const {
+    uint32_t t = tid;
+    asm volatile("" : "+v"(t));
+    uint8_t* r = rec + t;
+#pragma unroll
+    for (int rr = 0; rr < 4; ++rr) r[256 * rr] = (uint8_t)(pk >> (8 * rr));
+    const uint32_t un = pk & 0xF0F0F0F0u;
+    if (un == 0u) return;
+    const uint32_t grp = t & 15u, ly0 = t >> 4;
+    if (grp == 0u || grp == 15u) {
+      const uint32_t c = un >> (grp == 0u ? 4 : 7);
+      const uint32_t lo = ((c & 1u) | ((c >> 8) & 1u) << 16) << ly0;
+      const uint32_t hi = (((c >> 16) & 1u) | ((c >> 24) & 1u) << 16) << ly0;
+      uint32_t* w = s_edge + (grp == 0u ? 0 : 2);
+      if (lo) atomicOr(w, lo);
+      if (hi) atomicOr(w + 1, hi);
+    }
+    if (ly0 == 0u && (un & 0xF0u)) atomicOr(&s_edge[4 + (grp >> 3)], ((un >> 4) & 0xFu) << (4 * (grp & 7u)));
+    if (ly0 == 15u && (un >> 28)) atomicOr(&s_edge[6 + (grp >> 3)], (un >> 28) << (4 * (grp & 7u)));
+  }
+  __device__ void operator()(int, int, uint32_t) const {}
 };
-__device__ inline void edge_acc(EdgeAcc& e, uint32_t out, int q, int lane) {
-  const int c = lane & 3;
-  const uint64_t b0 = __ballot(c == 0 && ((out >> 4) & 1u));
-  const uint64_t b3 = __ballot(c == 3 && ((out >> 31) & 1u));
-  e.w[0] |= (uint64_t)every4th(b0) << (16 * q);
-  e.w[1] |= (uint64_t)every4th(b3 >> 3) << (16 * q);
-  if (q == 0 || q == 3) {
-    const uint32_t u16 = ((out >> 4) & 0xFu) | ((out >> 8) & 0xF0u) | ((out >> 12) & 0xF00u) | ((out >> 16) & 0xF000u);
-    const int base = q == 0 ? 0 : 60;
-    uint64_t r = 0ull;
-#pragma unroll
-    for (int k = 0; k < 4; ++k) r |= (uint64_t)__shfl(u16, base + k) << (16 * k);
-    e.w[q == 0 ? 2 : 3] = r;
-  }
-}
-
-__device__ inline void edge_store(const EdgeAcc& e, uint64_t* __restrict__ fedge, int64_t tile, uint64_t rows,
-                                  int lane) {
-  if (lane >= 4) return;
-  const uint64_t v = lane == 0 ? e.w[0] : lane == 1 ? e.w[1] : lane == 2 ? e.w[2] : e.w[3];
-  const uint64_t m = lane < 2 ? rows : ((rows >> (lane == 2 ? 0 : 63)) & 1ull) ? ~0ull : 0ull;
-  uint64_t* p = fedge + tile * 4 + lane;
-  if (m == ~0ull) *p = v;
-  else if (m) *p = (*p & ~m) | (v & m);
-}
+struct SparseRec {
+  static constexpr bool on = true, all = false;
+  uint8_t* rec;
+  uint32_t* s_mv;
+  __device__ void operator()(int ly, int grp, uint32_t v) const {
+    rec[ly * 16 + grp] = (uint8_t)v;
+    const uint32_t un = v >> 4;
+    if (grp == 0) {
+      atomicOr(&s_mv[0 + (ly >> 5)], 1u << (ly & 31));
+      if (un & 1u) atomicOr(&s_mv[8 + (ly >> 5)], 1u << (ly & 31));
+    }
+    if (grp == 15) {
+      atomicOr(&s_mv[2 + (ly >> 5)], 1u << (ly & 31));
+      if (un & 8u) atomicOr(&s_mv[10 + (ly >> 5)], 1u << (ly & 31));
+    }
+    if (ly == 0 || ly == DM_TS - 1) {
+      const int k = ly == 0 ? 4 : 6;
+      atomicOr(&s_mv[k + (grp >> 3)], 0xFu << (4 * (grp & 7)));
+      if (un) atomicOr(&s_mv[8 + k + (grp >> 3)], un << (4 * (grp & 7)));
+    }
+  }
+};
 
 __device__ inline int32_t zero_bytes(uint32_t x) {
   uint32_t t = (x & 0x7F7F7F7Fu) + 0x7F7F7F7Fu;
@@ -421,7 +471,7 @@
   return __popc(t);
 }
 
-template <int ROWS>
+template <int ROWS, bool VOK>
 struct CellRows {
   float4 l[ROWS];
   char4 s[ROWS];
@@ -457,12 +507,15 @@
     }
   }
 
-  template <class Counts>
+  template <class Counts, class Rec>
   __device__ void apply(const Geom& g, const ApplyArgs& p, int32_t tx0, int32_t ty0, int ly0, int dly,
                         int cx, float* __restrict__ L, int8_t* __restrict__ state, Counts&& counts,
-                        int32_t* sh_T, int32_t* sh_free, uint32_t* sh_U) {
+                        int32_t* sh_T, int32_t* sh_free, uint32_t* sh_U, Rec&& rec) {
+    using RecT = typename std::remove_reference<Rec>::type;
     int32_t dT = 0, dFree = 0;
     uint32_t dU = 0;
+    [[maybe_unused]] uint32_t pk = 0u;
+    static_assert(!RecT::all || ROWS == 4, "DenseRec: four row groups per thread");
 #pragma unroll
     for (int rr = 0; rr < ROWS; ++rr) {
       const int ly = ly0 + rr * dly;
@@ -470,7 +523,10 @@
       if (y >= g.r.R) continue;
       uint32_t h4[4], m4[4];
       counts(ly, h4, m4);
-      if (((h4[0] | m4[0]) | (h4[1] | m4[1]) | (h4[2] | m4[2]) | (h4[3] | m4[3])) == 0u) continue;
+      if (((h4[0] | m4[0]) | (h4[1] | m4[1]) | (h4[2] | m4[2]) | (h4[3] | m4[3])) == 0u) {
+        if (RecT::all && vec) pk |= (uint32_t)state_nibbles(*reinterpret_cast<const uint32_t*>(&s[rr])) << (8 * rr);
+        continue;
+      }
       const int64_t base = (int64_t)y * g.r.W + tx0 + cx;
       if (sh_U) {
 #pragma unroll
@@ -495,6 +551,8 @@
             make_float4(__uint_as_float(nlb[0]), __uint_as_float(nlb[1]), __uint_as_float(nlb[2]),
                         __uint_as_float(nlb[3]));
         *reinterpret_cast<uint32_t*>(state + base) = ns;
+        if (RecT::all) pk |= (uint32_t)state_nibbles(ns) << (8 * rr);
+        else if (RecT::on) rec(ly, cx >> 2, (uint32_t)state_nibbles(ns));
       } else if (vec) {
         float lv[4] = {l[rr].x, l[rr].y, l[rr].z, l[rr].w};
         int8_t sv[4] = {(int8_t)s[rr].x, (int8_t)s[rr].y, (int8_t)s[rr].z, (int8_t)s[rr].w};
@@ -512,7 +570,9 @@
                  zero_bytes(*reinterpret_cast<const uint32_t*>(&s[rr]));
         *reinterpret_cast<float4*>(L + base) = make_float4(lv[0], lv[1], lv[2], lv[3]);
         *reinterpret_cast<char4*>(state + base) = ns4;
-      } else {
+        if (RecT::all) pk |= (uint32_t)state_nibbles(*reinterpret_cast<const uint32_t*>(&ns4)) << (8 * rr);
+        else if (RecT::on) rec(ly, cx >> 2, (uint32_t)state_nibbles(*reinterpret_cast<const uint32_t*>(&ns4)));
+      } else if constexpr (!VOK) {
         for (int e = 0; e < 4; ++e) {
           if ((h4[e] | m4[e]) == 0u || tx0 + cx + e >= g.r.W) continue;
           const int64_t i = base + e;
@@ -529,6 +589,7 @@
     if (dT) atomicAdd(sh_T, dT);
     if (dFree) atomicAdd(sh_free, dFree);
     if (dU) atomicAdd(sh_U, dU);
+    if constexpr (RecT::all) rec.dense(pk);
   }
 };
 
@@ -706,16 +767,19 @@
 #define DM_EARLY_PIECES 1
 #endif
 constexpr int kAccumPerCu = DM_ACCUM_OCC;
+template <bool VOK>
 __global__ __launch_bounds__(kQuarter, kAccumPerCu) void k_tile_accum(
     Geom g, ApplyArgs p, const int4* __restrict__ list_a, int cnt_a, const int4* __restrict__ list_b,
     int cnt_b, int cnt_c, const PackedPiece* __restrict__ pieces, int32_t* tile_count, int32_t* tile_free,
     uint32_t* __restrict__ slabs, float* __restrict__ L, int8_t* __restrict__ state,
-    const unsigned long long* __restrict__ cnt, unsigned long long* ish, int vec_ok,
+    const unsigned long long* __restrict__ cnt, unsigned long long* ish, int ,
     const int32_t* __restrict__ heavy_list, int32_t* heavy_done, int32_t* tlist, unsigned long long* tlist_n,
-    unsigned long long* hint, const unsigned long long* __restrict__ halt, uint8_t* __restrict__ tile_seen) {
+    unsigned long long* hint, const unsigned long long* __restrict__ halt, uint8_t* __restrict__ tile_seen,
+    uint8_t* __restrict__ fmask, uint64_t* __restrict__ fedge) {
   __shared__ uint32_t tl[kTileWords + 64];
   __shared__ int32_t s_T, s_free, s_last;
   __shared__ uint32_t s_U;
+  __shared__ uint32_t s_edge[8];
   const int tid = threadIdx.x, lane = lane_id();
   DM_TL_BEGIN();
   const unsigned long long hv = *halt;
@@ -731,7 +795,6 @@
   if (blockIdx.x == 0 && tid == 0) {
     volatile unsigned long long* h = hint;
     h[0] = (unsigned long long)(n_items + (SI + 3) / 4);
-    h[1] = (unsigned long long)(n_items + SI);
   }
   const unsigned long long idle =
       ((int64_t)blockIdx.x >= n_items && sp_rank * (kQuarter / 64) >= SI) ? 1ull : 0ull;
@@ -749,7 +812,8 @@
   int4 info = item_of(blockIdx.x);
   int4 next = item_of(blockIdx.x + G);
   PackedPiece mine;
-  CellRows<4> cells;
+  constexpr int vec_ok = VOK ? 1 : 0;
+  CellRows<4, VOK> cells;
   int32_t tfree;
   auto split_of = [&](const int4& d) -> int32_t {
     const int32_t c = __builtin_amdgcn_readfirstlane(d.z);
@@ -768,6 +832,7 @@
   PackedPiece mine_n = mine;
   for (int e = tid; e < kTileWords; e += kQuarter) tl[e] = 0u;
   if (tid == 0) { s_T = 0; s_free = 0; s_U = 0u; s_accT = 0ull; s_accU = 0ull; }
+  if (tid < 8) s_edge[tid] = 0u;
   __syncthreads();
   DM_PH_INIT();
   [[maybe_unused]] unsigned long long tl_word = 0;
@@ -861,10 +926,22 @@
                       m4[e] = v & 0xFFFFu;
                     }
                   },
-                  &s_T, &s_free, inside ? nullptr : &s_U);
+                  &s_T, &s_free, inside ? nullptr : &s_U,
+                  DenseRec{fmask + (int64_t)tile * (DM_TS * 16), s_edge, (uint32_t)tid});
       DM_PH(dm_phase_acc_integrate, 4);
     }
     __syncthreads();
+    const bool rewrite = heavy >= 0 ? s_last != 0 : !vec_ok;
+    if (rewrite) {
+      uint64_t ew[4] = {0ull, 0ull, 0ull, 0ull};
+      uint8_t* rec = fmask + (int64_t)tile * (DM_TS * 16);
+      tile_record_rows(g, state, tile, tid >> 6, kQuarter / 64, ew,
+                       [&](int r, uint8_t v) { rec[r * 16 + lane] = v; }, [](int, int8_t, bool) {});
+      if (lane == 0) edge_or_words(s_edge, ew);
+      __syncthreads();
+    }
+    if (tid < 4 && (heavy < 0 || rewrite))
+      fedge[(int64_t)tile * 4 + tid] = (uint64_t)s_edge[2 * tid] | ((uint64_t)s_edge[2 * tid + 1] << 32);
     if (tid == 0 && heavy < 0) {
       s_accT += (unsigned long long)s_T;
       s_accU += (unsigned long long)s_U;
@@ -877,6 +954,7 @@
     mine = DM_EARLY_PIECES ? mine_n : load_pieces(info);
     for (int e = tid; e < kTileWords; e += kQuarter) tl[e] = 0u;
     if (tid == 0) { s_T = 0; s_free = 0; s_U = 0u; }
+    if (tid < 4) { s_edge[2 * tid] = 0u; s_edge[2 * tid + 1] = 0u; }
     __syncthreads();
   }
   __shared__ int32_t s_wT[kQuarter / 64], s_wfree[kQuarter / 64];
@@ -886,6 +964,8 @@
   uint32_t* tq = tl + wv * (DM_TS * DM_TS / 4);
   const int hcx = (lane & 15) * 4;
   if (lane == 0) { s_wT[wv] = 0; s_wfree[wv] = 0; s_wU[wv] = 0u; }
+  __shared__ uint32_t s_mv[kQuarter / 64][16];
+  if (lane < 16) s_mv[wv][lane] = 0u;
   const int nw = kQuarter / 64;
   for (int64_t it = sp_rank * nw + wv; it < SI; it += (int64_t)G * nw) {
     int4 d = list_b[(int64_t)g.act_cap - 1 - it];
@@ -916,6 +996,7 @@
         m4[e] = v & 0xFu;
       }
     };
+    const SparseRec srec{fmask + (int64_t)tile * (DM_TS * 16), s_mv[wv]};
     uint16_t* lst = s_list[wv];
     int nt = 0;
     {
@@ -936,27 +1017,27 @@
       for (int e0 = 0; e0 < nt; e0 += 128) {
         const int ea = e0 + lane, eb = e0 + 64 + lane;
         const int wa = ea < nt ? lst[ea] : 0, wb = eb < nt ? lst[eb] : 0;
-        CellRows<1> ca, cb;
+        CellRows<1, VOK> ca, cb;
         ca.load_touched(g, tx0, ty0, wa >> 4, 0, (wa & 15) * 4, L, state, vec_ok, [&](int) { return ea < nt; });
         cb.load_touched(g, tx0, ty0, wb >> 4, 0, (wb & 15) * 4, L, state, vec_ok, [&](int) { return eb < nt; });
         if (ea < nt)
           ca.apply(g, p, tx0, ty0, wa >> 4, 0, (wa & 15) * 4, L, state,
                    [&](int, uint32_t* h4, uint32_t* m4) { counts(wa, h4, m4); }, &s_wT[wv], &s_wfree[wv],
-                   inside ? nullptr : &s_wU[wv]);
+                   inside ? nullptr : &s_wU[wv], srec);
         if (eb < nt)
           cb.apply(g, p, tx0, ty0, wb >> 4, 0, (wb & 15) * 4, L, state,
                    [&](int, uint32_t* h4, uint32_t* m4) { counts(wb, h4, m4); }, &s_wT[wv], &s_wfree[wv],
-                   inside ? nullptr : &s_wU[wv]);
+                   inside ? nullptr : &s_wU[wv], srec);
       }
     } else {
       for (int pass = 0; pass < 4; ++pass) {
         const int ly0 = (lane >> 4) + 16 * pass;
-        CellRows<4> sc;
+        CellRows<4, VOK> sc;
         sc.load_touched(g, tx0, ty0, ly0, 4, hcx, L, state, vec_ok,
                         [&](int ly) { return tq[ly * 16 + (hcx >> 2)] != 0u; });
         sc.apply(g, p, tx0, ty0, ly0, 4, hcx, L, state,
                  [&](int ly, uint32_t* h4, uint32_t* m4) { counts(ly * 16 + (hcx >> 2), h4, m4); },
-                 &s_wT[wv], &s_wfree[wv], inside ? nullptr : &s_wU[wv]);
+                 &s_wT[wv], &s_wfree[wv], inside ? nullptr : &s_wU[wv], srec);
       }
     }
     DM_PH(dm_phase_acc_integrate, 7);
@@ -964,6 +1045,22 @@
     DM_PH_COUNT(dm_phase_acc_integrate, 22, c);
     __builtin_amdgcn_fence(__ATOMIC_ACQ_REL, "wavefront");
     __builtin_amdgcn_wave_barrier();
+    if (!vec_ok) {
+      __builtin_amdgcn_fence(__ATOMIC_ACQ_REL, "workgroup");
+      uint64_t ew[4] = {0ull, 0ull, 0ull, 0ull};
+      tile_record_rows(g, state, tile, 0, 1, ew, [&](int r, uint8_t v) { srec.rec[r * 16 + lane] = v; },
+                       [](int, int8_t, bool) {});
+      if (lane < 4) fedge[(int64_t)tile * 4 + lane] = lane == 0 ? ew[0] : lane == 1 ? ew[1] : lane == 2 ? ew[2] : ew[3];
+    } else if (lane < 4) {
+      const uint64_t m = (uint64_t)s_mv[wv][2 * lane] | ((uint64_t)s_mv[wv][2 * lane + 1] << 32);
+      const uint64_t v = (uint64_t)s_mv[wv][8 + 2 * lane] | ((uint64_t)s_mv[wv][8 + 2 * lane + 1] << 32);
+      if (m) {
+        uint64_t* pe = fedge + (int64_t)tile * 4 + lane;
+        *pe = (*pe & ~m) | v;
+        s_mv[wv][2 * lane] = 0u; s_mv[wv][2 * lane + 1] = 0u;
+        s_mv[wv][8 + 2 * lane] = 0u; s_mv[wv][8 + 2 * lane + 1] = 0u;
+      }
+    }
     if (lane == 0) {
       const int32_t T = s_wT[wv], df = s_wfree[wv];
       const uint32_t U = s_wU[wv] + wU;
@@ -1022,15 +1119,10 @@
   }
 }
 
-__device__ inline uint8_t fmask_byte(uint64_t fm, uint64_t um, int j) {
-  return (uint8_t)(((fm >> (4 * j)) & 0xFull) | (((um >> (4 * j)) & 0xFull) << 4));
-}
-
 __global__ __launch_bounds__(256) void k_recount(Geom g, const int8_t* __restrict__ state,
                                                  int32_t* __restrict__ tile_free, uint8_t* __restrict__ fmask,
                                                  uint64_t* __restrict__ fedge, uint8_t* __restrict__ tile_seen) {
   const int64_t tile = blockIdx.x;
-  const int32_t tx0 = (int32_t)(tile % g.r.TX) * DM_TS, ty0 = (int32_t)(tile / g.r.TX) * DM_TS;
   __shared__ int32_t acc, seen;
   __shared__ uint64_t s_edge[4][4];
   if (threadIdx.x == 0) { acc = 0; seen = 0; }
@@ -1038,23 +1130,14 @@
   int32_t c = 0, known = 0;
   uint64_t ew[4] = {0ull, 0ull, 0ull, 0ull};
   uint8_t* tm = fmask + tile * (DM_TS * 16);
-  for (int e = threadIdx.x; e < DM_TS * DM_TS; e += 256) {
-    const int32_t x = tx0 + (e & 63), y = ty0 + (e >> 6);
-    const int8_t b = (x < g.r.W && y < g.r.R) ? state[(int64_t)y * g.r.W + x] : (int8_t)1;
-    c += b == 0;
-    known |= (x < g.r.W && y < g.r.R && b != -1) ? 1 : 0;
-    const uint64_t fm = __ballot(b == 0);
-    const uint64_t um = __ballot(b == -1);
-    const int l = e & 63, r = e >> 6;
-    if (l < 16) tm[r * 16 + l] = fmask_byte(fm, um, l);
-    ew[0] |= (um & 1ull) << r;
-    ew[1] |= (um >> 63) << r;
-    if (r == 0) ew[2] = um;
-    if (r == DM_TS - 1) ew[3] = um;
-  }
+  const int l4 = __lane_id();
+  tile_record_rows(g, state, tile, threadIdx.x >> 6, 4, ew, [&](int r, uint8_t v) { tm[r * 16 + l4] = v; },
+                   [&](int, int8_t b, bool in) {
+                     c += b == 0;
+                     known |= (in && b != -1) ? 1 : 0;
+                   });
   if (c) atomicAdd(&acc, c);
   if (known) seen = 1;
-  const int l4 = __lane_id();
   if (l4 < 4) s_edge[threadIdx.x >> 6][l4] = l4 == 0 ? ew[0] : l4 == 1 ? ew[1] : l4 == 2 ? ew[2] : ew[3];
   __syncthreads();
   if (threadIdx.x == 0) {
@@ -1064,6 +1147,31 @@
   if (threadIdx.x < 4)
     fedge[tile * 4 + threadIdx.x] = s_edge[0][threadIdx.x] | s_edge[1][threadIdx.x] | s_edge[2][threadIdx.x] |
                                     s_edge[3][threadIdx.x];
+}
+
+__global__ __launch_bounds__(256) void k_check_records(Geom g, const int8_t* __restrict__ state,
+                                                       const uint8_t* __restrict__ fmask,
+                                                       const uint64_t* __restrict__ fedge,
+                                                       unsigned long long* mismatches) {
+  const int64_t tile = blockIdx.x;
+  __shared__ uint64_t s_edge[4][4];
+  __shared__ int32_t bad;
+  if (threadIdx.x == 0) bad = 0;
+  __syncthreads();
+  int32_t d = 0;
+  uint64_t ew[4] = {0ull, 0ull, 0ull, 0ull};
+  const uint8_t* tm = fmask + tile * (DM_TS * 16);
+  const int l4 = __lane_id();
+  tile_record_rows(g, state, tile, threadIdx.x >> 6, 4, ew, [&](int r, uint8_t v) { d += tm[r * 16 + l4] != v; },
+                   [](int, int8_t, bool) {});
+  if (l4 < 4) s_edge[threadIdx.x >> 6][l4] = l4 == 0 ? ew[0] : l4 == 1 ? ew[1] : l4 == 2 ? ew[2] : ew[3];
+  __syncthreads();
+  if (threadIdx.x < 4)
+    d += fedge[tile * 4 + threadIdx.x] != (s_edge[0][threadIdx.x] | s_edge[1][threadIdx.x] | s_edge[2][threadIdx.x] |
+                                           s_edge[3][threadIdx.x]);
+  if (d) atomicAdd(&bad, d);
+  __syncthreads();
+  if (threadIdx.x == 0 && bad) atomicAdd(mismatches, (unsigned long long)bad);
 }
 
 constexpr int kListIters = 16;
@@ -1109,73 +1217,6 @@
       pre += s_wn[i][0] + s_wn[i][1] + s_wn[i][2] + s_wn[i][3];
     }
     __syncthreads();
-  }
-}
-
-__device__ inline uint64_t upto_rows(int p) {
-  return p >= 63 ? ~0ull : ((2ull << p) - 1ull);
-}
-
-__global__ __launch_bounds__(256) void k_fmask_items(Geom g, const int4* __restrict__ list_a, int cnt_a,
-                                                     const int4* __restrict__ list_b, int cnt_b, int cnt_c,
-                                                     const PackedPiece* __restrict__ pieces,
-                                                     const unsigned long long* __restrict__ cnt,
-                                                     const int8_t* __restrict__ state, uint8_t* __restrict__ fmask,
-                                                     uint64_t* __restrict__ fedge,
-                                                     const unsigned long long* __restrict__ halt) {
-  if (*halt) return;
-  const int64_t HI = min((int64_t)cnt[cnt_a], g.hitem_cap);
-  const int64_t LI = min((int64_t)cnt[cnt_b], (int64_t)g.act_cap);
-  const int64_t SI = min((int64_t)cnt[cnt_c], (int64_t)g.act_cap);
-  const int lane = __lane_id();
-  for (int64_t it = (int64_t)blockIdx.x * 4 + (threadIdx.x >> 6); it < HI + LI + SI;
-       it += (int64_t)gridDim.x * 4) {
-    const int4 d = it < HI ? list_a[it]
-                           : (it < HI + LI ? list_b[it - HI] : list_b[(int64_t)g.act_cap - 1 - (it - HI - LI)]);
-    const int32_t tile = __builtin_amdgcn_readfirstlane(d.x);
-    uint64_t rows = ~0ull;
-    if (it >= HI + LI) {
-      const int32_t c0 = __builtin_amdgcn_readfirstlane(d.y);
-      const int32_t c = __builtin_amdgcn_readfirstlane(d.z);
-      uint64_t mine = 0ull;
-      if (lane < c && (int64_t)c0 + c <= g.seg_cap) {
-        const PackedPiece q = pieces[c0 + lane];
-        const TilePiece tp = dm_unpack_piece(q.x, q.y, q.z, q.w);
-        if (tp.len > 0) {
-          const int32_t ya = tp.addr0 / kLdsPitch;
-          const int32_t yb = dm_piece_addr(tp, tp.len - 1, __builtin_amdgcn_rcpf((float)tp.two_n)) / kLdsPitch;
-          const int lo = min(ya, yb), hi = max(ya, yb);
-          mine = upto_rows(hi) & ~(lo > 0 ? upto_rows(lo - 1) : 0ull);
-        }
-      }
-      for (int o = 32; o > 0; o >>= 1) mine |= __shfl_xor(mine, o);
-      rows = mine;
-    }
-    const int32_t tx0 = (tile % g.r.TX) * DM_TS, ty0 = (tile / g.r.TX) * DM_TS;
-    const int32_t x0 = tx0 + (lane & 3) * 16;
-    uint8_t* tm = fmask + (int64_t)tile * (DM_TS * 16);
-    EdgeAcc ea;
-#pragma unroll
-    for (int q = 0; q < 4; ++q) {
-      const int ly = 16 * q + (lane >> 2);
-      const bool mine = (rows >> ly) & 1ull;
-      const int32_t y = ty0 + ly;
-      uint32_t out = 0u;
-      if (mine && y < g.r.R) {
-        const int64_t off = (int64_t)y * g.r.W + x0;
-        if (x0 + 16 <= g.r.W && (off & 15) == 0) {
-          const uint4 v = *reinterpret_cast<const uint4*>(state + off);
-          const uint32_t wd[4] = {v.x, v.y, v.z, v.w};
-#pragma unroll
-          for (int k = 0; k < 4; ++k) out |= (uint32_t)state_nibbles(wd[k]) << (8 * k);
-        } else {
-          for (int k = 0; k < 4; ++k) out |= (uint32_t)state_nibbles_at(g, state, x0 + 4 * k, y) << (8 * k);
-        }
-      }
-      if (mine) *reinterpret_cast<uint32_t*>(tm + ly * 16 + (lane & 3) * 4) = out;
-      edge_acc(ea, out, q, lane);
-    }
-    edge_store(ea, fedge, tile, rows, lane);
   }
 }
 
@@ -1348,28 +1389,24 @@
 #ifndef DM_ACCUM_HINT
 #define DM_ACCUM_HINT 1
 #endif
-  const int64_t hw = DM_ACCUM_HINT ? (int64_t)hint[0] : 0, hi = DM_ACCUM_HINT ? (int64_t)hint[1] : 0;
+  const int64_t hw = DM_ACCUM_HINT ? (int64_t)hint[0] : 0;
   const int64_t accum_wgs = hw > 0 ? std::min(cap, dm_quantize_up(hw + hw / 16 + 64)) : cap;
-  DM_LAUNCH(k_tile_accum, dim3(grid_for(accum_wgs, 1, dm_grid::kAccumGrid)),
+  auto* const accum_kernel = vec_ok ? k_tile_accum<true> : k_tile_accum<false>;
+  DM_LAUNCH(accum_kernel, dim3(grid_for(accum_wgs, 1, dm_grid::kAccumGrid)),
                      dim3(kQuarter), 0,
                      g->stream, ge, make_apply(g), w.hitems, (int)CNT_ITEMS, w.litems, (int)CNT_LITEMS,
                      (int)CNT_SITEMS, w.pieces, w.tile_count, g->tile_free, w.slabs, g->L, g->state, w.cnt, w.sh, vec_ok,
                      w.heavy_list, w.heavy_done, g->ftiles, g->ftiles_n, g->d_hint, g->fe_flag + kHaltWord,
-                     g->tile_seen);
+                     g->tile_seen, g->fmask, g->fedge);
   dm_timer_end(g, &t);
   DM_HIP(hipGetLastError());
   if (g->overlap) w.free_owed = true;
-  if (!g->fmask_on) {
-    g->fmask_valid = false;
-    return DM_OK;
-  }
-  dm_timer_begin(g, "fmask", &t);
-  const int64_t fmask_items = hi > 0 ? std::min(cap, dm_quantize_up(hi + hi / 16 + 64)) : cap;
-  DM_LAUNCH(k_fmask_items, dim3(grid_for(fmask_items, 4, 8192)), dim3(256), 0, g->stream,
-                     ge, w.hitems, (int)CNT_ITEMS, w.litems, (int)CNT_LITEMS, (int)CNT_SITEMS, w.pieces, w.cnt,
-                     g->state, g->fmask, g->fedge,
-                     g->fe_flag + kHaltWord);
-  dm_timer_end(g, &t);
+  return DM_OK;
+}
+
+int dm_launch_check_records(dm_grid* g, unsigned long long* d_mismatches) {
+  DM_LAUNCH(k_check_records, dim3((unsigned)g->NT), dim3(256), 0, g->stream, make_geom(g), g->state, g->fmask,
+            g->fedge, d_mismatches);
   DM_HIP(hipGetLastError());
   return DM_OK;
 }
@@ -1416,9 +1453,7 @@
   DM_LAUNCH(k_recount, dim3((unsigned)g->NT), dim3(256), 0, g->stream, ge, g->state,
                      g->tile_free, g->fmask, g->fedge, g->tile_seen);
   DM_HIP(hipGetLastError());
-  if (int rc = dm_launch_relist(g, false)) return rc;
-  g->fmask_valid = true;
-  return DM_OK;
+  return dm_launch_relist(g, false);
 }
 
 int dm_launch_state_from_logodds(dm_grid* g) {
diff --git a/distributed-autonomous-exploration-and-mapping_amd/csrc/dm_internal.h b/distributed-autonomous-exploration-and-mapping_amd/csrc/dm_internal.h
--- a/distributed-autonomous-exploration-and-mapping_amd/csrc/dm_internal.h
+++ b/distributed-autonomous-exploration-and-mapping_amd/csrc/dm_internal.h
@@ -146,7 +146,6 @@
   uint8_t* fmask = nullptr;
   uint64_t* fedge = nullptr;
   uint8_t* tile_seen = nullptr;
-  bool fmask_on = false, fmask_valid = false;
   int fmask_mode = 0;
   unsigned long long* cnt = nullptr;
   unsigned long long* h_cnt = nullptr;
@@ -381,6 +380,7 @@
 int dm_launch_integrate(dm_grid* g, int32_t S, const double* d_pose4, int32_t N,
                         const float* d_ranges, const double* d_trig);
 int dm_launch_recount(dm_grid* g);
+int dm_launch_check_records(dm_grid* g, unsigned long long* d_mismatches);
 int dm_launch_relist(dm_grid* g, bool swap);
 constexpr int kRelistPasses = 16;
 int dm_launch_state_from_logodds(dm_grid* g);
@@ -401,7 +401,6 @@
                         int32_t* rank_of, unsigned long long* d_sorted, const unsigned long long* cnt,
                         int ncnt, int sorted_idx, const unsigned long long* fsh, dm_raw_record* host_out,
                         int64_t host_cap, int64_t expect);
-constexpr int64_t kFmaskOnTiles = 8192;
 constexpr int32_t kTileListed = 1 << 30;
 constexpr int32_t kTileFreeMask = kTileListed - 1;
 constexpr int64_t kSlotsPerTile = 4;
@@ -450,6 +449,7 @@
 int dm_sh_profile_read(dm_grid* g, dm_kernel_stat* out, int32_t cap, int32_t* n_out);
 int dm_sh_profile_reset(dm_grid* g);
 int dm_sh_map_image(dm_grid* g, uint8_t* out);
+int dm_sh_check_bit_records(dm_grid* g, int64_t* mismatches);
 int dm_sh_ld06_to_scans(dm_grid* g, int32_t S, const dm_ld06_point* points, const int64_t* offsets, int32_t N,
                         int dir, float* ranges, float* intensities);
 int dm_sh_ld06_to_scans_device(dm_grid* g, int32_t S, const dm_ld06_point* d_points, const int64_t* d_offsets,
diff --git a/distributed-autonomous-exploration-and-mapping_amd/csrc/dm_sharded.cpp b/distributed-autonomous-exploration-and-mapping_amd/csrc/dm_sharded.cpp
--- a/distributed-autonomous-exploration-and-mapping_amd/csrc/dm_sharded.cpp
+++ b/distributed-autonomous-exploration-and-mapping_amd/csrc/dm_sharded.cpp
@@ -487,6 +487,18 @@
   return DM_OK;
 }
 
+int dm_sh_check_bit_records(dm_grid* g, int64_t* mismatches) {
+  dm_shard_set* s = g->sh;
+  int64_t sum = 0;
+  for (int r = 0; r < s->P; ++r) {
+    int64_t n = 0;
+    if (int rc = dm_check_bit_records(s->band[(size_t)r], &n)) return rc;
+    sum += n;
+  }
+  *mismatches = sum;
+  return DM_OK;
+}
+
 int dm_sh_reset(dm_grid* g) {
   dm_shard_set* s = g->sh;
   for (int r = 0; r < s->P; ++r)
diff --git a/distributed-autonomous-exploration-and-mapping_amd/dm/_ffi.py b/distributed-autonomous-exploration-and-mapping_amd/dm/_ffi.py
--- a/distributed-autonomous-exploration-and-mapping_amd/dm/_ffi.py
+++ b/distributed-autonomous-exploration-and-mapping_amd/dm/_ffi.py
@@ -146,6 +146,7 @@
     "dm_profile_read": [_vp, ctypes.POINTER(DmKernelStat), _i32, ctypes.POINTER(_i32)],
     "dm_profile_reset": [_vp],
     "dm_map_image": [_vp, _vp],
+    "dm_check_bit_records": [_vp, ctypes.POINTER(_i64)],
     "dm_ld06_to_scans": [_vp, _i32, _vp, _vp, _i32, ctypes.c_int, _vp, _vp],
     "dm_ld06_to_scans_device": [_vp, _i32, _vp, _vp, _i32, ctypes.c_int, _vp, _vp],
     "dm_export_bytes": [_vp, _i64, ctypes.POINTER(_i64)],
diff --git a/distributed-autonomous-exploration-and-mapping_amd/dm/grid.py b/distributed-autonomous-exploration-and-mapping_amd/dm/grid.py
--- a/distributed-autonomous-exploration-and-mapping_amd/dm/grid.py
+++ b/distributed-autonomous-exploration-and-mapping_amd/dm/grid.py
@@ -199,6 +199,12 @@
             check(self._lib.dm_map_image(self._handle(), _vp(out)))
         return out
 
+    def check_bit_records(self) -> int:
+        n = ctypes.c_int64(-1)
+        with self._lock:
+            check(self._lib.dm_check_bit_records(self._handle(), ctypes.byref(n)))
+        return int(n.value)
+
     def assign_goals(self, robots_xy, min_size: int = 8, distance_weight: float = 1.0,
                      min_distance: float = 0.0):
         xy = np.ascontiguousarray(np.asarray(robots_xy, np.float64).reshape(-1, 2))
diff --git a/include/dm.h b/include/dm.h
--- a/include/dm.h
+++ b/include/dm.h
@@ -141,6 +141,8 @@
 
 int dm_map_image(dm_grid* g, uint8_t* out);
 
+int dm_check_bit_records(dm_grid* g, int64_t* mismatches);
+
 int dm_assign_goals(dm_grid* g, const double* robots_xy, int32_t n_robots, int64_t min_size,
                     double distance_weight, double min_distance, int64_t* out_index, double* out_xy);
 
```

Measured after the change: 205.0 billion. 0.962x the previous value.
